# KHU-VLL/DEVIAS

Measured on AMD Instinct MI355X. Metric: clips/sec fwd+bwd, ViT-B/16 16x224^2 slot head, bs=32/GPU, higher is better.
Workload: dtype bf16

## Files before the change

devias_amd/_lib.py:

```python
from __future__ import annotations

import ctypes
import os
from ctypes import POINTER, Structure, c_char_p, c_float, c_int, c_int32, c_int64, c_void_p

import torch

_HERE = os.path.dirname(os.path.abspath(__file__))
LIB_PATH = os.environ.get("DEVIAS_LIB_PATH") or os.path.join(_HERE, "libdevias_amd.so")

F32, BF16 = 0, 1
ATTN_Q_PRESCALED = 1
ABI_VERSION = 168
ACT_NONE, ACT_GELU, ACT_RELU, ACT_SIGMOID, ACT_DGELU, ACT_DRELU = 0, 1, 2, 3, 4, 5


class GemmArgs(Structure):
    _fields_ = [
        ("A", c_void_p), ("B", c_void_p), ("C", c_void_p),
        ("M", c_int32), ("N", c_int32), ("K", c_int32),
        ("lda", c_int32), ("ldb", c_int32), ("ldc", c_int32),
        ("trans_a", c_int32), ("trans_b", c_int32),
        ("dtype", c_int32), ("c_f32", c_int32),
        ("bias", c_void_p), ("act", c_int32),
        ("aux_in", c_void_p), ("aux_out", c_void_p), ("ld_aux", c_int32),
        ("res", c_void_p), ("ldr", c_int32), ("res_mod", c_int32),
        ("beta", c_float), ("split_k", c_int32), ("ws", c_void_p),
        ("colsum", c_void_p), ("colsum_beta", c_float),
        ("row_scale", c_void_p), ("rows_per_scale", c_int32),
        ("batch", c_int32), ("stride_a", c_int64), ("stride_b", c_int64), ("stride_c", c_int64),
        ("sk_ws", c_void_p), ("sk_ws_bytes", c_int64),
    ]


class LossDims(Structure):
    _fields_ = [(n, c_int32) for n in ("B", "S", "C", "nb", "ns", "D", "G", "N", "nh")] + \
               [("w_scene", c_float), ("w_mask_pred", c_float), ("w_mask_distill", c_float), ("dtype", c_int32), ("scene_ce", c_int32)]


_FP = POINTER(c_float)


class BlockArgs(Structure):
    _fields_ = [(n, c_int32) for n in ("B", "N", "D", "H", "hidden", "dtype")] + [("eps", c_float)] + \
               [(n, c_void_p) for n in ("n1w", "n1b", "n2w", "n2b", "Wqkv", "Wp", "W1", "W2", "qkv_bias", "pb", "b1", "b2", "ds1", "ds2", "save", "ws")] + \
               [("ws_bytes", c_int64), ("sk_ws", c_void_p), ("sk_ws_bytes", c_int64)] + \
               [(n, c_void_p) for n in ("WqkvT", "WpT", "W1T", "W2T")] + \
               [("WqkvS", c_void_p), ("qkv_biasS", c_void_p)]


class BlockGrads(Structure):
    _fields_ = [(n, c_void_p) for n in ("dn1w", "dn1b", "dWqkv", "dbqkv", "dWp", "dbp", "dn2w", "dn2b", "dW1", "db1", "dW2", "db2", "dx_colsum")] + \
               [("db2_done", c_int32), ("dbq", c_void_p), ("dbv", c_void_p)]


class HeadArgs(Structure):
    _fields_ = [(n, c_int32) for n in ("R", "D", "C", "h1", "h2", "G", "dtype")] + \
               [(n, c_void_p) for n in ("Wh", "W0", "W2", "W4", "bh", "b0", "b2", "b4", "ws")] + [("ws_bytes", c_int64), ("drop_mask", c_void_p)]


class HeadGrads(Structure):
    _fields_ = [(n, c_void_p) for n in ("dWh", "dbh", "dW0", "db0", "dW2", "db2", "dW4", "db4")]


AGG_MAX_DEPTH = 16
AGG_PARAM_FIELDS = ("Wq", "Wk", "Wv", "Wo", "W1", "W2", "bo", "norm_w", "norm_b", "ctx_w", "ctx_b", "b1", "b2", "ffn_w", "ffn_b")
AGG_GRAD_FIELDS = ("dWq", "dWk", "dWv", "dWo", "dbo", "dnorm_w", "dnorm_b", "dctx_w", "dctx_b", "dW1", "db1", "dW2", "db2", "dffn_w", "dffn_b")


class AggLayerParams(Structure):
    _fields_ = [(n, c_void_p) for n in AGG_PARAM_FIELDS]


class AggLayerGrads(Structure):
    _fields_ = [(n, c_void_p) for n in AGG_GRAD_FIELDS]


class AggArgs(Structure):
    _fields_ = [(n, c_int32) for n in ("B", "N", "S", "D", "depth", "tied", "heads", "dh", "ff", "dtype")] + \
               [("eps_enc", c_float), ("eps_agg", c_float)] + \
               [(n, c_void_p) for n in ("norm_w", "norm_b", "latents", "last_w", "last_b")] + \
               [("sets", AggLayerParams * AGG_MAX_DEPTH), ("save", c_void_p), ("ws", c_void_p), ("ws_bytes", c_int64)]


class AggGrads(Structure):
    _fields_ = [(n, c_void_p) for n in ("dnorm_w", "dnorm_b", "dlatents", "dlast_w", "dlast_b", "dx_colsum")] + \
               [("sets", AggLayerGrads * AGG_MAX_DEPTH)]


_P, _I, _L, _F = c_void_p, c_int32, c_int64, c_float
PROTOTYPES = {
    "devias_version": (c_int, []),
    "devias_last_error": (c_char_p, []),
    "devias_device_info": (c_int, [c_int, POINTER(c_int64)]),
    "devias_allreduce_bucket": (c_int, [_P, _P, _L, _I, _P]),
    "devias_shutdown": (None, []),
    "devias_counter": (c_int64, [c_int32]),
    "devias_counters_reset": (None, []),
    "devias_set_option": (c_int, [c_char_p, c_int32]),
    "devias_get_option": (c_int, [c_char_p, POINTER(c_int32)]),
    "devias_debug_mfma_probe": (c_int, [_P, _L, _I, _I, _P, _P, _P]),
    "devias_debug_mfma_probe_flops": (c_int64, [_I, _I]),
    "devias_debug_gemm_timer_arm": (c_int, [_I, _I, _I, _I, _I]),
    "devias_debug_dkdv_stamps": (c_int, [_P, _I]),
    "devias_debug_gemm_timer_read": (c_int, [POINTER(c_int32), POINTER(c_float)]),
    "devias_debug_gemm_timer_read_each": (c_int, [POINTER(c_int32), POINTER(c_float), c_int32]),
    "devias_gemm_release_queue_stream": (c_int, [_P]),
    "devias_gemm": (c_int, [POINTER(GemmArgs), _P]),
    "devias_gemm_workspace_bytes": (c_int64, [_I, _I, _I]),
    "devias_cast": (c_int, [_P, _I, _P, _I, _L, _P]),
    "devias_cast_scale": (c_int, [_P, _I, _P, _I, _L, c_float, _P]),
    "devias_patch_im2col": (c_int, [_P, _I, _P, _I, _I, _I, _I, _I, _I, _I, _I, _P]),
    "devias_colsum": (c_int, [_P, _I, _I, _I, _I, _P, _F, _P, _P]),
    "devias_colsum_workspace_bytes": (c_int64, [_I, _I]),
    "devias_rows_reduce_mod": (c_int, [_P, _I, _I, _I, _I, _P, _P]),
    "devias_rows_broadcast": (c_int, [_P, _I, _I, _P, _I, _I, _P]),
    "devias_act_bwd": (c_int, [_P, _P, _P, _I, _I, _L, _P]),
    "devias_row_scale": (c_int, [_P, _P, _I, _P, _I, _I, _I, _P]),
    "devias_add": (c_int, [_P, _P, _P, _I, _L, _P]),
    "devias_mul_mask": (c_int, [_P, _P, _P, _P, _I, _L, _P]),
    "devias_layernorm_fwd": (c_int, [_P, _P, _P, _P, _P, _P, _I, _I, _F, _I, _P]),
    "devias_layernorm_bwd": (c_int, [_P, _P, _P, _P, _P, _P, _P, _P, _P, _F, _P, _I, _I, _I, _P, _P]),
    "devias_layernorm_bwd_workspace_bytes": (c_int64, [_I, _I]),
    "devias_mhsa_fwd": (c_int, [_P, _P, _P, _I, _I, _I, _F, _I, _P]),
    "devias_mhsa_bwd": (c_int, [_P, _P, _P, _P, _P, _P, _I, _I, _I, _F, _I, _P, _P]),
    "devias_mhsa_fwd_flags": (c_int, [_P, _P, _P, _I, _I, _I, _F, _I, _I, _P]),
    "devias_mhsa_bwd_flags": (c_int, [_P, _P, _P, _P, _P, _P, _I, _I, _I, _F, _I, _P, _I, _P]),
    "devias_mhsa_bwd_bias_flags": (c_int, [_P, _P, _P, _P, _P, _P, _I, _I, _I, _F, _I, _F, ctypes.c_uint64, _P, _P, _P, _P, _I, _P]),
    "devias_mhsa_bwd_workspace_bytes": (c_int64, [_I, _I, _I]),
    "devias_mhsa_bwd_bias_dv_from_do": (c_int32, [_I, _F]),
    "devias_mhsa_fwd_dropout": (c_int, [_P, _P, _P, _I, _I, _I, _F, _I, _F, ctypes.c_uint64, _P]),
    "devias_mhsa_bwd_dropout": (c_int, [_P, _P, _P, _P, _P, _P, _I, _I, _I, _F, _I, _F, ctypes.c_uint64, _P]),
    "devias_mhsa_bwd_bias": (c_int, [_P, _P, _P, _P, _P, _P, _I, _I, _I, _F, _I, _F, ctypes.c_uint64, _P, _P, _P, _P, _P]),
    "devias_mhsa_bwd_bias_workspace_bytes": (c_int64, [_I, _I, _I]),
    "devias_slot_attn_fwd": (c_int, [_P, _P, _P, _P, _P, _I, _I, _I, _I, _I, _F, _I, _P, _P]),
    "devias_slot_attn_bwd": (c_int, [_P, _P, _P, _P, _P, _P, _P, _P, _P, _I, _I, _I, _I, _I, _F, _I, _P, _P]),
    "devias_slot_attn_kv_grad": (c_int, [_P, _P, _P, _P, _P, _P, _I, _I, _I, _I, _I, _I, _F, _I, _P]),
    "devias_slot_attn_workspace_bytes": (c_int64, [_I, _I, _I, _I, _I]),
    "devias_slotf_fwd": (c_int, [_P, _P, _P, _P, _P, _I, _I, _I, _I, _I, _F, _I, _P, _P]),
    "devias_slotf_bwd": (c_int, [_P, _P, _P, _P, _P, _P, _P, _P, _I, _I, _I, _I, _I, _F, _I, _P, _P]),
    "devias_slotf_pack": (c_int, [_P, _P, _P, _P, _P, _P, _P, _I, _I, _I, _I, _I, _I, _I, _F, _I, _P]),
    "devias_slotf_workspace_bytes": (c_int64, [_I, _I, _I, _I, _I]),
    "devias_slot_select": (c_int, [_P, _I, _I, _I, _I, _I, _P, _P]),
    "devias_head_match_loss_fwd": (c_int, [POINTER(LossDims), _P, _P, _P, _P, _P, _P, _P, _P, _P, _P, _P, _P, _P]),
    "devias_head_match_loss_bwd": (c_int, [POINTER(LossDims), _P, _P, _P, _P, _P, _P, _P, _P, _P, _P, _P, _P, _P, _P, _P]),
    "devias_head_match_loss_workspace_bytes": (c_int64, [_I]),
    "devias_head_match_loss_labels_fwd": (c_int, [POINTER(LossDims), _P, _P, _P, _P, _P, _P, _P, _P, _P, _P, _P, _P, _P]),
    "devias_head_match_loss_labels_bwd": (c_int, [POINTER(LossDims), _P, _P, _P, _P, _P, _P, _P, _P, _P, _P, _P, _P, _P, _P, _P]),
    "devias_adamw_step": (c_int, [_P, _P, _P, _P, _L, _F, _F, _F, _F, _F, _I, _F, _P]),
    "devias_grad_sumsq_multi": (c_int, [_P, _P, _P, _I, _P, _P]),
    "devias_clip_coef": (c_int, [_P, _I, _F, _P, _P]),
    "devias_adamw_multi": (c_int, [_P, _P, _P, _I, _F, _F, _F, _F, _P, _P]),
    "devias_fame_diff_color": (c_int, [_P, _I, _I, _I, _I, _P, _P, _P]),
    "devias_fame_blur": (c_int, [_P, _P, _I, _I, _I, _I, _F, _P]),
    "devias_fame_seg_refine": (c_int, [_P, _P, _I, _I, _I, _F, _P, _P]),
    "devias_fame_binarize_pool": (c_int, [_P, _I, _I, _I, _I, _I, _P, _P, _P]),
    "devias_fame_mix": (c_int, [_P, _P, _I, _P, _P, _P, _P, _I, _I, _I, _P]),
    "devias_debug_cu_hog": (c_int, [_I, _I, _P]),
    "devias_range_push": (None, [c_char_p]),
    "devias_range_pop": (None, []),
    "devias_encoder_block_save_bytes": (c_int64, [_I, _I, _I, _I, _I, _I]),
    "devias_encoder_block_scratch_bytes": (c_int64, [_I, _I, _I, _I, _I, _I]),
    "devias_encoder_block_workspace_bytes": (c_int64, [_I, _I, _I, _I, _I, _I]),
    "devias_encoder_block_fwd": (c_int, [POINTER(BlockArgs), _P, _P, _P]),
    "devias_encoder_block_bwd": (c_int, [POINTER(BlockArgs), _P, _P, _P, POINTER(BlockGrads), _P, _L, _P]),
    "devias_head_workspace_bytes": (c_int64, [_I, _I, _I, _I, _I, _I, _I]),
    "devias_head_save_bytes": (c_int64, [_I, _I, _I, _I, _I]),
    "devias_head_fwd": (c_int, [POINTER(HeadArgs), _P, _P, _P, _P, _P]),
    "devias_head_bwd": (c_int, [POINTER(HeadArgs), _P, _P, _P, _P, _P, _P, POINTER(HeadGrads), _P]),
    "devias_agg_block_save_bytes": (c_int64, [POINTER(AggArgs)]),
    "devias_agg_block_scratch_bytes": (c_int64, [POINTER(AggArgs)]),
    "devias_agg_block_workspace_bytes": (c_int64, [POINTER(AggArgs)]),
    "devias_agg_block_fwd": (c_int, [POINTER(AggArgs), _P, _P, POINTER(c_void_p), _P]),
    "devias_agg_block_bwd": (c_int, [POINTER(AggArgs), _P, _P, _P, _P, POINTER(AggGrads), _P, _L, _P]),
    "devias_policy_gemm_cus": (c_int32, []),
    "devias_policy_small_m_split": (c_int32, [_I, _I, _I, _I]),
    "devias_policy_wgrad_split": (c_int32, [_I, _I, _I, _I]),
}
COUNTERS = {"gemm128_f32": 0, "gemm128_bf16": 1, "gemm_ss": 2, "gemm256": 3, "gemm256p": 4, "splitk_reduce": 5,
            "mhsa_fwd_bf16": 6, "mhsa_bwd_bf16": 7, "mhsa_fwd_f32": 8, "mhsa_bwd_f32": 9, "mhsa_bwd_fused": 10, "gemm_sk": 11, "gemm256w": 12, "gemm_smallm": 13, "gemm256d": 14,
            "dkdv1w": 15, "dkdv1w_pers": 16, "dkdv1w_rest": 17, "dkdv2w": 18, "mhsa_qpre": 19, "loss_labels": 20}
OPT_CHUNK = 16384
OPT_TENSOR_BYTES = 64

_lib = None


class DeviasLibraryError(RuntimeError):
    pass


def load() -> ctypes.CDLL:
    global _lib
    if _lib is not None:
        return _lib
    if not os.path.exists(LIB_PATH):
        raise DeviasLibraryError(
            f"{LIB_PATH} is missing: the HIP extension is not built. Run `python -m devias_amd.build` "
            "(hipcc, gfx950). There is no CPU/PyTorch fallback for the DEVIAS hot path.")
    try:
        lib = ctypes.CDLL(LIB_PATH)
    except OSError as e:
        raise DeviasLibraryError(f"cannot load {LIB_PATH}: {e}") from e
    for name, (res, args) in PROTOTYPES.items():
        try:
            fn = getattr(lib, name)
        except AttributeError as e:
            raise DeviasLibraryError(f"{LIB_PATH} does not export {name}; rebuild it") from e
        fn.restype = res
        fn.argtypes = args
    if lib.devias_version() < ABI_VERSION:
        raise DeviasLibraryError(f"{LIB_PATH} is ABI version {lib.devias_version()}, this binding needs {ABI_VERSION}; rebuild it (python -m devias_amd.build --force)")
    _lib = lib
    return lib


CALLS = [0]


def check(rc: int, what: str) -> None:
    CALLS[0] += 1
    if rc != 0:
        msg = load().devias_last_error()
        raise RuntimeError(f"{what} failed (code {rc}): {msg.decode() if msg else '?'}")
```

devias_amd/csrc/api.hip:

```cpp
#include "common.h"
#include <string.h>

static thread_local char g_err[512] = "";

int devias_set_error(int code, const char* fmt, ...) {
    va_list ap;
    va_start(ap, fmt);
    vsnprintf(g_err, sizeof(g_err), fmt, ap);
    va_end(ap);
    return code;
}

extern "C" int devias_version(void) { return 168; }

#include <atomic>
static std::atomic<int64_t> g_cnt[DEVIAS_CNT_MAX];
void devias_count(int id) { if (id >= 0 && id < DEVIAS_CNT_MAX) g_cnt[id].fetch_add(1, std::memory_order_relaxed); }
extern "C" int64_t devias_counter(int32_t id) { return (id >= 0 && id < DEVIAS_CNT_MAX) ? g_cnt[id].load(std::memory_order_relaxed) : -1; }
extern "C" void devias_counters_reset(void) { for (int i = 0; i < DEVIAS_CNT_MAX; ++i) g_cnt[i].store(0, std::memory_order_relaxed); }

extern "C" int devias_set_option(const char* name, int32_t value) {
    if (!name) return devias_set_error(DEVIAS_EINVAL, "devias_set_option: null name");
    if (devias_gemm_set_option(name, value) || devias_attn_set_option(name, value)) return DEVIAS_OK;
    if (!strcmp(name, "regions_defer")) { devias_defer_enabled() = value; return DEVIAS_OK; }
    return devias_set_error(DEVIAS_EINVAL, "devias_set_option: unknown option '%s'", name);
}

extern "C" int devias_get_option(const char* name, int32_t* value) {
    if (!name || !value) return devias_set_error(DEVIAS_EINVAL, "devias_get_option: null argument");
    int v = 0;
    if (devias_gemm_get_option(name, &v) || devias_attn_get_option(name, &v)) { *value = v; return DEVIAS_OK; }
    if (!strcmp(name, "regions_defer")) { *value = devias_defer_enabled(); return DEVIAS_OK; }
    return devias_set_error(DEVIAS_EINVAL, "devias_get_option: unknown option '%s'", name);
}

extern "C" const char* devias_last_error(void) { return g_err; }
DeviasDeferList*& devias_defer_slot() { static thread_local DeviasDeferList* slot = nullptr; return slot; }
int& devias_defer_enabled() { static int on = [] { const char* e = getenv("DEVIAS_REGIONS_DEFER"); return e ? atoi(e) : 1; }(); return on; }

extern "C" int devias_device_info(int device, int64_t* out5) {
    if (!out5) return devias_set_error(DEVIAS_EINVAL, "devias_device_info: null output");
    hipDeviceProp_t p;
    hipError_t e = hipGetDeviceProperties(&p, device);
    if (e != hipSuccess) return devias_set_error(DEVIAS_ELAUNCH, "devias_device_info: %s", hipGetErrorString(e));
    out5[0] = p.multiProcessorCount;
    out5[1] = p.clockRate;
    out5[2] = (int64_t)p.sharedMemPerBlock;
    out5[3] = p.warpSize;
    int arch = 0;
    const char* s = strstr(p.gcnArchName, "gfx");
    if (s) arch = atoi(s + 3);
    out5[4] = arch;
    return DEVIAS_OK;
}


#include <dlfcn.h>
typedef int (*devias_nccl_allreduce_fn)(const void*, void*, size_t, int, int, void*, hipStream_t);
static devias_nccl_allreduce_fn resolve_allreduce() {
    static devias_nccl_allreduce_fn fn = [] {
        void* sym = dlsym(RTLD_DEFAULT, "ncclAllReduce");
        if (!sym) {
            void* h = dlopen("librccl.so", RTLD_NOW | RTLD_GLOBAL);
            if (!h) h = dlopen("librccl.so.1", RTLD_NOW | RTLD_GLOBAL);
            if (h) sym = dlsym(h, "ncclAllReduce");
        }
        return (devias_nccl_allreduce_fn)sym;
    }();
    return fn;
}
extern "C" int devias_allreduce_bucket(void* nccl_comm, void* bucket, int64_t count, int32_t dtype, void* stream) {
    if (!nccl_comm || !bucket || count <= 0) return devias_set_error(DEVIAS_EINVAL, "devias_allreduce_bucket: null communicator / bucket or empty bucket");
    if (dtype != DEVIAS_F32 && dtype != DEVIAS_BF16) return devias_set_error(DEVIAS_EINVAL, "devias_allreduce_bucket: bad dtype %d", dtype);
    devias_nccl_allreduce_fn fn = resolve_allreduce();
    if (!fn) return devias_set_error(DEVIAS_EUNSUPPORTED, "devias_allreduce_bucket: ncclAllReduce not found (librccl.so is not loadable)");
    const int nccl_dtype = dtype == DEVIAS_F32 ? 7  : 9 ;
    const int rc = fn(bucket, bucket, (size_t)count, nccl_dtype, 0 , nccl_comm, (hipStream_t)stream);
    if (rc != 0) return devias_set_error(DEVIAS_ELAUNCH, "devias_allreduce_bucket: ncclAllReduce returned %d", rc);
    return DEVIAS_OK;
}

extern "C" void devias_shutdown(void) { devias_counters_reset(); }


#include "roctx_shim.h"
#include <stdlib.h>
typedef int (*roctx_push_fn)(const char*);
typedef int (*roctx_pop_fn)(void);
static roctx_push_fn g_roctx_push = nullptr;
static roctx_pop_fn g_roctx_pop = nullptr;
static int g_roctx_state = -1;
static int roctx_resolve() {
    const char* e = getenv("DEVIAS_ROCTX");
    if (!e || atoi(e) == 0) return 0;
    const char* libs[] = {"librocprofiler-sdk-roctx.so", "librocprofiler-sdk-roctx.so.1", "libroctx64.so", "libroctx64.so.4"};
    for (const char* l : libs) {
// ... 17 lines not shown
```

devias_amd/csrc/gemm.hip:

```cpp
#include "common.h"
#include <mutex>
#include <utility>
#include <stdlib.h>
#include <string.h>
#include <atomic>

namespace {

enum { BM = 128, BN = 128, NTHREADS = 256 };

struct GemmP {
    const void* A; const void* B; void* C;
    int M, N, K, lda, ldb, ldc;
    const float* bias; int act;
    const void* aux_in; void* aux_out; int ld_aux;
    const void* res; int ldr, res_mod;
    float beta; int c_f32; int vec_c; int vec16;
    float* ws; int k_per_split; int split_k;
    int tiles_m, tiles_n;
    const float* row_scale; int rows_per_scale;
    float* colsum_part;
    int group_m;
    int epi_swap;
    int debug;
    int aux_nt;
    int c_nt;
    int tail_split;
    int64_t sA, sB, sC;
    unsigned int* tq; unsigned int* tq_clear; int tq_nwhole[2], tq_items[2];
};

#ifdef DEVIAS_GEMM_DEBUG
#define GDBG(flag) (p.debug & (flag))
#else
#define GDBG(flag) 0
#endif

template <typename T> struct Tr;
template <> struct Tr<bf16> {
    enum { BK = 64, KSTEP = 32, CH = 8, KC_BYTES = 128 * 128, KS_BYTES = 64 * 256 };
    typedef bf16x8 frag;
};
template <> struct Tr<float> {
    enum { BK = 16, KSTEP = 4, CH = 4, KC_BYTES = 128 * 20 * 4, KS_BYTES = 16 * 144 * 4 };
    typedef float frag;
};

__device__ __forceinline__ int ks_f(int k) { return (k & 3) | (((k >> 3) & 1) << 2); }
template <typename T> __device__ __forceinline__ int off_kc(int row, int k);
template <typename T> __device__ __forceinline__ int off_ks(int k, int col);
template <> __device__ __forceinline__ int off_kc<bf16>(int row, int k) {
    return row * 128 + ((((k >> 3) ^ (row & 7))) << 4) + (k & 7) * 2;
}
template <> __device__ __forceinline__ int off_ks<bf16>(int k, int col) {
    return k * 256 + ((((col >> 4) ^ ks_f(k))) << 5) + (col & 15) * 2;
}
template <> __device__ __forceinline__ int off_kc<float>(int row, int k) { return (row * 20 + k) * 4; }
template <> __device__ __forceinline__ int off_ks<float>(int k, int col) { return (k * 144 + col) * 4; }

template <typename T, bool KSTRIDED, bool VEC>
struct Stage {
    enum { BK = Tr<T>::BK, CH = Tr<T>::CH, NCH = 128 * BK / CH / NTHREADS, NEL = 128 * BK / NTHREADS };
    u32x4 v[NCH];

    __device__ __forceinline__ void load(const T* __restrict__ ptr, int ld, int r0, int R, int k0, int kend, int tid) {
        if constexpr (VEC) {
#pragma unroll
            for (int i = 0; i < NCH; ++i) {
                int c = tid + i * NTHREADS;
                int row, k;
                if constexpr (!KSTRIDED) { row = c / (BK / CH); k = (c % (BK / CH)) * CH; }
                else { k = c / (128 / CH); row = (c % (128 / CH)) * CH; }
                int gr = r0 + row, gk = k0 + k;
                bool ok = gr < R && gk < kend;
                const T* src = KSTRIDED ? ptr + (int64_t)gk * ld + gr : ptr + (int64_t)gr * ld + gk;
                u32x4 z = {0u, 0u, 0u, 0u};
                v[i] = ok ? *reinterpret_cast<const u32x4*>(src) : z;
            }
        } else {
            T* e = reinterpret_cast<T*>(v);
#pragma unroll
            for (int i = 0; i < NCH; ++i) {
                int c = tid + i * NTHREADS;
                int row, k;
                if constexpr (!KSTRIDED) { row = c / (BK / CH); k = (c % (BK / CH)) * CH; }
                else { k = c / (128 / CH); row = (c % (128 / CH)) * CH; }
#pragma unroll
                for (int j = 0; j < CH; ++j) {
                    int gr = r0 + row + (KSTRIDED ? j : 0), gk = k0 + k + (KSTRIDED ? 0 : j);
                    bool ok = gr < R && gk < kend;
                    const T* src = KSTRIDED ? ptr + (int64_t)gk * ld + gr : ptr + (int64_t)gr * ld + gk;
                    e[i * CH + j] = ok ? *src : from_f32<T>(0.f);
                }
            }
        }
    }

    __device__ __forceinline__ void store(char* lds, int tid) const {
#pragma unroll
        for (int i = 0; i < NCH; ++i) {
            int c = tid + i * NTHREADS;
            int off;
            if constexpr (!KSTRIDED) { int row = c / (BK / CH), k = (c % (BK / CH)) * CH; off = off_kc<T>(row, k); }
            else { int k = c / (128 / CH), col = (c % (128 / CH)) * CH; off = off_ks<T>(k, col); }
            *reinterpret_cast<u32x4*>(lds + off) = v[i];
        }
    }
};

template <bool KSTRIDED>
__device__ __forceinline__ bf16x8 read_frag(const char* lds, int base16, int ks, int lane, bf16*) {
    if constexpr (!KSTRIDED) {
// ... 590 lines not shown
template <int N>
__device__ __forceinline__ void tr_fence(TrFrag (&f)[N]) {
    static_assert(N == 4 || N == 8, "fragment groups of 4 (B) or 8 (A)");
    if constexpr (N == 4)
        asm volatile("s_waitcnt lgkmcnt(0)" : "+v"(f[0].lo), "+v"(f[0].hi), "+v"(f[1].lo), "+v"(f[1].hi), "+v"(f[2].lo), "+v"(f[2].hi), "+v"(f[3].lo), "+v"(f[3].hi) :: "memory");
    else
        asm volatile("s_waitcnt lgkmcnt(0)" : "+v"(f[0].lo), "+v"(f[0].hi), "+v"(f[1].lo), "+v"(f[1].hi), "+v"(f[2].lo), "+v"(f[2].hi), "+v"(f[3].lo), "+v"(f[3].hi),
                     "+v"(f[4].lo), "+v"(f[4].hi), "+v"(f[5].lo), "+v"(f[5].hi), "+v"(f[6].lo), "+v"(f[6].hi), "+v"(f[7].lo), "+v"(f[7].hi) :: "memory");
}
template <int N>
__device__ __forceinline__ void plain_fence(bf16x8 (&f)[N]) {
    static_assert(N == 4 || N == 8, "fragment groups of 4 (B) or 8 (A)");
    if constexpr (N == 4) asm volatile("s_waitcnt lgkmcnt(0)" : "+v"(f[0]), "+v"(f[1]), "+v"(f[2]), "+v"(f[3]) :: "memory");
    else asm volatile("s_waitcnt lgkmcnt(0)" : "+v"(f[0]), "+v"(f[1]), "+v"(f[2]), "+v"(f[3]), "+v"(f[4]), "+v"(f[5]), "+v"(f[6]), "+v"(f[7]) :: "memory");
}

__device__ __forceinline__ void ktile_nt_pinned(f32x4 (&acc)[8][4], const char* cur, char* nxt, const bf16* a_next, int lda,
                                                const bf16* b_next, int ldb, int wave, int lane, int wm, int wn) {
    const char* sA = cur; const char* sB = cur + 32768;
    const uint32_t vo_a = glds_voff_kc(lda, lane), vo_b = glds_voff_kc(ldb, lane);
    bf16x8 fb0[4], fb1[4], fa0[4], fa1[4];
#define G_RA(ks, ih, i) read_frag2<false>(sA, wm * 128 + ((ih) * 4 + (i)) * 16, ks, lane)
#define G_RB(ks, j) read_frag2<false>(sB, wn * 64 + (j) * 16, ks, lane)
#define G_MM4(ih, i, fb, fa) _Pragma("unroll") for (int j = 0; j < 4; ++j) acc[(ih) * 4 + (i)][j] = mfma16(fb[j], fa[i], acc[(ih) * 4 + (i)][j]);
#define G_SB __builtin_amdgcn_sched_barrier(0);
#define G_DMA(n) { const int r8 = wave * 32 + ((n) & 3) * 8; \
                   const char* ub = reinterpret_cast<const char*>((n) < 4 ? a_next + (int64_t)r8 * lda : b_next + (int64_t)r8 * ldb); \
                   __builtin_amdgcn_global_load_lds((glb_void_ptr)(ub + ((n) < 4 ? vo_a : vo_b)), (lds_void_ptr)(nxt + ((n) < 4 ? 0 : 32768) + r8 * 128), 16, 0, 0); }
    G_SB
#pragma unroll
    for (int j = 0; j < 4; ++j) fb0[j] = G_RB(0, j);
#pragma unroll
    for (int i = 0; i < 4; ++i) fa0[i] = G_RA(0, 0, i);
    G_SB
    G_MM4(0, 0, fb0, fa0) G_DMA(0) fa1[0] = G_RA(0, 1, 0); fb1[0] = G_RB(1, 0); G_SB
    G_MM4(0, 1, fb0, fa0) G_DMA(1) fa1[1] = G_RA(0, 1, 1); fb1[1] = G_RB(1, 1); G_SB
    G_MM4(0, 2, fb0, fa0) G_DMA(2) fa1[2] = G_RA(0, 1, 2); fb1[2] = G_RB(1, 2); G_SB
    G_MM4(0, 3, fb0, fa0) G_DMA(3) fa1[3] = G_RA(0, 1, 3); fb1[3] = G_RB(1, 3); G_SB
    G_MM4(1, 0, fb0, fa1) G_DMA(4) fa0[0] = G_RA(1, 0, 0); G_SB
    G_MM4(1, 1, fb0, fa1) G_DMA(5) fa0[1] = G_RA(1, 0, 1); G_SB
    G_MM4(1, 2, fb0, fa1) G_DMA(6) fa0[2] = G_RA(1, 0, 2); G_SB
    G_MM4(1, 3, fb0, fa1) G_DMA(7) fa0[3] = G_RA(1, 0, 3); G_SB
    G_MM4(0, 0, fb1, fa0) fa1[0] = G_RA(1, 1, 0); G_SB
    G_MM4(0, 1, fb1, fa0) fa1[1] = G_RA(1, 1, 1); G_SB
    G_MM4(0, 2, fb1, fa0) fa1[2] = G_RA(1, 1, 2); G_SB
    G_MM4(0, 3, fb1, fa0) fa1[3] = G_RA(1, 1, 3); G_SB
    G_MM4(1, 0, fb1, fa1) G_SB
    G_MM4(1, 1, fb1, fa1) G_SB
    G_MM4(1, 2, fb1, fa1) G_SB
    G_MM4(1, 3, fb1, fa1) G_SB
#undef G_RA
#undef G_RB
#undef G_MM4
#undef G_SB
#undef G_DMA
}

template <bool TA, bool TB>
__device__ __forceinline__ void ktile_generic(f32x4 (&acc)[8][4], const char* cur, int lane, int wm, int wn) {
#pragma unroll
    for (int ks = 0; ks < 2; ++ks) {
        bf16x8 fa[8], fb[4];
        if constexpr (TA || TB) {
            TrFrag ta[TA ? 8 : 1], tb[TB ? 4 : 1];
            if constexpr (!TB) { _Pragma("unroll") for (int j = 0; j < 4; ++j) fb[j] = read_frag2<false>(cur + 32768, wn * 64 + j * 16, ks, lane); }
            if constexpr (!TA) { _Pragma("unroll") for (int i = 0; i < 8; ++i) fa[i] = read_frag2<false>(cur, wm * 128 + i * 16, ks, lane); }
            if constexpr (TB) { _Pragma("unroll") for (int j = 0; j < 4; ++j) tb[j] = read_frag2a(cur + 32768, wn * 64 + j * 16, ks, lane); }
            if constexpr (TA) { _Pragma("unroll") for (int i = 0; i < 8; ++i) ta[i] = read_frag2a(cur, wm * 128 + i * 16, ks, lane); }
            if constexpr (TB) { tr_fence(tb); _Pragma("unroll") for (int j = 0; j < 4; ++j) fb[j] = tr_assemble(tb[j]); } else plain_fence(fb);
            if constexpr (TA) { tr_fence(ta); _Pragma("unroll") for (int i = 0; i < 8; ++i) fa[i] = tr_assemble(ta[i]); } else plain_fence(fa);
        } else {
#pragma unroll
            for (int j = 0; j < 4; ++j) fb[j] = read_frag2<TB>(cur + 32768, wn * 64 + j * 16, ks, lane);
#pragma unroll
            for (int i = 0; i < 8; ++i) fa[i] = read_frag2<TA>(cur, wm * 128 + i * 16, ks, lane);
        }
#pragma unroll
        for (int i = 0; i < 8; ++i)
#pragma unroll
            for (int j = 0; j < 4; ++j) acc[i][j] = mfma16(fb[j], fa[i], acc[i][j]);
    }
}

template <bool TA, bool TB, int PIN = 0>
__global__ __launch_bounds__(NT2) void gemm256_kernel(GemmP p) {
    __shared__ __attribute__((aligned(16))) char smem[2 * STAGE2];
    const int tid = threadIdx.x, lane = tid & 63;
    const int wave = __builtin_amdgcn_readfirstlane(tid >> 6);
    const int wm = wave >> 2, wn = wave & 3;
    const int ntiles = p.tiles_m * p.tiles_n;
    int t, z;
    if (gridDim.y == 1 && p.split_k > 1) {
        const int total = ntiles * p.split_k, per = (total + 7) >> 3;
        const int j = (int)(blockIdx.x & 7) * per + (int)(blockIdx.x >> 3);
        if (j >= total || (int)(blockIdx.x >> 3) >= per) return;
        z = j / ntiles; t = j - z * ntiles;
    } else {
        t = xcd_remap(blockIdx.x, ntiles);
        z = blockIdx.y;
    }
    int tm, tn;
    tile_coords(t, p.tiles_m, p.tiles_n, p.group_m, tm, tn);
    const int m0 = tm * T2, n0 = tn * T2;
    const int kbeg = z * p.k_per_split;
    const int kend = min(p.K, kbeg + p.k_per_split);
    int nk = (kend - kbeg) / 64;
    if (GDBG(1)) nk = min(nk, 1);
    const bf16* A = reinterpret_cast<const bf16*>(p.A);
    const bf16* B = reinterpret_cast<const bf16*>(p.B);

#ifdef DEVIAS_GEMM_DEBUG
    unsigned long long st0 = 0, st1 = 0, st2 = 0, st3 = 0;
    if (GDBG(8)) st0 = __builtin_amdgcn_s_memrealtime();
#endif
    f32x4 acc[8][4];
#pragma unroll
    for (int i = 0; i < 8; ++i)
#pragma unroll
        for (int j = 0; j < 4; ++j) acc[i][j] = f32x4{0.f, 0.f, 0.f, 0.f};

    if (nk > 0) {
        glds_tile<TA>(A, p.lda, m0, kbeg, smem, wave, lane);
        glds_tile<TB>(B, p.ldb, n0, kbeg, smem + 32768, wave, lane);
    }
    for (int kt = 0; kt < nk; ++kt) {
#ifdef DEVIAS_GEMM_DEBUG
        if (GDBG(8) && kt == 0) st1 = __builtin_amdgcn_s_memrealtime();
#endif
        asm volatile("s_waitcnt vmcnt(0)" ::: "memory");
        __syncthreads();
#ifdef DEVIAS_GEMM_DEBUG
        if (GDBG(8) && kt == 0) st2 = __builtin_amdgcn_s_memrealtime();
#endif
        char* cur = smem + (kt & 1) * STAGE2;
        char* nxt = smem + ((kt + 1) & 1) * STAGE2;
        if constexpr (!TA && !TB && PIN != 0) {
            const int kn = kbeg + (kt + 1 < nk ? kt + 1 : kt) * 64;
            ktile_nt_pinned(acc, cur, nxt, A + (int64_t)m0 * p.lda + kn, p.lda, B + (int64_t)n0 * p.ldb + kn, p.ldb, wave, lane, wm, wn);
        } else {
            if (kt + 1 < nk && !GDBG(4)) {
                glds_tile<TA>(A, p.lda, m0, kbeg + (kt + 1) * 64, nxt, wave, lane);
                glds_tile<TB>(B, p.ldb, n0, kbeg + (kt + 1) * 64, nxt + 32768, wave, lane);
            }
            ktile_generic<TA, TB>(acc, cur, lane, wm, wn);
        }
    }

#ifdef DEVIAS_GEMM_DEBUG
    if (GDBG(8)) {
        st3 = __builtin_amdgcn_s_memrealtime();
        if (tid == 0) {
            unsigned long long* d = reinterpret_cast<unsigned long long*>(p.ws) + (size_t)blockIdx.x * 6;
            d[0] = st0; d[1] = st1; d[2] = st2; d[3] = st3;
            d[4] = __builtin_amdgcn_s_getreg(0x1800 | 20) ; d[5] = t;
        }
    }
    if (GDBG(2) && acc[0][0][0] != 12345.678f) return;
#endif
    if constexpr (PIN == 1) asm volatile("s_waitcnt vmcnt(0)" ::: "memory");
    if (p.epi_swap) { epilogue_swap<8>(p, acc, m0 + wm * 128, n0 + wn * 64, z, lane); return; }
    __syncthreads();
    epilogue_staged<8, 4>(p, acc, smem + wave * 16384, m0 + wm * 128, n0 + wn * 64, z, lane);
}


__device__ __forceinline__ void piece_rows(int code, int& lo, int& hi) {
    if (code < 0) { lo = 0; hi = 16; }
    else if (code < 16) { lo = 8 * code; hi = lo + 8; }
    else if (code < 32) { const int i = code - 16; lo = i == 0 ? 0 : (i == 1 ? 5 : 11); hi = i == 0 ? 5 : (i == 1 ? 11 : 16); }
    else { lo = 4 * (code - 32); hi = lo + 4; }
}
__device__ __forceinline__ void piece_wave_rows(int code, int wm, int& il, int& ih) {
    int lo, hi;
    piece_rows(code, lo, hi);
    il = max(lo - 8 * wm, 0); ih = min(hi - 8 * wm, 8);
    if (ih < il) ih = il;
}
__device__ __forceinline__ bool piece_needs_wave_rows(int code, int w) {
    int lo, hi;
    piece_rows(code, lo, hi);
    return 2 * w < hi && 2 * w + 2 > lo;
}
template <int IL, int IH>
__device__ __forceinline__ void ktile_nt_rows(f32x4 (&acc)[IH - IL][4], const char* cur, int lane, int wm, int wn) {
#pragma unroll
    for (int ks = 0; ks < 2; ++ks) {
        bf16x8 fb[4];
#pragma unroll
        for (int j = 0; j < 4; ++j) fb[j] = read_frag2<false>(cur + 32768, wn * 64 + j * 16, ks, lane);
#pragma unroll
        for (int i = IL; i < IH; ++i) {
            const bf16x8 fa = read_frag2<false>(cur, wm * 128 + i * 16, ks, lane);
#pragma unroll
            for (int j = 0; j < 4; ++j) acc[i - IL][j] = mfma16(fb[j], fa, acc[i - IL][j]);
        }
    }
}

enum { TQ_RING = 64, TQ_LINE = 32 , TQ_SLOT = 16 * TQ_LINE, TQ_MASKS = 8 * TQ_LINE * 4 , TQ_NONE = 0x0fffffff };
__device__ unsigned int g_tile_queue[TQ_RING][TQ_SLOT];

__device__ __forceinline__ void tq_issue(unsigned& ticket, unsigned int* slot, int queue) {
    const unsigned voff = (unsigned)queue * (TQ_LINE * 4), one = 1u;
    asm volatile("s_nop 4\n\ts_mov_b64 exec, 1\n\tglobal_atomic_add %0, %1, %2, %3 sc0\n\ts_mov_b64 exec, -1" : "+v"(ticket) : "v"(voff), "v"(one), "s"(slot) : "memory");
}
__device__ __forceinline__ void tq_issue_claim(unsigned& old, unsigned int* slot, int queue, unsigned bit) {
    const unsigned voff = TQ_MASKS + (unsigned)queue * (TQ_LINE * 4);
    asm volatile("s_nop 4\n\ts_mov_b64 exec, 1\n\tglobal_atomic_or %0, %1, %2, %3 sc0\n\ts_mov_b64 exec, -1" : "+v"(old) : "v"(voff), "v"(bit), "s"(slot) : "memory");
}
__device__ __forceinline__ void tq_issue_peek(unsigned& snap, unsigned int* slot, int lane) {
    const unsigned voff = (unsigned)(lane & 15) * (TQ_LINE * 4), zero = 0u;
    asm volatile("s_nop 4\n\ts_mov_b64 exec, 0xffff\n\tglobal_atomic_add %0, %1, %2, %3 sc0\n\ts_mov_b64 exec, -1" : "+v"(snap) : "v"(voff), "v"(zero), "s"(slot) : "memory");
}
template <bool WAIT>
__device__ __forceinline__ void tq_publish(char* word, unsigned seq, int code) {
    const unsigned v = ((seq & 15u) << 28) | ((unsigned)code & 0x0fffffffu);
    const unsigned addr = (unsigned)(size_t)(__attribute__((address_space(3))) char*)word;
    if constexpr (WAIT) asm volatile("ds_write_b32 %0, %1\n\ts_waitcnt lgkmcnt(0)" ::"v"(addr), "v"(v) : "memory");
    else asm volatile("ds_write_b32 %0, %1" ::"v"(addr), "v"(v) : "memory");
}
__device__ __forceinline__ int tq_read(const char* word, unsigned seq) {
    unsigned v;
    const unsigned addr = (unsigned)(size_t)(__attribute__((address_space(3))) const char*)word;
    asm volatile("ds_read_b32 %0, %1\n\ts_waitcnt lgkmcnt(0)" : "=v"(v) : "v"(addr) : "memory");
    v = __builtin_amdgcn_readfirstlane(v);
    return (v >> 28) == (seq & 15u) ? (int)(v & 0x0fffffffu) : -2;
}

template <bool TB, int SIDE, bool DYN, int EPI = -1>
__global__ __launch_bounds__(NT2) void gemm256p_kernel(GemmP p) {
    __shared__ __attribute__((aligned(16))) char smem[2 * STAGE2 + (DYN ? 16 : 0)];
    const int tid = threadIdx.x, lane = tid & 63;
#ifdef DEVIAS_GEMM_DEBUG
    const unsigned long long t_entry = __builtin_amdgcn_s_memrealtime();
#endif
    const int wave = __builtin_amdgcn_readfirstlane(tid >> 6);
    const int wm = wave >> 2, wn = wave & 3;
    const int ntiles = p.tiles_m * p.tiles_n;
    const int nk = p.K / 64;
    const bf16* A = reinterpret_cast<const bf16*>(p.A);
    const bf16* B = reinterpret_cast<const bf16*>(p.B);
    const int xcd = blockIdx.x & 7, stride = gridDim.x >> 3;
    const int q = ntiles >> 3, r = ntiles & 7;
    const int base = xcd < r ? xcd * (q + 1) : r * (q + 1) + (xcd - r) * q;
    const int cnt = q + (xcd < r ? 1 : 0);
    const int li0 = blockIdx.x >> 3;
    int li = li0;
    if constexpr (!DYN) { if (li >= cnt) return; }
    auto coords = [&](int l, int& m0, int& n0) {
        int tm, tn;
        tile_coords(base + l, p.tiles_m, p.tiles_n, p.group_m, tm, tn);
        m0 = tm * T2; n0 = tn * T2;
    };
    const int rfull = cnt / stride, rem = cnt - rfull * stride;
    const bool split = p.tail_split != 0 && rfull >= 1 && rem > 0 && 2 * rem <= stride;
    const int parts = (!split || DYN || TB || p.colsum_part != nullptr || p.tail_split < 3) ? 2 : min(min(p.tail_split, 4), stride / rem);
    auto tile_at = [&](int k, int& l, int& half) -> bool {
        half = -1;
        if (k < rfull) { l = li0 + k * stride; return true; }
        if (k > rfull) return false;
        if (split) {
            if (li0 >= parts * rem) return false;
            l = rfull * stride + li0 / parts;
            half = (parts == 2 ? 0 : (parts == 3 ? 16 : 32)) + li0 % parts;
            return true;
        }
        if (li0 >= rem) return false;
        l = rfull * stride + li0;
        return true;
    };
    char* const tq_word = smem + 2 * STAGE2;
    int nwhole_a = p.tq_nwhole[0], nwhole_b = p.tq_nwhole[1], items_a = p.tq_items[0], items_b = p.tq_items[1];
    unsigned int* tq = p.tq;
    if constexpr (DYN) asm volatile("" : "+s"(nwhole_a), "+s"(nwhole_b), "+s"(items_a), "+s"(items_b), "+s"(tq));
    auto qgeom = [&](int y, int& qbase, int& nwhole, int& items) {
        qbase = y < r ? y * (q + 1) : r * (q + 1) + (y - r) * q;
        nwhole = y < r ? nwhole_a : nwhole_b;
        items = y < r ? items_a : items_b;
    };
    auto decode = [&](int code, int& m0, int& n0, int& half) {
        const int y = code >> 20, i = code & 0xfffff;
        int qbase, nwhole, items;
        qgeom(y, qbase, nwhole, items);
        const int l = i < nwhole ? i : nwhole + ((i - nwhole) >> 1);
        half = i < nwhole ? -1 : ((i - nwhole) & 1);
        int tm, tn;
        tile_coords(qbase + l, p.tiles_m, p.tiles_n, p.group_m, tm, tn);
        m0 = tm * T2; n0 = tn * T2;
    };
    int fq = xcd;
    bool fdead = false;
    unsigned ticket = 0, seq = 0;
    auto settle = [&]() -> int {
        const int t = stride + (int)__builtin_amdgcn_readfirstlane(ticket);
        int qbase, nwhole, items;
        qgeom(fq, qbase, nwhole, items);
        return t < items ? ((fq << 20) | t) : -2;
    };
    auto find_elsewhere = [&]() -> int {
        const int lane_f = __builtin_amdgcn_mbcnt_hi(~0u, __builtin_amdgcn_mbcnt_lo(~0u, 0u));
        const unsigned wmask = stride >= 32 ? 0xffffffffu : ((1u << stride) - 1u);
        for (int attempt = 0; attempt < 256 && !fdead; ++attempt) {
            unsigned snap = 0;
            tq_issue_peek(snap, tq, lane_f);
            asm volatile("s_waitcnt vmcnt(0)" : "+v"(snap) :: "memory");
            int pick = -1, kind = 0;
            unsigned bit = 0;
            for (int d = 1; d <= 8 && pick < 0; ++d) {
                const int y = (xcd + d) & 7;
                int qbase, nwhole, items;
                qgeom(y, qbase, nwhole, items);
                if (stride + (int)__builtin_amdgcn_readlane(snap, y) < items) pick = y;
            }
            for (int d = 0; d < 8 && pick < 0 && !(p.debug & 512); ++d) {
                const int y = (xcd + d) & 7;
                const unsigned avail = ~(unsigned)__builtin_amdgcn_readlane(snap, 8 + y) & wmask;
                if (avail) { pick = y; kind = 1; bit = avail & (0u - avail); }
            }
            if (pick < 0) { fdead = true; break; }
            if (kind == 0) {
                fq = pick;
                tq_issue(ticket, tq, fq);
                asm volatile("s_waitcnt vmcnt(0)" : "+v"(ticket) :: "memory");
                const int c = settle();
                if (c != -2) return c;
            } else {
                unsigned old = 0;
                tq_issue_claim(old, tq, pick, bit);
                asm volatile("s_waitcnt vmcnt(0)" : "+v"(old) :: "memory");
                if (!((unsigned)__builtin_amdgcn_readfirstlane(old) & bit)) return (pick << 20) | (int)__builtin_ctz(bit);
            }
        }
        fdead = true;
        return (int)TQ_NONE;
    };
    if constexpr (DYN) {
        if (blockIdx.x == 0 && tid < 16)
            asm volatile("s_nop 4\n\tglobal_store_dword %0, %1, %2 sc1" ::"v"((unsigned)tid * (TQ_LINE * 4)), "v"(0u), "s"(p.tq_clear) : "memory");
    }
// ... 58 lines not shown
                tq_publish<true>(tq_word + 4, 1, c1);
                if (c1 != (int)TQ_NONE && !fdead) tq_issue(ticket, tq, fq);
            }
            __builtin_amdgcn_s_barrier();
            asm volatile("" ::: "memory");
            const int code = tq_read(tq_word, 0);
            if (code == (int)TQ_NONE) return;
            if (code != ((xcd << 20) | li0)) {
                decode(code, m0, n0, half);
                __builtin_amdgcn_s_barrier();
                glds_tile<false>(A, p.lda, m0, 0, smem, wave, lane);
                glds_tile<TB>(B, p.ldb, n0, 0, smem + 32768, wave, lane);
                asm volatile("s_waitcnt vmcnt(0)" ::: "memory");
            }
            ncode = tq_read(tq_word + 4, 1);
            has_next = ncode != (int)TQ_NONE;
            m0n = m0; n0n = n0;
            if (has_next) decode(ncode, m0n, n0n, halfn);
            seq = 2;
        }
        bool act = half < 0 || wm == half;
        bool tail_piece = false;
        int gtail = 0;
        for (int g = 0, kt = 0;; ++g) {
            __builtin_amdgcn_s_barrier();
            asm volatile("" ::: "memory");
            if (kt == 0) { PSTAMP(1); PSTAMP(9); }
            char* cur = smem + (g & 1) * STAGE2;
            char* nxt = smem + ((g + 1) & 1) * STAGE2;
            const bool same = kt + 1 < nk;
            const int am = (same || !has_next) ? m0 : m0n, bn = (same || !has_next) ? n0 : n0n;
            const int kn = same ? (kt + 1) * 64 : (has_next ? 0 : kt * 64);
            int lane_k = __builtin_amdgcn_mbcnt_hi(~0u, __builtin_amdgcn_mbcnt_lo(~0u, 0u));
            asm volatile("" : "+v"(lane_k));
            const bool stage_a = p.tail_split < 2 || act || (DYN && !same && has_next && (halfn < 0 || wm == halfn));
            if constexpr (!TB) {
                if (act) ktile_nt_pinned(acc, cur, nxt, A + (int64_t)am * p.lda + kn, p.lda, B + (int64_t)bn * p.ldb + kn, p.ldb, wave, lane_k, wm, wn);
                else {
                    if (stage_a) glds_tile<false>(A, p.lda, am, kn, nxt, wave, lane_k);
                    glds_tile<false>(B, p.ldb, bn, kn, nxt + 32768, wave, lane_k);
                }
            } else {
                if (stage_a) glds_tile<false>(A, p.lda, am, kn, nxt, wave, lane_k);
                glds_tile<true>(B, p.ldb, bn, kn, nxt + 32768, wave, lane_k);
                if (act) ktile_generic<false, true>(acc, cur, lane_k, wm, wn);
            }
            if (same) {
                ++kt;
                asm volatile("s_waitcnt vmcnt(0)" ::: "memory");
                if (kt == 1) PSTAMP(4);
                continue;
            }
            PSTAMP(2); PSTAMP(10);
            int lane_e = __builtin_amdgcn_mbcnt_hi(~0u, __builtin_amdgcn_mbcnt_lo(~0u, 0u));
            asm volatile("" : "+v"(lane_e));
            if (act) epilogue_swap<8, true, SIDE, EPI>(p, acc, m0 + wm * 128, n0 + wn * 64, 0, lane_e);
            if (!has_next) break;
            int m0x = 0, n0x = 0, halfx = -1;
            bool issued = false;
            if constexpr (DYN) {
                PSTAMP(5);
                if (wave == 0) {
                    asm volatile("" : "+v"(ticket));
                    int c = fdead ? (int)TQ_NONE : settle();
                    if (c == -2) c = find_elsewhere();
                    tq_publish<false>(tq_word, seq, c);
                    issued = c != (int)TQ_NONE && !fdead;
                    if (issued) tq_issue(ticket, tq, fq);
                }
                do { ncode = tq_read(tq_word, seq); } while (ncode == -2);
                ++seq;
                if (ncode != (int)TQ_NONE) decode(ncode, m0x, n0x, halfx);
                PSTAMP(6);
            }
            if (DYN && !act) asm volatile("s_waitcnt vmcnt(0)" ::: "memory");
#if !defined(TQ_EXP) || TQ_EXP != 1
            else if (DYN && issued) asm volatile("s_waitcnt vmcnt(17)" ::: "memory");
#endif
            else asm volatile("s_waitcnt vmcnt(16)" ::: "memory");
            PSTAMP(3);
            kt = 0;
            ++tk;
            m0 = m0n; n0 = n0n; half = halfn;
            if (!DYN && !TB && half >= 16) { tail_piece = true; gtail = g + 1; break; }
            act = half < 0 || wm == half;
            if constexpr (!DYN) {
                int ln = li;
                has_next = tile_at(tk + 1, ln, halfn);
                if (has_next) coords(ln, m0n, n0n);
            } else {
                has_next = ncode != (int)TQ_NONE;
                if (has_next) { m0n = m0x; n0n = n0x; halfn = halfx; }
            }
#pragma unroll
            for (int i = 0; i < 8; ++i)
#pragma unroll
                for (int j = 0; j < 4; ++j) acc[i][j] = f32x4{0.f, 0.f, 0.f, 0.f};
        }
        if constexpr (!DYN && !TB && !(EPI >= 0 && (EPI & EPI_CS))) {
            if (tail_piece) {
                int il, ih;
                piece_wave_rows(half, wm, il, ih);
                auto run = [&](auto ilc, auto ihc) {
                    constexpr int IL = decltype(ilc)::value, IH = decltype(ihc)::value, NR = IH > IL ? IH - IL : 1;
                    f32x4 tacc[NR][4];
#pragma unroll
                    for (int i = 0; i < NR; ++i)
#pragma unroll
                        for (int j = 0; j < 4; ++j) tacc[i][j] = f32x4{0.f, 0.f, 0.f, 0.f};
                    const bool stage_a = p.tail_split < 2 || piece_needs_wave_rows(half, wave);
                    for (int kt = 0, g = gtail; kt < nk; ++kt, ++g) {
                        __builtin_amdgcn_s_barrier();
                        asm volatile("" ::: "memory");
                        char* cur = smem + (g & 1) * STAGE2;
                        char* nxt = smem + ((g + 1) & 1) * STAGE2;
                        int lane_k = __builtin_amdgcn_mbcnt_hi(~0u, __builtin_amdgcn_mbcnt_lo(~0u, 0u));
                        asm volatile("" : "+v"(lane_k));
                        if (kt + 1 < nk) {
                            if (stage_a) glds_tile<false>(A, p.lda, m0, (kt + 1) * 64, nxt, wave, lane_k);
                            glds_tile<false>(B, p.ldb, n0, (kt + 1) * 64, nxt + 32768, wave, lane_k);
                        }
                        if constexpr (IH > IL) ktile_nt_rows<IL, IH>(tacc, cur, lane_k, wm, wn);
                        asm volatile("s_waitcnt vmcnt(0)" ::: "memory");
                    }
                    if constexpr (IH > IL) {
                        int lane_e = __builtin_amdgcn_mbcnt_hi(~0u, __builtin_amdgcn_mbcnt_lo(~0u, 0u));
                        asm volatile("" : "+v"(lane_e));
                        epilogue_swap<NR, true, SIDE, EPI>(p, tacc, m0 + wm * 128 + IL * 16, n0 + wn * 64, 0, lane_e);
                    }
                };
                using std::integral_constant;
                if (il >= ih) run(integral_constant<int, 0>{}, integral_constant<int, 0>{});
                else if (il == 0 && ih == 5) run(integral_constant<int, 0>{}, integral_constant<int, 5>{});
                else if (il == 5 && ih == 8) run(integral_constant<int, 5>{}, integral_constant<int, 8>{});
                else if (il == 0 && ih == 3) run(integral_constant<int, 0>{}, integral_constant<int, 3>{});
                else if (il == 3 && ih == 8) run(integral_constant<int, 3>{}, integral_constant<int, 8>{});
                else if (il == 0 && ih == 4) run(integral_constant<int, 0>{}, integral_constant<int, 4>{});
                else run(integral_constant<int, 4>{}, integral_constant<int, 8>{});
            }
        }
        asm volatile("s_waitcnt vmcnt(0)" ::: "memory");
    }
}


enum { NTW = 256 };

#define DEVIAS_A10(b) "a" #b "0", "a" #b "1", "a" #b "2", "a" #b "3", "a" #b "4", "a" #b "5", "a" #b "6", "a" #b "7", "a" #b "8", "a" #b "9"
template <int I> __device__ __forceinline__ void acc_zero1() { asm volatile("v_accvgpr_write_b32 a[%c0], 0" ::"i"(I)); }
template <int... I> __device__ __forceinline__ void acc_zero_seq(std::integer_sequence<int, I...>) { (acc_zero1<I>(), ...); }
__device__ __forceinline__ void acc_claim() {
    asm volatile("" ::: DEVIAS_A10(), DEVIAS_A10(1), DEVIAS_A10(2), DEVIAS_A10(3), DEVIAS_A10(4), DEVIAS_A10(5), DEVIAS_A10(6), DEVIAS_A10(7), DEVIAS_A10(8), DEVIAS_A10(9),
                 DEVIAS_A10(10), DEVIAS_A10(11), DEVIAS_A10(12), DEVIAS_A10(13), DEVIAS_A10(14), DEVIAS_A10(15), DEVIAS_A10(16), DEVIAS_A10(17), DEVIAS_A10(18), DEVIAS_A10(19),
                 DEVIAS_A10(20), DEVIAS_A10(21), DEVIAS_A10(22), DEVIAS_A10(23), DEVIAS_A10(24), "a250", "a251", "a252", "a253", "a254", "a255");
}
__device__ __forceinline__ void acc_zero() { acc_zero_seq(std::make_integer_sequence<int, 256>{}); }
template <int I> __device__ __forceinline__ float acc_read1() { float x; asm volatile("v_accvgpr_read_b32 %0, a[%c1]" : "=v"(x) : "i"(I)); return x; }

template <int SIDE>
__device__ __forceinline__ bf16x8 side_load_w(const GemmP& p, int mrow0, int ncol0, int lane, int n) {
    const int lm = lane & 15, g = lane >> 4;
    const bf16* side = reinterpret_cast<const bf16*>(SIDE == 1 ? p.res : p.aux_in);
    const int side_ld = SIDE == 1 ? p.ldr : p.ld_aux;
    const int h = n >> 4, i = (n >> 1) & 7, pr = n & 1;
    int m = mrow0 + i * 16 + lm;
    if (SIDE == 1 && p.res_mod > 0) m %= p.res_mod;
    return *reinterpret_cast<const bf16x8*>(side + (int64_t)m * side_ld + ncol0 + 64 * h + 16 * (2 * pr + (g & 1)) + 8 * (g >> 1));
}

template <int SIDE>
__device__ __forceinline__ void epilogue_w(const GemmP& p, int mrow0, int ncol0, int lane, bf16x8 (&sbuf)[SIDE != 0 ? 16 : 1]) {
    const int lm = lane & 15, g = lane >> 4;
    const uint32_t col2 = (uint32_t)(16 * (g & 1) + 8 * (g >> 1)) * 2;
    const uint32_t vo_c = (uint32_t)lm * (uint32_t)p.ldc * 2 + col2, vo_x = (uint32_t)lm * (uint32_t)p.ld_aux * 2 + col2;
    constexpr bool BIAS_ON = SIDE != 2, CS_ON = SIDE != 1;
    f32x4 bias4[BIAS_ON ? 8 : 1];
    if constexpr (BIAS_ON) {
#pragma unroll
        for (int j = 0; j < 8; ++j) bias4[j] = p.bias ? *reinterpret_cast<const f32x4*>(p.bias + ncol0 + j * 16 + g * 4) : f32x4{0.f, 0.f, 0.f, 0.f};
    }
    float rs_lo = 1.f, rs_hi = 1.f;
    int rs_edge = 0;
    if (p.row_scale) {
        const int r0 = mrow0 / p.rows_per_scale, rl = (p.M - 1) / p.rows_per_scale;
        rs_lo = p.row_scale[r0]; rs_hi = p.row_scale[r0 < rl ? r0 + 1 : rl];
        rs_edge = (r0 + 1) * p.rows_per_scale;
    }
    bf16* aux_out = reinterpret_cast<bf16*>(p.aux_out);
    constexpr int PF = 16;
    auto side_load = [&](int n) -> bf16x8 { return side_load_w<SIDE>(p, mrow0, ncol0, lane, n); };
    float cs[CS_ON ? 4 : 1][8];
    if constexpr (CS_ON) {
#pragma unroll
        for (int c = 0; c < 4; ++c)
#pragma unroll
            for (int e = 0; e < 8; ++e) cs[c][e] = 0.f;
    }
    static_for<32>([&](auto nc) {
        constexpr int n = decltype(nc)::value, h = n >> 4, i = (n >> 1) & 7, pr = n & 1;
        constexpr int ra = 16 * (8 * h + i) + 8 * pr;
        const int m = mrow0 + i * 16 + lm;
        bf16x8 side8 = sbuf[SIDE != 0 ? n % PF : 0];
        if constexpr (SIDE != 0 && n + PF < 32) sbuf[n % PF] = side_load(n + PF);
        f32x4 A = f32x4{acc_read1<ra>(), acc_read1<ra + 1>(), acc_read1<ra + 2>(), acc_read1<ra + 3>()};
        f32x4 B = f32x4{acc_read1<ra + 4>(), acc_read1<ra + 5>(), acc_read1<ra + 6>(), acc_read1<ra + 7>()};
        if constexpr (BIAS_ON) { A += bias4[4 * h + 2 * pr]; B += bias4[4 * h + 2 * pr + 1]; }
        else { A += f32x4{0.f, 0.f, 0.f, 0.f}; B += f32x4{0.f, 0.f, 0.f, 0.f}; }
        float v[8];
#pragma unroll
        for (int r = 0; r < 4; ++r) {
            const auto sw = __builtin_amdgcn_permlane16_swap(__float_as_uint(A[r]), __float_as_uint(B[r]), false, false);
            v[r] = __uint_as_float(sw[0]);
            v[4 + r] = __uint_as_float(sw[1]);
        }
        if constexpr (SIDE == 2) {
            if (p.act == DEVIAS_ACT_DGELU) {
#pragma unroll
                for (int e = 0; e < 8; e += 2) {
                    const f32x2 d = dgelu_fast2(f32x2{(float)side8[e], (float)side8[e + 1]});
                    v[e] *= d[0]; v[e + 1] *= d[1];
                }
            } else {
#pragma unroll
                for (int e = 0; e < 8; ++e) v[e] = (float)side8[e] > 0.f ? v[e] : 0.f;
// ... 490 lines not shown
        for (int w = 0; w < 3; ++w) v += red[w][t][lane];
        if (m >= p.M) continue;
        if (p.bias) v += bias;
        if (p.act == DEVIAS_ACT_GELU) {
            if (aux_out) store4(aux_out + (int64_t)m * p.ld_aux + n, v);
#pragma unroll
            for (int e = 0; e < 4; ++e) v[e] = gelu_t<bf16>(v[e]);
        } else if (p.act == DEVIAS_ACT_RELU) {
#pragma unroll
            for (int e = 0; e < 4; ++e) v[e] = fmaxf(v[e], 0.f);
        } else if (p.act == DEVIAS_ACT_SIGMOID) {
#pragma unroll
            for (int e = 0; e < 4; ++e) v[e] = 1.0f / (1.0f + expf(-v[e]));
        } else if (dact) {
            const f32x4 a4 = {(float)auxv[t][0], (float)auxv[t][1], (float)auxv[t][2], (float)auxv[t][3]};
#pragma unroll
            for (int e = 0; e < 4; ++e) v[e] = p.act == DEVIAS_ACT_DGELU ? v[e] * dgelu_t<bf16>(a4[e]) : (a4[e] > 0.f ? v[e] : 0.f);
        }
        if (p.row_scale) v *= p.row_scale[m / p.rows_per_scale];
        if (res) v += f32x4{(float)resv[t][0], (float)resv[t][1], (float)resv[t][2], (float)resv[t][3]};
        store4(C + (int64_t)m * p.ldc + n, v);
    }
}

__global__ __launch_bounds__(256) void splitk_reduce_plain_kernel(const float* __restrict__ ws, int split_k, int64_t total4, float* __restrict__ C, float beta) {
    for (int64_t i = (int64_t)blockIdx.x * 256 + threadIdx.x; i < total4; i += (int64_t)gridDim.x * 256) {
        f32x4 v = *reinterpret_cast<const f32x4*>(ws + i * 4);
        for (int z = 1; z < split_k; ++z) v += *reinterpret_cast<const f32x4*>(ws + ((int64_t)z * total4 + i) * 4);
        if (beta != 0.f) v += beta * *reinterpret_cast<const f32x4*>(C + i * 4);
        *reinterpret_cast<f32x4*>(C + i * 4) = v;
    }
}

__global__ void gemm_colsum_final_kernel(const float* __restrict__ part, int nparts, int N, float* __restrict__ out, float beta) {
    __shared__ float sm[16][64];
    int n = blockIdx.x * 64 + threadIdx.x;
    float s = 0.f;
    if (n < N)
        for (int i = threadIdx.y; i < nparts; i += 16) s += part[(int64_t)i * N + n];
    sm[threadIdx.y][threadIdx.x] = s;
    __syncthreads();
    if (threadIdx.y == 0 && n < N) {
        float t = 0.f;
#pragma unroll
        for (int k = 0; k < 16; ++k) t += sm[k][threadIdx.x];
        out[n] = t + (beta != 0.f ? beta * out[n] : 0.f);
    }
}

template <typename T, bool VEC>
int launch(const GemmP& p, int ta, int tb, hipStream_t st, int batch = 1) {
    dim3 grid(p.tiles_m * p.tiles_n, p.split_k, batch), block(NTHREADS);
    if (!ta && !tb) hipLaunchKernelGGL((gemm_kernel<T, false, false, VEC>), grid, block, 0, st, p);
    else if (!ta && tb) hipLaunchKernelGGL((gemm_kernel<T, false, true, VEC>), grid, block, 0, st, p);
    else if (ta && tb) hipLaunchKernelGGL((gemm_kernel<T, true, true, VEC>), grid, block, 0, st, p);
    else hipLaunchKernelGGL((gemm_kernel<T, true, false, VEC>), grid, block, 0, st, p);
    return 0;
}

}

extern "C" int64_t devias_gemm_workspace_bytes(int32_t M, int32_t N, int32_t split_k) {
    return split_k > 1 ? (int64_t)split_k * M * N * 4 : 0;
}

namespace {
struct GemmKnobs {
    int epi_swap;
    int use256;
    int use_ss;
    int group_m;
    int persistent;
    int debug;
    int epi_spec;
    int wt;
    int aux_nt;
    int smallm;
    int tail_split;
    int w4;
    int splitk_xcd;
    int dynamic;
    int concurrent;
    int reserve;
    int ncu;
};
int env_int(const char* name, int dflt) { const char* e = getenv(name); return e ? atoi(e) : dflt; }
GemmKnobs& knobs() {
    static GemmKnobs k = [] {
        GemmKnobs x;
        x.epi_swap = env_int("DEVIAS_GEMM_EPI", 1);
        x.use256 = env_int("DEVIAS_GEMM256", 1);
        x.use_ss = env_int("DEVIAS_GEMM_SS", -1);
        x.group_m = env_int("DEVIAS_GEMM_GROUPM", 0);
        x.persistent = env_int("DEVIAS_GEMM_PERSIST", 1);
        x.debug = env_int("DEVIAS_GEMM_DEBUG", 0);
        x.reserve = env_int("DEVIAS_GEMM_RESERVE_CUS", 0);
        x.splitk_xcd = env_int("DEVIAS_GEMM_SPLITK_XCD", 1);
        x.dynamic = env_int("DEVIAS_GEMM_DYNAMIC", -1);
        x.concurrent = env_int("DEVIAS_GEMM_CONCURRENT", 0);
        x.w4 = env_int("DEVIAS_GEMM_W4", -1);
        x.tail_split = env_int("DEVIAS_GEMM_TAIL_SPLIT", 3);
        x.smallm = env_int("DEVIAS_GEMM_SMALLM", 1);
        x.epi_spec = env_int("DEVIAS_GEMM_EPI_SPEC", 1);
        x.wt = env_int("DEVIAS_GEMM_WT", 1);
        x.aux_nt = env_int("DEVIAS_GEMM_AUX_NT", 5);
        x.ncu = 0;
        return x;
    }();
    return k;
}
}

namespace {
struct TileQueueRing { unsigned int* base; hipStream_t owner; bool owned; unsigned seq; };
std::mutex g_tq_mutex;
TileQueueRing g_tq_ring[16];
}
static bool tile_queue_slot(hipStream_t st, unsigned int** slot, unsigned int** clear) {
    int dev = 0;
    if (hipGetDevice(&dev) != hipSuccess || dev < 0 || dev >= 16) return false;
    std::lock_guard<std::mutex> lock(g_tq_mutex);
    TileQueueRing& r = g_tq_ring[dev];
    if (!r.base) {
        void* sym = nullptr;
        if (hipGetSymbolAddress(&sym, HIP_SYMBOL(g_tile_queue)) != hipSuccess || !sym) { (void)hipGetLastError(); return false; }
        r.base = reinterpret_cast<unsigned int*>(sym);
    }
    if (!r.owned) { r.owner = st; r.owned = true; }
    if (r.owner != st) return false;
    const unsigned n = r.seq++;
    *slot = r.base + (size_t)(n % TQ_RING) * TQ_SLOT;
    *clear = r.base + (size_t)((n + TQ_RING / 2) % TQ_RING) * TQ_SLOT;
    return true;
}
extern "C" int devias_gemm_release_queue_stream(void* stream) {
    int dev = 0;
    if (hipGetDevice(&dev) != hipSuccess || dev < 0 || dev >= 16) return devias_set_error(DEVIAS_EINVAL, "devias_gemm_release_queue_stream: no current device");
    std::lock_guard<std::mutex> lock(g_tq_mutex);
    TileQueueRing& r = g_tq_ring[dev];
    if (r.base && hipMemsetAsync(r.base, 0, sizeof(unsigned int) * TQ_RING * TQ_SLOT, (hipStream_t)stream) != hipSuccess) {
        (void)hipGetLastError();
        return devias_set_error(DEVIAS_EINVAL, "devias_gemm_release_queue_stream: cannot zero the ring");
    }
    r.owner = (hipStream_t)stream; r.owned = true; r.seq = 0;
    return DEVIAS_OK;
}

int devias_policy_gemm_wt(void) { return knobs().wt; }

extern "C" int32_t devias_policy_gemm_cus(void) {
    const GemmKnobs& k = knobs();
    const int ncu = devias_device_cus();
    return (ncu - k.reserve > 8 ? ncu - k.reserve : 8) & ~7;
}

static int* gemm_option_slot(const char* name) {
    GemmKnobs& k = knobs();
    if (!strcmp(name, "gemm_epi")) return &k.epi_swap;
    if (!strcmp(name, "gemm256")) return &k.use256;
    if (!strcmp(name, "gemm_ss")) return &k.use_ss;
    if (!strcmp(name, "gemm_groupm")) return &k.group_m;
    if (!strcmp(name, "gemm_persistent")) return &k.persistent;
    if (!strcmp(name, "gemm_debug")) return &k.debug;
    if (!strcmp(name, "gemm_w4")) return &k.w4;
    if (!strcmp(name, "gemm_tail_split")) return &k.tail_split;
    if (!strcmp(name, "gemm_smallm")) return &k.smallm;
    if (!strcmp(name, "gemm_epi_spec")) return &k.epi_spec;
    if (!strcmp(name, "gemm_wt")) return &k.wt;
    if (!strcmp(name, "gemm_aux_nt")) return &k.aux_nt;
    if (!strcmp(name, "gemm_reserve_cus")) return &k.reserve;
    if (!strcmp(name, "gemm_splitk_xcd")) return &k.splitk_xcd;
    if (!strcmp(name, "gemm_dynamic")) return &k.dynamic;
    if (!strcmp(name, "gemm_concurrent")) return &k.concurrent;
    return nullptr;
}
int devias_gemm_set_option(const char* name, int value) {
    int* slot = gemm_option_slot(name);
    if (!slot) return 0;
    *slot = (!strcmp(name, "gemm_reserve_cus") && value < 0) ? 0 : value;
    return 1;
}
int devias_gemm_get_option(const char* name, int* value) {
    const int* slot = gemm_option_slot(name);
    if (!slot) return 0;
    *value = *slot;
    return 1;
}

namespace {
template <bool TB, int SIDE, bool DYN, int EPI>
void pers_launch1(dim3 grid, hipStream_t st, const GemmP& p) { hipLaunchKernelGGL((gemm256p_kernel<TB, SIDE, DYN, EPI>), grid, dim3(NT2), 0, st, p); }
template <bool DYN>
void pers_launch(bool tb, int side, int epi, dim3 grid, hipStream_t st, const GemmP& p) {
    if (!tb && side == 0) {
        if (epi == EPI_BIAS) pers_launch1<false, 0, DYN, EPI_BIAS>(grid, st, p);
        else if (epi == (DEVIAS_ACT_GELU | EPI_BIAS | EPI_AUX)) pers_launch1<false, 0, DYN, DEVIAS_ACT_GELU | EPI_BIAS | EPI_AUX>(grid, st, p);
        else if (epi == 0) pers_launch1<false, 0, DYN, 0>(grid, st, p);
        else if (epi == EPI_CS) pers_launch1<false, 0, DYN, EPI_CS>(grid, st, p);
        else pers_launch1<false, 0, DYN, -1>(grid, st, p);
    } else if (!tb && side == 1) {
        if (epi == EPI_BIAS) pers_launch1<false, 1, DYN, EPI_BIAS>(grid, st, p);
        else pers_launch1<false, 1, DYN, -1>(grid, st, p);
    } else if (!tb) {
        if (epi == (DEVIAS_ACT_DGELU | EPI_CS)) pers_launch1<false, 2, DYN, DEVIAS_ACT_DGELU | EPI_CS>(grid, st, p);
        else pers_launch1<false, 2, DYN, -1>(grid, st, p);
    } else if (side == 0) pers_launch1<true, 0, DYN, -1>(grid, st, p);
    else pers_launch1<true, 2, DYN, -1>(grid, st, p);
}
}

static int gemm_impl(const devias_gemm_args* a, void* stream) {
    hipStream_t st = (hipStream_t)stream;
    DEVIAS_REQUIRE(a && a->A && a->B && a->C, "devias_gemm: null operand");
    DEVIAS_REQUIRE(a->M > 0 && a->N > 0 && a->K > 0, "devias_gemm: bad dims M=%d N=%d K=%d", a->M, a->N, a->K);
    DEVIAS_REQUIRE(a->dtype == DEVIAS_F32 || a->dtype == DEVIAS_BF16, "devias_gemm: bad dtype %d", a->dtype);
    DEVIAS_REQUIRE(a->act >= 0 && a->act <= DEVIAS_ACT_DRELU, "devias_gemm: bad act %d", a->act);
    if (a->act == DEVIAS_ACT_DGELU || a->act == DEVIAS_ACT_DRELU)
        DEVIAS_REQUIRE(a->aux_in, "devias_gemm: act %d needs aux_in", a->act);
    const GemmKnobs& kn = knobs();
    const int es = a->dtype == DEVIAS_BF16 ? 2 : 4;
    const int ch = 16 / es;
    GemmP p;
    p.A = a->A; p.B = a->B; p.C = a->C;
    p.M = a->M; p.N = a->N; p.K = a->K; p.lda = a->lda; p.ldb = a->ldb; p.ldc = a->ldc;
    p.bias = a->bias; p.act = a->act; p.aux_in = a->aux_in; p.aux_out = a->aux_out; p.ld_aux = a->ld_aux;
    p.res = a->res; p.ldr = a->ldr; p.res_mod = a->res_mod;
    p.c_f32 = (a->c_f32 || a->dtype == DEVIAS_F32) ? 1 : 0;
    p.beta = p.c_f32 ? a->beta : 0.f;
    p.tiles_m = cdiv(a->M, BM); p.tiles_n = cdiv(a->N, BN);
    const int BK = a->dtype == DEVIAS_BF16 ? 64 : 16;
    int split = a->split_k > 1 ? a->split_k : 1;
    if (split > 1) {
        DEVIAS_REQUIRE(a->ws, "devias_gemm: split_k needs a workspace");
        int kps = cdiv(cdiv(a->K, split), BK) * BK;
        split = cdiv(a->K, kps);
        p.k_per_split = kps;
    } else {
        p.k_per_split = a->K;
    }
    p.split_k = split; p.ws = a->ws;
    p.colsum_part = nullptr;
    p.row_scale = a->row_scale; p.rows_per_scale = a->rows_per_scale > 0 ? a->rows_per_scale : 1;
    bool vec = aligned16(a->A) && aligned16(a->B) && (a->lda % ch == 0) && (a->ldb % ch == 0);
    vec = vec && (a->trans_a ? (a->M % ch == 0) : (a->K % ch == 0));
    vec = vec && (a->trans_b ? (a->N % ch == 0) : (a->K % ch == 0));
    if (a->batch > 1) vec = vec && (a->stride_a % ch == 0) && (a->stride_b % ch == 0);
    bool vc = (a->N % 4 == 0) && (a->ldc % 4 == 0) && (p.c_f32 ? aligned16(a->C) : aligned8(a->C));
    if (a->bias) vc = vc && aligned16(a->bias);
    if (a->res) vc = vc && (a->ldr % 4 == 0) && aligned8(a->res);
    if (a->aux_in) vc = vc && (a->ld_aux % 4 == 0) && aligned8(a->aux_in);
    if (a->aux_out) vc = vc && (a->ld_aux % 4 == 0) && aligned8(a->aux_out);
    if (es == 4) vc = vc && (!a->res || aligned16(a->res)) && (!a->aux_in || aligned16(a->aux_in)) &&
                      (!a->aux_out || aligned16(a->aux_out)) && aligned16(a->C);
    if (a->batch > 1) vc = vc && (a->stride_c % 4 == 0);
    p.vec_c = vc ? 1 : 0;
    const int batch = a->batch > 1 ? a->batch : 1;
    p.sA = batch > 1 ? a->stride_a : 0; p.sB = batch > 1 ? a->stride_b : 0; p.sC = batch > 1 ? a->stride_c : 0;
    if (batch > 1)
        DEVIAS_REQUIRE(split == 1 && !a->colsum && !a->res && !a->aux_in && !a->aux_out && batch <= 65535,
                       "devias_gemm: batched launches support bias / activation epilogues only (no split-K, residual, aux, colsum)");
    p.debug = kn.debug;
    p.tail_split = kn.tail_split;
    p.aux_nt = kn.aux_nt;
    p.c_nt = ((kn.aux_nt & 4) && a->aux_out) ? 1 : 0;
    p.epi_swap = kn.epi_swap;
    p.tq = nullptr; p.tq_clear = nullptr; p.tq_nwhole[0] = p.tq_nwhole[1] = p.tq_items[0] = p.tq_items[1] = 0;
    p.group_m = kn.group_m > 0 ? kn.group_m : ((!a->trans_a && a->N >= 2048) ? 8 : 1);

    const bool v16 = vc && (a->N % 8 == 0) && (a->ldc % 8 == 0) && aligned16(a->C) && (!a->bias || aligned16(a->bias)) &&
                     (!a->res || ((a->ldr % 8 == 0) && aligned16(a->res))) &&
                     (!a->aux_in || ((a->ld_aux % 8 == 0) && aligned16(a->aux_in))) &&
                     (!a->aux_out || ((a->ld_aux % 8 == 0) && aligned16(a->aux_out))) && (split == 1 || aligned16(a->ws));
    p.vec16 = (v16 && a->dtype == DEVIAS_BF16) ? 1 : 0;
    bool big = kn.use256 && a->dtype == DEVIAS_BF16 && vec && vc && (a->M % T2 == 0) && (a->N % T2 == 0) && (a->K % 64 == 0) &&
               (p.k_per_split % 64 == 0);
    big = big && v16 && batch == 1;
    bool ss = kn.use_ss != 0 && a->dtype == DEVIAS_BF16 && vec && v16 && (a->M % SS_BM == 0) && (a->N % SS_BN == 0) && (a->K % 64 == 0) &&
              (p.k_per_split % 64 == 0) && batch == 1 && !(a->trans_a && !a->trans_b);
    if (ss && big) {
        const bool nt = !a->trans_a && !a->trans_b;
        if (kn.use_ss < 0 || nt) ss = false;
    }
    const bool smallm = kn.smallm && a->dtype == DEVIAS_BF16 && !a->trans_a && (!a->trans_b || kn.smallm == 1) && a->M <= 128 && batch == 1 && !p.c_f32 && !a->colsum && vec && vc &&
                        (a->N % 16 == 0) && (a->K % 128 == 0) && (a->lda % 8 == 0) && (a->ldb % 8 == 0) && (a->ldc % 4 == 0) && aligned8(a->C) &&
                        (!a->bias || aligned16(a->bias)) && (!a->res || (a->ldr % 4 == 0 && aligned8(a->res))) &&
                        (!a->aux_in || (a->ld_aux % 4 == 0 && aligned8(a->aux_in))) && (!a->aux_out || (a->ld_aux % 4 == 0 && aligned8(a->aux_out)));
    if (smallm) {
        p.split_k = 1; p.k_per_split = a->K;
        const int mt = cdiv(a->M, 16);
        dim3 grid(a->N / 16), block(256);
        if (a->trans_b) { grid = dim3(a->N / 16, mt); hipLaunchKernelGGL((gemm_smallm_kernel<1, 12, true>), grid, block, 0, st, p); }
        else if (kn.smallm == 1 && mt > 1 && a->N / 16 < 128) { grid = dim3(a->N / 16, mt); hipLaunchKernelGGL((gemm_smallm_kernel<1, 12>), grid, block, 0, st, p); }
        else
        if (mt <= 1) hipLaunchKernelGGL((gemm_smallm_kernel<1, 12>), grid, block, 0, st, p);
        else if (mt <= 2) hipLaunchKernelGGL((gemm_smallm_kernel<2>), grid, block, 0, st, p);
        else if (mt <= 4) hipLaunchKernelGGL((gemm_smallm_kernel<4>), grid, block, 0, st, p);
        else if (mt <= 6) hipLaunchKernelGGL((gemm_smallm_kernel<6>), grid, block, 0, st, p);
        else hipLaunchKernelGGL((gemm_smallm_kernel<8>), grid, block, 0, st, p);
        devias_count(DEVIAS_CNT_GEMM_SMALLM);
        DEVIAS_CHECK_LAUNCH("devias_gemm(small M)");
        return DEVIAS_OK;
    }
    bool colsum_fused = false;
    if (a->colsum) {
        DEVIAS_REQUIRE(split == 1 && a->ws && !(a->c_f32 && a->dtype == DEVIAS_BF16),
                       "devias_gemm: colsum needs split_k == 1, a workspace (M/128 * N floats) and a T-typed C");
        if (ss || big) { p.colsum_part = a->ws; colsum_fused = true; }
    }
    if (ss) {
        p.tiles_m = a->M / SS_BM; p.tiles_n = a->N / SS_BN;
        dim3 grid(p.tiles_m * p.tiles_n, p.split_k), block(SS_NT);
        const int ta = a->trans_a, tb = a->trans_b;
        if (!ta && !tb) hipLaunchKernelGGL((gemm_ss_kernel<false, false, 2>), grid, block, 0, st, p);
        else if (!ta && tb) hipLaunchKernelGGL((gemm_ss_kernel<false, true, 2>), grid, block, 0, st, p);
        else hipLaunchKernelGGL((gemm_ss_kernel<true, true, 2>), grid, block, 0, st, p);
        devias_count(DEVIAS_CNT_GEMM_SS);
    } else if (big) {
        p.tiles_m = a->M / T2; p.tiles_n = a->N / T2;
        const int ta = a->trans_a, tb = a->trans_b;
        const int nt = p.tiles_m * p.tiles_n;
        const bool dyn = kn.dynamic > 0 || (kn.dynamic < 0 && kn.concurrent != 0);
        const int gp = dyn ? (devias_device_cus() & ~7) : devias_policy_gemm_cus();
        const bool dact = a->act == DEVIAS_ACT_DGELU || a->act == DEVIAS_ACT_DRELU;
        const int side = a->res ? 1 : (dact ? 2 : 0);
        const bool pers_ok = !ta && split == 1 && !p.c_f32 && p.epi_swap && gp >= 8 && !(a->res && dact) && !(tb && side == 1) &&
                             (!a->row_scale || p.rows_per_scale >= 128) && !(side == 2 && a->bias) && !(side == 1 && a->colsum) &&
                             !(side != 0 && a->aux_out);
#define PERS_LAUNCH(KERNEL, ...) do { \
            if (!tb) { if (side == 0) hipLaunchKernelGGL((KERNEL<false, 0 __VA_ARGS__>), grid, block, 0, st, p); else hipLaunchKernelGGL((KERNEL<false, 1 __VA_ARGS__>), grid, block, 0, st, p); } \
            else { if (side == 0) hipLaunchKernelGGL((KERNEL<true, 0 __VA_ARGS__>), grid, block, 0, st, p); else hipLaunchKernelGGL((KERNEL<true, 2 __VA_ARGS__>), grid, block, 0, st, p); } } while (0)
        const int w4_form = (tb ? 2 : 0) + (side != 0 ? 1 : 0);
        const int w4_mask = kn.w4 >= 0 ? kn.w4 : 0;
        const bool w4_ok = kn.persistent && !dyn && ((w4_mask >> w4_form) & 1) && pers_ok && !(!tb && side == 2) && nt > gp && a->K >= 128 &&
                           (a->act == DEVIAS_ACT_NONE || a->act == DEVIAS_ACT_GELU || a->act == DEVIAS_ACT_DGELU || a->act == DEVIAS_ACT_DRELU);
        if (w4_ok) {
            dim3 grid(gp), block(NTW);
            PERS_LAUNCH(gemm256w_kernel);
            devias_count(DEVIAS_CNT_GEMM256P);
            devias_count(DEVIAS_CNT_GEMM256W);
        } else if (kn.persistent && pers_ok && nt > gp) {
            dim3 grid(gp);
            const int epi = !kn.epi_spec ? -1 : (a->act | (a->bias ? EPI_BIAS : 0) | (a->aux_out ? EPI_AUX : 0) | (a->row_scale ? EPI_RS : 0) | (p.colsum_part ? EPI_CS : 0));
            unsigned int *tq = nullptr, *tq_clear = nullptr;
            if (!(dyn && a->K >= 128 && (gp >> 3) <= 32 && (nt >> 3) >= (gp >> 3) && tile_queue_slot(st, &tq, &tq_clear))) tq = nullptr;
            if (tq) {
                p.tq = tq;
                p.tq_clear = tq_clear;
                const int stride = gp >> 3;
                for (int v = 0; v < 2; ++v) {
                    const int cnt = (nt >> 3) + (v == 0 ? 1 : 0);
                    const int rfull = cnt / stride, rem = cnt - rfull * stride;
                    const bool split = kn.tail_split != 0 && rfull >= 1 && rem > 0 && 2 * rem <= stride;
                    p.tq_nwhole[v] = split ? rfull * stride : cnt;
                    p.tq_items[v] = split ? rfull * stride + 2 * rem : cnt;
                }
                pers_launch<true>(tb != 0, side, epi, grid, st, p);
                devias_count(DEVIAS_CNT_GEMM256D);
            } else {
                pers_launch<false>(tb != 0, side, epi, grid, st, p);
            }
            devias_count(DEVIAS_CNT_GEMM256P);
        } else {
            dim3 grid(nt, p.split_k), block(NT2);
            if (p.split_k > 1 && kn.splitk_xcd) grid = dim3(8 * ((nt * p.split_k + 7) / 8));
            if (!ta && !tb) hipLaunchKernelGGL((gemm256_kernel<false, false, 1>), grid, block, 0, st, p);
            else if (!ta && tb) hipLaunchKernelGGL((gemm256_kernel<false, true>), grid, block, 0, st, p);
            else if (ta && tb) hipLaunchKernelGGL((gemm256_kernel<true, true>), grid, block, 0, st, p);
            else hipLaunchKernelGGL((gemm256_kernel<true, false>), grid, block, 0, st, p);
            devias_count(DEVIAS_CNT_GEMM256);
        }
    } else if (a->dtype == DEVIAS_BF16) {
        if (vec) launch<bf16, true>(p, a->trans_a, a->trans_b, st, batch);
        else launch<bf16, false>(p, a->trans_a, a->trans_b, st, batch);
        devias_count(DEVIAS_CNT_GEMM128_BF16);
    } else {
        if (vec) launch<float, true>(p, a->trans_a, a->trans_b, st, batch);
        else launch<float, false>(p, a->trans_a, a->trans_b, st, batch);
        devias_count(DEVIAS_CNT_GEMM128_F32);
    }
    DEVIAS_CHECK_LAUNCH("devias_gemm");
    if (a->colsum) {
        const DeviasReduceJob cj = {a->ws, a->M / 128, a->N, a->N, a->colsum, a->colsum_beta};
        if (colsum_fused && devias_defer(&cj, 1)) {
        } else if (colsum_fused) {
            hipLaunchKernelGGL(gemm_colsum_final_kernel, dim3(cdiv(a->N, 64)), dim3(64, 16), 0, st, a->ws, a->M / 128, a->N, a->colsum, a->colsum_beta);
            DEVIAS_CHECK_LAUNCH("devias_gemm(colsum)");
        } else {
            int rc = devias_colsum(a->C, a->dtype, a->M, a->N, a->ldc, a->colsum, a->colsum_beta, a->ws, stream);
            if (rc) return rc;
        }
    }
    if (split > 1) {
        int64_t total = (int64_t)a->M * a->N;
        int blocks = (int)((total + 255) / 256); if (blocks > 2048) blocks = 2048;
        const bool plain = p.c_f32 && a->ldc == a->N && (total % 4 == 0) && !a->bias && a->act == DEVIAS_ACT_NONE && !a->res && !a->row_scale &&
                           aligned16(a->ws) && aligned16(a->C);
        if (plain) {
            int b4 = (int)((total / 4 + 255) / 256); if (b4 > 2048) b4 = 2048;
            hipLaunchKernelGGL(splitk_reduce_plain_kernel, dim3(b4), dim3(256), 0, st, a->ws, split, total / 4, reinterpret_cast<float*>(a->C), a->beta);
        } else if (a->dtype == DEVIAS_BF16) hipLaunchKernelGGL((splitk_reduce_kernel<bf16>), dim3(blocks), dim3(256), 0, st, p);
        else hipLaunchKernelGGL((splitk_reduce_kernel<float>), dim3(blocks), dim3(256), 0, st, p);
        devias_count(DEVIAS_CNT_SPLITK_REDUCE);
        DEVIAS_CHECK_LAUNCH("devias_gemm(split-k reduce)");
    }
    return DEVIAS_OK;
}

namespace {
struct GemmTimer {
    std::mutex mu;
    bool armed = false;
    int M = 0, N = 0, K = 0, ta = 0, tb = 0, n = 0;
    hipEvent_t e0[64], e1[64];
};
GemmTimer& gemm_timer() { static GemmTimer t; return t; }
std::atomic<int> g_gemm_timer_armed{0};
}
extern "C" int devias_debug_gemm_timer_arm(int32_t M, int32_t N, int32_t K, int32_t trans_a, int32_t trans_b) {
    GemmTimer& t = gemm_timer();
    std::lock_guard<std::mutex> lock(t.mu);
    for (int i = 0; i < t.n; ++i) { (void)hipEventDestroy(t.e0[i]); (void)hipEventDestroy(t.e1[i]); }
    t.n = 0;
    t.armed = M > 0;
    t.M = M; t.N = N; t.K = K; t.ta = trans_a != 0; t.tb = trans_b != 0;
    g_gemm_timer_armed.store(t.armed ? 1 : 0);
    return DEVIAS_OK;
}
extern "C" int devias_debug_gemm_timer_read(int32_t* count, float* total_ms) {
    DEVIAS_REQUIRE(count && total_ms, "devias_debug_gemm_timer_read: null output");
    GemmTimer& t = gemm_timer();
    std::lock_guard<std::mutex> lock(t.mu);
    float sum = 0.f;
    for (int i = 0; i < t.n; ++i) {
        float ms = 0.f;
        if (hipEventSynchronize(t.e1[i]) != hipSuccess || hipEventElapsedTime(&ms, t.e0[i], t.e1[i]) != hipSuccess) {
            (void)hipGetLastError();
            return devias_set_error(DEVIAS_ELAUNCH, "devias_debug_gemm_timer_read: event %d not readable", i);
        }
        sum += ms;
    }
    *count = t.n; *total_ms = sum;
    return DEVIAS_OK;
}

extern "C" int devias_debug_gemm_timer_read_each(int32_t* count, float* each_ms, int32_t cap) {
    DEVIAS_REQUIRE(count && each_ms && cap > 0, "devias_debug_gemm_timer_read_each: null output");
    GemmTimer& t = gemm_timer();
    std::lock_guard<std::mutex> lock(t.mu);
    for (int i = 0; i < t.n && i < cap; ++i) {
        float ms = 0.f;
        if (hipEventSynchronize(t.e1[i]) != hipSuccess || hipEventElapsedTime(&ms, t.e0[i], t.e1[i]) != hipSuccess) {
            (void)hipGetLastError();
            return devias_set_error(DEVIAS_ELAUNCH, "devias_debug_gemm_timer_read_each: event %d not readable", i);
        }
        each_ms[i] = ms;
    }
    *count = t.n < cap ? t.n : cap;
    return DEVIAS_OK;
}

extern "C" int devias_gemm(const devias_gemm_args* a, void* stream) {
    if (!g_gemm_timer_armed.load(std::memory_order_relaxed) || !a) return gemm_impl(a, stream);
    GemmTimer& t = gemm_timer();
    int slot = -1;
    {
        std::lock_guard<std::mutex> lock(t.mu);
        if (t.armed && a->M == t.M && a->N == t.N && a->K == t.K && (a->trans_a != 0) == (t.ta != 0) && (a->trans_b != 0) == (t.tb != 0) && t.n < 64 &&
            hipEventCreate(&t.e0[t.n]) == hipSuccess) {
            if (hipEventCreate(&t.e1[t.n]) == hipSuccess) slot = t.n++;
            else (void)hipEventDestroy(t.e0[t.n]);
        }
    }
    if (slot < 0) return gemm_impl(a, stream);
    (void)hipEventRecord(t.e0[slot], (hipStream_t)stream);
    const int rc = gemm_impl(a, stream);
    (void)hipEventRecord(t.e1[slot], (hipStream_t)stream);
    return rc;
}
```

devias_amd/csrc/regions.hip:

```cpp
#include "common.h"
#include <stdlib.h>
#include <string.h>
#include "roctx_shim.h"

namespace {

inline int64_t al256(int64_t n) { return (n + 255) & ~(int64_t)255; }
inline int esize(int dtype) { return dtype == DEVIAS_BF16 ? 2 : 4; }

int small_m_split(int M, int N, int K, int trans_a) {
    if (!(M <= 256 && K >= 512 && !trans_a)) return 1;
    const int tiles = cdiv(M, 128) * cdiv(N, 128);
    int s = K / 128;
    const int t = (256 + tiles - 1) / tiles;
    if (t < s) s = t;
    return s > 1 ? s : 1;
}
int wgrad_split(int Nout, int Kin, int Mrows, int dtype) {
    const int bk = dtype == DEVIAS_BF16 ? 64 : 16;
    const int cus = devias_policy_gemm_cus();
    int tiles, slots;
    if (bk == 64 && Nout % 256 == 0 && Kin % 128 == 0) { tiles = (Nout / 256) * (Kin / 128); slots = 2 * cus; }
    else { tiles = cdiv(Nout, 128) * cdiv(Kin, 128); slots = 3 * cus; }
    if (tiles >= slots || Mrows < 8 * bk) return 1;
    int s = slots / tiles;
    if (Mrows / (4 * bk) < s) s = Mrows / (4 * bk);
    if (s > 64) s = 64;
    return s > 1 ? s : 1;
}

struct Ctx {
    int dtype;
    float* ws; int64_t ws_bytes;
    void* sk_ws; int64_t sk_ws_bytes;
    void* st;
};

struct Epi {
    const float* bias = nullptr; int act = DEVIAS_ACT_NONE;
    const void* aux_in = nullptr; void* aux_out = nullptr;
    const void* res = nullptr; int res_mod = 0;
    float* colsum = nullptr; float colsum_beta = 0.f;
    const float* row_scale = nullptr; int rows_per_scale = 0;
};
int gemm(const Ctx& c, const void* A, const void* B, void* C, int M, int N, int K, int lda, int ldb, int trans_a, int trans_b, const Epi& e,
         int c_f32 = 0, float beta = 0.f, int split_k = 1) {
    devias_gemm_args a;
    memset(&a, 0, sizeof(a));
    a.A = A; a.B = B; a.C = C; a.M = M; a.N = N; a.K = K; a.lda = lda; a.ldb = ldb; a.ldc = N;
    a.trans_a = trans_a; a.trans_b = trans_b; a.dtype = c.dtype; a.c_f32 = c_f32;
    a.bias = e.bias; a.act = e.act; a.aux_in = e.aux_in; a.aux_out = e.aux_out; a.ld_aux = N;
    a.res = e.res; a.ldr = N; a.res_mod = e.res_mod; a.beta = beta;
    a.row_scale = e.row_scale; a.rows_per_scale = e.rows_per_scale;
    if (split_k == 1) split_k = small_m_split(M, N, K, trans_a);
    if (e.colsum) { split_k = 1; a.colsum = e.colsum; a.colsum_beta = e.colsum_beta; a.ws = c.ws; }
    a.split_k = split_k;
    if (split_k > 1) {
        if (devias_gemm_workspace_bytes(M, N, split_k) > c.ws_bytes) return devias_set_error(DEVIAS_EINVAL, "fused region: workspace too small for a split-K GEMM (%d x %d x %d)", M, N, split_k);
        a.ws = c.ws;
    }
    return devias_gemm(&a, c.st);
}
int wgrad(const Ctx& c, const void* dY, const void* X, float* dW, int M, int Nout, int Kin, float beta = 0.f) {
    Epi e;
    return gemm(c, dY, X, dW, Nout, Kin, M, Nout, Kin, 1, 1, e, 1, beta, wgrad_split(Nout, Kin, M, c.dtype));
}
int gemm_batched(const Ctx& c, const void* A, const void* B, void* C, int c_f32, int M, int N, int K, int lda, int ldb, int ldc, int64_t sa, int64_t sb, int64_t sc,
                 int batch, int trans_a, int trans_b) {
    devias_gemm_args a;
    memset(&a, 0, sizeof(a));
    a.A = A; a.B = B; a.C = C; a.M = M; a.N = N; a.K = K; a.lda = lda; a.ldb = ldb; a.ldc = ldc;
    a.trans_a = trans_a; a.trans_b = trans_b; a.dtype = c.dtype; a.c_f32 = c_f32; a.split_k = 1;
    a.batch = batch; a.stride_a = sa; a.stride_b = sb; a.stride_c = sc;
    return devias_gemm(&a, c.st);
}
int ln_fwd(const Ctx& c, const void* x, const float* g, const float* b, void* y, float* mean, float* rstd, int M, int D, float eps) {
    return devias_layernorm_fwd(x, g, b, y, mean, rstd, M, D, eps, c.dtype, c.st);
}
int ln_bwd(const Ctx& c, const void* dy, const void* x, const float* g, const float* mean, const float* rstd, const void* dres, void* dx, float* dg, float* db,
           float beta_acc, float* dx_colsum, int M, int D) {
    return devias_layernorm_bwd(dy, x, g, mean, rstd, dres, dx, dg, db, beta_acc, dx_colsum, M, D, c.dtype, c.ws, c.st);
}
int colsum(const Ctx& c, const void* x, int M, int N, float* out, float beta = 0.f) { return devias_colsum(x, c.dtype, M, N, N, out, beta, c.ws, c.st); }

#define RUN(call) do { int rc__ = (call); if (rc__) return rc__; } while (0)

int64_t max64(int64_t a, int64_t b) { return a > b ? a : b; }
int64_t gemm_ws(int M, int N, int K, int trans_a) { return devias_gemm_workspace_bytes(M, N, small_m_split(M, N, K, trans_a)); }
int64_t wgrad_ws(int Nout, int Kin, int M, int dtype) { return devias_gemm_workspace_bytes(Nout, Kin, wgrad_split(Nout, Kin, M, dtype)); }
int64_t colsum_gemm_ws(int M, int N) { return max64((int64_t)cdiv(M, 128) * N * 4, devias_colsum_workspace_bytes(M, N)); }

struct BlockSave {
    char *u, *qkv, *o, *x1, *u2, *hpre, *hact;
    float *mean1, *rstd1, *mean2, *rstd2, *lse;
    int64_t bytes;
    BlockSave(void* base, int B, int N, int D, int H, int hid, int dtype) {
        const int64_t M = (int64_t)B * N, es = esize(dtype);
        int64_t off = 0;
        const uintptr_t p = reinterpret_cast<uintptr_t>(base);
        auto take = [&](int64_t n) { char* r = reinterpret_cast<char*>(p + (uintptr_t)off); off += al256(n); return r; };
        u = take(M * D * es); qkv = take(M * 3 * D * es); o = take(M * D * es); x1 = take(M * D * es); u2 = take(M * D * es);
        hpre = take(M * hid * es); hact = take(M * hid * es);
        mean1 = (float*)take(M * 4); rstd1 = (float*)take(M * 4); mean2 = (float*)take(M * 4); rstd2 = (float*)take(M * 4);
        lse = (float*)take((int64_t)B * H * N * 4);
        bytes = off;
    }
};
struct BlockScratch {
    char *big, *small, *dx1, *g;
    float* delta;
    float *p_ln2, *p_ln1, *p_db1, *p_b2, *p_bp, *p_q, *p_v;
    int64_t bytes;
    BlockScratch(void* base, int B, int N, int D, int H, int hid, int dtype) {
        const int64_t M = (int64_t)B * N, es = esize(dtype);
        int64_t off = 0;
        const uintptr_t p = reinterpret_cast<uintptr_t>(base);
        auto take = [&](int64_t n) { char* r = reinterpret_cast<char*>(p + (uintptr_t)off); off += al256(n); return r; };
        big = take(M * (hid > 3 * D ? hid : 3 * D) * es); small = take(M * D * es); dx1 = take(M * D * es); g = take(M * D * es);
        delta = (float*)take((int64_t)B * H * N * 4);
        const int64_t lnw = devias_layernorm_bwd_workspace_bytes((int)M, D), csw = devias_colsum_workspace_bytes((int)M, 3 * D);
        p_ln2 = (float*)take(lnw); p_ln1 = (float*)take(lnw);
        p_db1 = (float*)take(max64((int64_t)cdiv(M, 128) * hid * 4, devias_colsum_workspace_bytes((int)M, hid)));
        p_b2 = (float*)take(csw); p_bp = (float*)take(csw);
        const int64_t abw = max64(csw, devias_mhsa_bwd_bias_workspace_bytes(B, N, H));
        p_q = (float*)take(abw); p_v = (float*)take(abw);
        bytes = off;
    }
};
inline bool block_qpre(const devias_block_args* a) { return a->dtype == DEVIAS_BF16 && a->WqkvS && a->qkv_biasS; }
int block_check(const devias_block_args* a, const char* who) {
    DEVIAS_REQUIRE(a, "%s: null args", who);
    DEVIAS_REQUIRE(a->B > 0 && a->N > 0 && a->D > 0 && a->H > 0 && a->hidden > 0 && a->D == a->H * 64, "%s: bad dims (B=%d N=%d D=%d H=%d hidden=%d; head dim must be 64)", who,
                   a->B, a->N, a->D, a->H, a->hidden);
    DEVIAS_REQUIRE(a->dtype == DEVIAS_BF16 || a->dtype == DEVIAS_F32, "%s: bad dtype %d", who, a->dtype);
    DEVIAS_REQUIRE(a->n1w && a->n1b && a->n2w && a->n2b && a->Wqkv && a->Wp && a->W1 && a->W2 && a->qkv_bias && a->pb && a->b1 && a->b2, "%s: null parameter", who);
    DEVIAS_REQUIRE((a->WqkvS != nullptr) == (a->qkv_biasS != nullptr) && (!a->WqkvS || a->dtype == DEVIAS_BF16), "%s: WqkvS and qkv_biasS go together (bf16 only)", who);
    DEVIAS_REQUIRE(a->save && a->ws && aligned16(a->save) && aligned16(a->ws), "%s: save / ws must be 16-byte aligned, non-null", who);
    DEVIAS_REQUIRE(a->ws_bytes >= devias_encoder_block_workspace_bytes(a->B, a->N, a->D, a->H, a->hidden, a->dtype), "%s: workspace too small", who);
    return DEVIAS_OK;
}

}

extern "C" int64_t devias_encoder_block_save_bytes(int32_t B, int32_t N, int32_t D, int32_t H, int32_t hidden, int32_t dtype) {
    return BlockSave(nullptr, B, N, D, H, hidden, dtype).bytes;
}
extern "C" int64_t devias_encoder_block_scratch_bytes(int32_t B, int32_t N, int32_t D, int32_t H, int32_t hidden, int32_t dtype) {
    return BlockScratch(nullptr, B, N, D, H, hidden, dtype).bytes;
}
extern "C" int64_t devias_encoder_block_workspace_bytes(int32_t B, int32_t N, int32_t D, int32_t H, int32_t hidden, int32_t dtype) {
    const int M = B * N;
    int64_t w = devias_layernorm_bwd_workspace_bytes(M, D);
    w = max64(w, colsum_gemm_ws(M, hidden));
    w = max64(w, devias_colsum_workspace_bytes(M, 3 * D));
    w = max64(w, max64(gemm_ws(M, 3 * D, D, 0), max64(gemm_ws(M, hidden, D, 0), max64(gemm_ws(M, D, hidden, 0), gemm_ws(M, D, 3 * D, 0)))));
    w = max64(w, max64(wgrad_ws(D, hidden, M, dtype), max64(wgrad_ws(hidden, D, M, dtype), max64(wgrad_ws(D, D, M, dtype), wgrad_ws(3 * D, D, M, dtype)))));
    return al256(w) + 256;
}

extern "C" int devias_encoder_block_fwd(const devias_block_args* a, const void* x, void* x2, void* stream) {
    RUN(block_check(a, "devias_encoder_block_fwd"));
    DEVIAS_REQUIRE(x && x2, "devias_encoder_block_fwd: null activation");
    const int B = a->B, N = a->N, D = a->D, H = a->H, hid = a->hidden, M = B * N;
    const Ctx c{a->dtype, a->ws, a->ws_bytes, a->sk_ws, a->sk_ws_bytes, stream};
    const BlockSave s(a->save, B, N, D, H, hid, a->dtype);
    devias_range r("encoder_block_fwd");
    RUN(ln_fwd(c, x, a->n1w, a->n1b, s.u, s.mean1, s.rstd1, M, D, a->eps));
    const bool qpre = block_qpre(a);
    { Epi e; e.bias = qpre ? a->qkv_biasS : a->qkv_bias; RUN(gemm(c, s.u, qpre ? a->WqkvS : a->Wqkv, s.qkv, M, 3 * D, D, D, D, 0, 0, e)); }
    RUN(devias_mhsa_fwd_flags(s.qkv, s.o, s.lse, B, N, H, 0.125f, a->dtype, qpre ? DEVIAS_ATTN_Q_PRESCALED : 0, stream));
    { Epi e; e.bias = a->pb; e.res = x; e.row_scale = a->ds1; e.rows_per_scale = N; RUN(gemm(c, s.o, a->Wp, s.x1, M, D, D, D, D, 0, 0, e)); }
    RUN(ln_fwd(c, s.x1, a->n2w, a->n2b, s.u2, s.mean2, s.rstd2, M, D, a->eps));
    { Epi e; e.bias = a->b1; e.act = DEVIAS_ACT_GELU; e.aux_out = s.hpre; RUN(gemm(c, s.u2, a->W1, s.hact, M, hid, D, D, D, 0, 0, e)); }
    { Epi e; e.bias = a->b2; e.res = s.x1; e.row_scale = a->ds2; e.rows_per_scale = N; RUN(gemm(c, s.hact, a->W2, x2, M, D, hid, hid, hid, 0, 0, e)); }
    return DEVIAS_OK;
}

extern "C" int devias_encoder_block_bwd(const devias_block_args* a, const void* x, const void* dx2, void* dx, const devias_block_grads* g,
                                        void* scratch, int64_t scratch_bytes, void* stream) {
    RUN(block_check(a, "devias_encoder_block_bwd"));
    DEVIAS_REQUIRE(x && dx2 && dx && g && scratch && aligned16(scratch), "devias_encoder_block_bwd: null / unaligned argument");
    DEVIAS_REQUIRE(g->dn1w && g->dn1b && g->dWqkv && (g->dbqkv || (g->dbq && g->dbv)) && g->dWp && g->dbp && g->dn2w && g->dn2b && g->dW1 && g->db1 && g->dW2 && g->dx_colsum &&
                   (g->db2 || g->db2_done), "devias_encoder_block_bwd: null gradient destination");
    const int B = a->B, N = a->N, D = a->D, H = a->H, hid = a->hidden, M = B * N;
    DEVIAS_REQUIRE(scratch_bytes >= devias_encoder_block_scratch_bytes(B, N, D, H, hid, a->dtype), "devias_encoder_block_bwd: scratch too small");
    const Ctx c{a->dtype, a->ws, a->ws_bytes, a->sk_ws, a->sk_ws_bytes, stream};
    const BlockSave s(a->save, B, N, D, H, hid, a->dtype);
    const BlockScratch t(scratch, B, N, D, H, hid, a->dtype);
    devias_range r("encoder_block_bwd");
    const bool wt = a->dtype == DEVIAS_BF16 && devias_policy_gemm_wt() != 0;
    const void *WqkvT = wt ? a->WqkvT : nullptr, *WpT = wt ? a->WpT : nullptr, *W1T = wt ? a->W1T : nullptr, *W2T = wt ? a->W2T : nullptr;
    DeviasDeferList dl; dl.n = 0;
    struct Collect { Collect(DeviasDeferList* l) { devias_defer_slot() = l; } ~Collect() { devias_defer_slot() = nullptr; } } collecting(&dl);
    auto with_ws = [&](float* area) { Ctx k = c; k.ws = area; return k; };
    const void* g2 = dx2;
    if (a->ds2) {
        RUN(devias_row_scale_colsum(dx2, a->ds2, N, t.g, a->dtype, M, D, g->db2, 0.f, t.p_b2, (hipStream_t)stream));
        g2 = t.g;
    } else if (!g->db2_done) {
        RUN(colsum(with_ws(t.p_b2), dx2, M, D, g->db2));
    }
    RUN(wgrad(c, g2, s.hact, g->dW2, M, D, hid));
    { Epi e; e.act = DEVIAS_ACT_DGELU; e.aux_in = s.hpre; e.colsum = g->db1;
      if (W2T) RUN(gemm(with_ws(t.p_db1), g2, W2T, t.big, M, hid, D, D, D, 0, 0, e)); else RUN(gemm(with_ws(t.p_db1), g2, a->W2, t.big, M, hid, D, D, hid, 0, 1, e)); }
    RUN(wgrad(c, t.big, s.u2, g->dW1, M, hid, D));
    { Epi e; if (W1T) RUN(gemm(c, t.big, W1T, t.small, M, D, hid, hid, hid, 0, 0, e)); else RUN(gemm(c, t.big, a->W1, t.small, M, D, hid, hid, D, 0, 1, e)); }
    RUN(ln_bwd(with_ws(t.p_ln2), t.small, s.x1, a->n2w, s.mean2, s.rstd2, dx2, t.dx1, g->dn2w, g->dn2b, 0.f, a->ds1 ? nullptr : g->dbp, M, D));
    const void* g1 = t.dx1;
    if (a->ds1) {
        RUN(devias_row_scale_colsum(t.dx1, a->ds1, N, t.g, a->dtype, M, D, g->dbp, 0.f, t.p_bp, (hipStream_t)stream));
        g1 = t.g;
    }
    RUN(wgrad(c, g1, s.o, g->dWp, M, D, D));
    const bool dv_from_do = g->dbq && g->dbv && devias_mhsa_bwd_bias_dv_from_do(a->dtype, 1.0f);
    const int aflags = block_qpre(a) ? DEVIAS_ATTN_Q_PRESCALED : 0;
    { Epi e; if (dv_from_do) e.colsum = g->dbv;
      const Ctx k = dv_from_do ? with_ws(t.p_v) : c;
      if (WpT) RUN(gemm(k, g1, WpT, t.small, M, D, D, D, D, 0, 0, e)); else RUN(gemm(k, g1, a->Wp, t.small, M, D, D, D, D, 0, 1, e)); }
    if (g->dbq && g->dbv)
        RUN(devias_mhsa_bwd_bias_flags(s.qkv, s.o, t.small, s.lse, t.delta, t.big, B, N, H, 0.125f, a->dtype, 1.0f, 0, g->dbq, dv_from_do ? nullptr : g->dbv, t.p_q, t.p_v, aflags, stream));
    else
        RUN(devias_mhsa_bwd_flags(s.qkv, s.o, t.small, s.lse, t.delta, t.big, B, N, H, 0.125f, a->dtype, t.p_q, aflags, stream));
    RUN(wgrad(c, t.big, s.u, g->dWqkv, M, 3 * D, D));
    if (g->dbq && g->dbv) {
    } else {
        RUN(colsum(with_ws(t.p_q), t.big, M, 3 * D, g->dbqkv));
    }
    { Epi e; if (WqkvT) RUN(gemm(c, t.big, WqkvT, t.small, M, D, 3 * D, 3 * D, 3 * D, 0, 0, e)); else RUN(gemm(c, t.big, a->Wqkv, t.small, M, D, 3 * D, 3 * D, D, 0, 1, e)); }
    RUN(ln_bwd(with_ws(t.p_ln1), t.small, x, a->n1w, s.mean1, s.rstd1, t.dx1, dx, g->dn1w, g->dn1b, 0.f, g->dx_colsum, M, D));
    RUN(devias_flush_deferred(&dl, (hipStream_t)stream));
    return DEVIAS_OK;
}

namespace {
struct HeadSave {
    char *m1, *m2, *sd;
    int64_t bytes;
    HeadSave(void* base, int R, int D, int h1, int h2, int dtype) {
        const int64_t es = esize(dtype);
        int64_t off = 0;
        const uintptr_t p = reinterpret_cast<uintptr_t>(base);
        auto take = [&](int64_t n) { char* r = reinterpret_cast<char*>(p + (uintptr_t)off); off += al256(n); return r; };
        m1 = take((int64_t)R * h1 * es); m2 = take((int64_t)R * h2 * es); sd = take((int64_t)R * D * es);
        bytes = off;
    }
};
int64_t head_tmp_bytes(int R, int D, int h1, int h2, int G, int dtype) {
    const int64_t es = esize(dtype);
    return al256((int64_t)R * G * es) + al256((int64_t)R * h2 * es) + al256((int64_t)R * h1 * es) + 2 * al256((int64_t)R * D * es);
}
int head_check(const devias_head_args* a, const char* who) {
    DEVIAS_REQUIRE(a && a->R > 0 && a->D > 0 && a->C > 0 && a->h1 > 0 && a->h2 > 0 && a->G > 0, "%s: bad dims", who);
    DEVIAS_REQUIRE(a->dtype == DEVIAS_BF16 || a->dtype == DEVIAS_F32, "%s: bad dtype %d", who, a->dtype);
    DEVIAS_REQUIRE(a->Wh && a->bh && a->W0 && a->b0 && a->W2 && a->b2 && a->W4 && a->b4 && a->ws, "%s: null parameter / workspace", who);
    DEVIAS_REQUIRE(a->ws_bytes >= devias_head_workspace_bytes(a->R, a->D, a->C, a->h1, a->h2, a->G, a->dtype), "%s: workspace too small", who);
    return DEVIAS_OK;
}
}

extern "C" int64_t devias_head_workspace_bytes(int32_t R, int32_t D, int32_t C, int32_t h1, int32_t h2, int32_t G, int32_t dtype) {
    int64_t w = 0;
    const int dims[][3] = {{R, C, D}, {R, h1, D}, {R, h2, h1}, {R, G, h2}, {R, h2, G}, {R, h1, h2}, {R, D, h1}, {R, D, C}};
    for (auto& d : dims) w = max64(w, gemm_ws(d[0], d[1], d[2], 0));
    const int wg[][2] = {{G, h2}, {h2, h1}, {h1, D}, {C, D}};
    for (auto& d : wg) w = max64(w, wgrad_ws(d[0], d[1], R, dtype));
    const int cs[] = {G, h2, h1, C};
    for (int n : cs) w = max64(w, devias_colsum_workspace_bytes(R, n));
    return al256(w) + 256 + head_tmp_bytes(R, D, h1, h2, G, dtype);
}
extern "C" int64_t devias_head_save_bytes(int32_t R, int32_t D, int32_t h1, int32_t h2, int32_t dtype) { return HeadSave(nullptr, R, D, h1, h2, dtype).bytes; }

extern "C" int devias_head_fwd(const devias_head_args* a, const void* slots, void* Z, void* Mk, void* save, void* stream) {
    RUN(head_check(a, "devias_head_fwd"));
    DEVIAS_REQUIRE(slots && Z && Mk && save, "devias_head_fwd: null pointer");
    const Ctx c{a->dtype, a->ws, a->ws_bytes, nullptr, 0, stream};
    const HeadSave s(save, a->R, a->D, a->h1, a->h2, a->dtype);
    devias_range r("head_fwd");
    const void* hin = slots;
    if (a->drop_mask) { RUN(devias_mul_mask(slots, a->drop_mask, nullptr, s.sd, a->dtype, (int64_t)a->R * a->D, stream)); hin = s.sd; }
    { Epi e; e.bias = a->bh; RUN(gemm(c, hin, a->Wh, Z, a->R, a->C, a->D, a->D, a->D, 0, 0, e)); }
    { Epi e; e.bias = a->b0; e.act = DEVIAS_ACT_RELU; RUN(gemm(c, slots, a->W0, s.m1, a->R, a->h1, a->D, a->D, a->D, 0, 0, e)); }
    { Epi e; e.bias = a->b2; e.act = DEVIAS_ACT_RELU; RUN(gemm(c, s.m1, a->W2, s.m2, a->R, a->h2, a->h1, a->h1, a->h1, 0, 0, e)); }
    { Epi e; e.bias = a->b4; e.act = DEVIAS_ACT_SIGMOID; RUN(gemm(c, s.m2, a->W4, Mk, a->R, a->G, a->h2, a->h2, a->h2, 0, 0, e)); }
    return DEVIAS_OK;
}

extern "C" int devias_head_bwd(const devias_head_args* a, const void* slots, const void* Mk, const void* save, const void* dZ, const void* dM, void* dslots,
                               const devias_head_grads* g, void* stream) {
    RUN(head_check(a, "devias_head_bwd"));
    DEVIAS_REQUIRE(slots && Mk && save && dZ && dM && dslots && g, "devias_head_bwd: null pointer");
    DEVIAS_REQUIRE(g->dWh && g->dbh && g->dW0 && g->db0 && g->dW2 && g->db2 && g->dW4 && g->db4, "devias_head_bwd: null gradient destination");
    const int R = a->R, D = a->D, C = a->C, h1 = a->h1, h2 = a->h2, G = a->G;
    const int64_t es = esize(a->dtype);
    const int64_t wk = devias_head_workspace_bytes(R, D, C, h1, h2, G, a->dtype) - head_tmp_bytes(R, D, h1, h2, G, a->dtype);
    const Ctx c{a->dtype, a->ws, wk, nullptr, 0, stream};
    char* tp = reinterpret_cast<char*>(a->ws) + wk;
    char* dp3 = tp; tp += al256((int64_t)R * G * es);
    char* dp2 = tp; tp += al256((int64_t)R * h2 * es);
    char* dp1 = tp; tp += al256((int64_t)R * h1 * es);
    char* dsm = tp; tp += al256((int64_t)R * D * es);
    char* dsd = tp;
    const HeadSave s(const_cast<void*>(save), R, D, h1, h2, a->dtype);
    devias_range r("head_bwd");
    RUN(devias_act_bwd(dM, Mk, dp3, DEVIAS_ACT_SIGMOID, a->dtype, (int64_t)R * G, stream));
    RUN(wgrad(c, dp3, s.m2, g->dW4, R, G, h2)); RUN(colsum(c, dp3, R, G, g->db4));
    { Epi e; e.act = DEVIAS_ACT_DRELU; e.aux_in = s.m2; RUN(gemm(c, dp3, a->W4, dp2, R, h2, G, G, h2, 0, 1, e)); }
    RUN(wgrad(c, dp2, s.m1, g->dW2, R, h2, h1)); RUN(colsum(c, dp2, R, h2, g->db2));
    { Epi e; e.act = DEVIAS_ACT_DRELU; e.aux_in = s.m1; RUN(gemm(c, dp2, a->W2, dp1, R, h1, h2, h2, h1, 0, 1, e)); }
    RUN(wgrad(c, dp1, slots, g->dW0, R, h1, D)); RUN(colsum(c, dp1, R, h1, g->db0));
    { Epi e; RUN(gemm(c, dp1, a->W0, dsm, R, D, h1, h1, D, 0, 1, e)); }
    if (a->drop_mask) {
// ... 263 lines not shown
```

devias_amd/modeling_slot.py:

```python
from __future__ import annotations

import math
from functools import partial
from typing import Dict, List, Optional

import numpy as np
import torch
import torch.nn as nn
from torch.autograd import Function

from . import ops
from .ops import ACT_DGELU, ACT_DRELU, ACT_GELU, ACT_NONE, ACT_RELU, ACT_SIGMOID

_MODEL_REGISTRY: Dict[str, callable] = {}


def register_model(fn):
    _MODEL_REGISTRY[fn.__name__] = fn
    try:
        from timm.models.registry import register_model as _timm_register
        _timm_register(fn)
    except Exception:
        pass
    return fn


def create_model(name: str, pretrained: bool = False, **kwargs):
    kwargs = {k: v for k, v in kwargs.items() if v is not None}
    return _MODEL_REGISTRY[name](pretrained=pretrained, **kwargs)


def _cfg(url="", **kwargs):
    return {"url": url, "num_classes": 400, "input_size": (3, 224, 224), "pool_size": None, "crop_pct": .9,
            "interpolation": "bicubic", "mean": (0.5, 0.5, 0.5), "std": (0.5, 0.5, 0.5), **kwargs}


def get_sinusoid_encoding_table(n_position: int, d_hid: int) -> torch.Tensor:
    pos = np.arange(n_position, dtype=np.float64)[:, None]
    j = np.arange(d_hid)
    angle = pos / np.power(10000.0, 2.0 * (j // 2) / d_hid)[None, :]
    table = angle.copy()
    table[:, 0::2] = np.sin(angle[:, 0::2])
    table[:, 1::2] = np.cos(angle[:, 1::2])
    return torch.tensor(table, dtype=torch.float32).unsqueeze(0)


import weakref

_WEIGHTS_EPOCH = [0]


def invalidate_weight_cache() -> None:
    _WEIGHTS_EPOCH[0] += 1


class _WeakIdDict:

    def __init__(self):
        self._d = {}

    def get(self, obj, default=None):
        e = self._d.get(id(obj))
        return e[1] if e is not None and e[0]() is obj else default

    def __setitem__(self, obj, value):
        k = id(obj)
        self._d[k] = (weakref.ref(obj, lambda _r, k=k, d=self._d: d.pop(k, None) if (d.get(k) is not None and d[k][0] is _r) else None), value)

    def __len__(self):
        return len(self._d)


class _WeightCache:
    def __init__(self):
        self._c = _WeakIdDict()
        self._cat = _WeakIdDict()
        self._qkvb = _WeakIdDict()
        self._t = _WeakIdDict()
        self._qs = _WeakIdDict()
        self.casts = 0
        self.transposes = 0
        self.qscaled = 0

    @staticmethod
    def _stamp(p: torch.Tensor):
        return (_WEIGHTS_EPOCH[0], p._version, p.data_ptr(), p.device)

    def get(self, p: torch.Tensor, dtype: torch.dtype) -> torch.Tensor:
        d = p.detach()
        if d.dim() > 2:
            d = d.reshape(d.shape[0], -1)
        if dtype == torch.float32:
            return d if d.is_contiguous() else d.contiguous()
        stamp = self._stamp(p)
        hit = self._c.get(p)
# ... 141 lines not shown
    def forward(ctx, x, weight, bias, pos, meta):
        ts, ps, cdt = meta
        A = ops.patch_im2col(x, ts, ps, cdt)
        w = _WCACHE.get(weight, cdt)
        y = ops.gemm(A, w, bias=_f32(bias), res=pos, res_mod=pos.shape[0])
        ctx.A = A
        ctx.params = (weight, bias)
        return y

    @staticmethod
    def backward(ctx, dy):
        dy = dy.contiguous()
        weight, bias = ctx.params
        dW = ops.wgrad(dy, ctx.A, out=_gout(weight, (weight.shape[0], -1))).view(weight.shape)
        db = _take_colsum(dy, out=_gout(bias))
        ctx.A = None
        return None, dW, db, None, None


class EncoderBlockFn(Function):

    @staticmethod
    def forward(ctx, x, n1w, n1b, qkvw, qb, vb, pw, pb, n2w, n2b, f1w, f1b, f2w, f2b, meta, ds1=None, ds2=None, drop=None):
        B, N, H, eps, cdt = meta
        scale = 64 ** -0.5
        E1, E2, adrop = drop if drop is not None else (None, None, None)
        assert (E1 is None) == (E2 is None) and (E1 is None or (ds1 is None and ds2 is None))
        n1w_, n1b_, n2w_, n2b_ = _f32(n1w), _f32(n1b), _f32(n2w), _f32(n2b)
        Wqkv, Wp, W1, W2 = (_WCACHE.get(w, cdt) for w in (qkvw, pw, f1w, f2w))
        u, mean1, rstd1 = ops.layernorm_fwd(x, n1w_, n1b_, eps)
        qkv_bias = torch.cat((_f32(qb), torch.zeros_like(_f32(vb)), _f32(vb)))
        qpre = _use_q_prescale(cdt, adrop)
        if qpre:
            D3 = qkv_bias.shape[0] // 3
            qkv_bias = qkv_bias.clone()
            qkv_bias[:D3] *= _Q_PRESCALE
            qkv = ops.gemm(u, _WCACHE.get_qscaled(qkvw, D3, _Q_PRESCALE, cdt), bias=qkv_bias)
        else:
            qkv = ops.gemm(u, Wqkv, bias=qkv_bias)
        o, lse = ops.mhsa_fwd(qkv, B, N, H, scale, drop=adrop, q_prescaled=qpre)
        if E1 is None:
            x1 = ops.gemm(o, Wp, bias=_f32(pb), res=x, row_scale=ds1, rows_per_scale=N)
        else:
            x1 = ops.mul_mask(ops.gemm(o, Wp, bias=_f32(pb)), E1, x)
        u2, mean2, rstd2 = ops.layernorm_fwd(x1, n2w_, n2b_, eps)
        hpre = torch.empty((x.shape[0], W1.shape[0]), dtype=cdt, device=x.device)
        hact = ops.gemm(u2, W1, bias=_f32(f1b), act=ACT_GELU, aux_out=hpre)
        if E2 is None:
            x2 = ops.gemm(hact, W2, bias=_f32(f2b), res=x1, row_scale=ds2, rows_per_scale=N)
        else:
            x2 = ops.mul_mask(ops.gemm(hact, W2, bias=_f32(f2b)), E2, x1)
        ctx.meta = meta
        ctx.drop = (E1, E2, adrop)
        ctx.qpre = qpre
        ctx.ds = (ds1, ds2)
        ctx.params = (n1w, n1b, qkvw, pw, pb, n2w, n2b, f1w, f1b, f2w, f2b, qb, vb)
        ctx.saved = (x, u, mean1, rstd1, qkv, o, lse, x1, u2, mean2, rstd2, hpre, hact, n1w_, n2w_, Wqkv, Wp, W1, W2)
        return x2

    @staticmethod
    def backward(ctx, dx2):
        B, N, H, eps, cdt = ctx.meta
        scale = 64 ** -0.5
        (x, u, mean1, rstd1, qkv, o, lse, x1, u2, mean2, rstd2, hpre, hact, n1w_, n2w_, Wqkv, Wp, W1, W2) = ctx.saved
        ctx.saved = None
        dx2 = dx2.contiguous()
        D = x.shape[1]
        dev = x.device
        ds1, ds2 = ctx.ds
        E1, E2, adrop = ctx.drop
        lane = _WgradLane(dev)
        (p_n1w, p_n1b, p_qkvw, p_pw, p_pb, p_n2w, p_n2b, p_f1w, p_f1b, p_f2w, p_f2b, p_qb, p_vb) = ctx.params
        f32 = lambda n: torch.empty((n,), dtype=torch.float32, device=dev)
        dst = lambda p_, n: _gout(p_) if _gout(p_) is not None else f32(n)
        if E2 is not None:
            g2 = ops.mul_mask(dx2, E2)
            db2 = ops.colsum(g2, out=_gout(p_f2b))
        elif ds2 is None:
            g2, db2 = dx2, _take_colsum(dx2, out=_gout(p_f2b))
        else:
            g2 = ops.row_scale(dx2, ds2, N)
            db2 = ops.colsum(g2, out=_gout(p_f2b))
        with lane.after_main():
            dW2 = ops.wgrad(g2, hact, out=_gout(p_f2w))
        db1 = dst(p_f1b, W1.shape[0])
        dhpre = ops.gemm(g2, W2, trans_b=True, act=ACT_DGELU, aux_in=hpre, colsum=db1)
        with lane.after_main():
            dW1 = ops.wgrad(dhpre, u2, out=_gout(p_f1w))
        du2 = ops.gemm(dhpre, W1, trans_b=True)
        dbp = dst(p_pb, D)
        dx1, dn2w, dn2b = ops.layernorm_bwd(du2, x1, n2w_, mean2, rstd2, dres=dx2, dx_colsum=dbp,
                                            dgamma=_gout(p_n2w), dbeta=_gout(p_n2b))
        if E1 is not None:
            g1 = ops.mul_mask(dx1, E1)
            dbp = ops.colsum(g1, out=dbp)
        elif ds1 is None:
            g1 = dx1
        else:
            g1 = ops.row_scale(dx1, ds1, N)
            dbp = ops.colsum(g1, out=dbp)
        with lane.after_main():
            dWp = ops.wgrad(g1, o, out=_gout(p_pw))
        dbq, dbv = dst(p_qb, D), dst(p_vb, D)
        if ops.mhsa_bwd_dv_from_do(g1.dtype, adrop):
            d_o = ops.gemm(g1, Wp, trans_b=True, colsum=dbv)
            dqkv = ops.mhsa_bwd(qkv, o, d_o, lse, B, N, H, scale, drop=adrop, bias_out=(dbq, None), q_prescaled=ctx.qpre)
        else:
            d_o = ops.gemm(g1, Wp, trans_b=True)
            dqkv = ops.mhsa_bwd(qkv, o, d_o, lse, B, N, H, scale, drop=adrop, bias_out=(dbq, dbv), q_prescaled=ctx.qpre)
        with lane.after_main():
            dWqkv = ops.wgrad(dqkv, u, out=_gout(p_qkvw))
        du = ops.gemm(dqkv, Wqkv, trans_b=True)
        dxs = f32(D)
        dx, dn1w, dn1b = ops.layernorm_bwd(du, x, n1w_, mean1, rstd1, dres=dx1, dx_colsum=dxs, dgamma=_gout(p_n1w), dbeta=_gout(p_n1b))
        _publish_colsum(dx, dxs)
        lane.join(dW2, dW1, dWp, dWqkv, dbq, dbv)
        return (dx, dn1w, dn1b, dWqkv, dbq, dbv, dWp, dbp, dn2w, dn2b, dW1, db1, dW2, db2, None, None, None, None)


class DropMaskFn(Function):

    @staticmethod
    def forward(ctx, x, mask):
        ctx.mask = mask
        return ops.mul_mask(x, mask)

    @staticmethod
    def backward(ctx, dy):
        return ops.mul_mask(dy.contiguous(), ctx.mask), None


class DropoutSource:

    def element_mask(self, kind: str, block: int, shape, keep: float, device) -> torch.Tensor:
        return ((keep + torch.rand(shape, device=device, dtype=torch.float32)).floor() / keep).contiguous()

    def path_scale(self, block: int, B: int, keep: float, device) -> torch.Tensor:
        return ((keep + torch.rand((2, B), device=device, dtype=torch.float32)).floor() / keep).contiguous()

    def attn_seed(self, block: int) -> int:
        return int(torch.randint(0, 2 ** 62, (1,), dtype=torch.int64).item())


_LAYER_KEYS = ("to_q", "to_k", "to_v", "to_out_w", "to_out_b", "norm_w", "norm_b", "ctx_w", "ctx_b",
               "ff0_w", "ff0_b", "ff3_w", "ff3_b", "ffn_w", "ffn_b")


class AggBlockFn(Function):

    @staticmethod
    def forward(ctx, x, norm_w, norm_b, latents, last_w, last_b, meta, *layer_params):
        B, N, S, depth, tied, heads, dh, eps_enc, eps_agg, cdt = meta
        nset = 1 if tied else depth
        assert len(layer_params) == nset * len(_LAYER_KEYS)
        LP = [dict(zip(_LAYER_KEYS, layer_params[i * 15:(i + 1) * 15])) for i in range(nset)]
        inner = heads * dh
        scale = dh ** -0.5
        dev = x.device
        M = x.shape[0]
        feats, m0, r0 = ops.layernorm_fwd(x, _f32(norm_w), _f32(norm_b), eps_enc)
        kvsets = []
        for P in LP:
            c, mc, rc = ops.layernorm_fwd(feats, _f32(P["ctx_w"]), _f32(P["ctx_b"]), eps_agg)
            Wkv = _WCACHE.get_cat((P["to_k"], P["to_v"]), cdt)
            kv = ops.gemm(c, Wkv)
            kvsets.append((c, mc, rc, Wkv, kv))
        xs = ops.rows_broadcast(_f32(latents), B * S, cdt)
        q_stack = torch.empty((depth, B * S, inner), dtype=cdt, device=dev)
        attn_stack = torch.empty((depth, B * heads, S, N), dtype=torch.float32, device=dev)
        rsum_stack = torch.empty((depth, B * heads, S), dtype=torch.float32, device=dev)
        layers = []
        for l in range(depth):
            P = LP[0 if tied else l]
            kv = kvsets[0 if tied else l][4]
            Wq, Wo, W1, W2 = (_WCACHE.get(P[k], cdt) for k in ("to_q", "to_out_w", "ff0_w", "ff3_w"))
            qn, mq, rq = ops.layernorm_fwd(xs, _f32(P["norm_w"]), _f32(P["norm_b"]), eps_agg)
            q = ops.gemm(qn, Wq, out=q_stack[l])
            _, _, o = ops.slot_attn_fwd(q, kv, B, S, N, heads, dh, scale, attn_out=attn_stack[l], rsum_out=rsum_stack[l])
            xs1 = ops.gemm(o, Wo, bias=_f32(P["to_out_b"]), res=xs)
            f, mf, rf = ops.layernorm_fwd(xs1, _f32(P["ffn_w"]), _f32(P["ffn_b"]), eps_agg)
            fpre = torch.empty((B * S, W1.shape[0]), dtype=cdt, device=dev)
            fact = ops.gemm(f, W1, bias=_f32(P["ff0_b"]), act=ACT_GELU, aux_out=fpre)
            xs2 = ops.gemm(fact, W2, bias=_f32(P["ff3_b"]), res=xs1)
            layers.append((xs, mq, rq, qn, o, xs1, mf, rf, f, fpre, fact, Wq, Wo, W1, W2))
            xs = xs2
        slots, ml, rl = ops.layernorm_fwd(xs, _f32(last_w), _f32(last_b), eps_agg)
        ctx.meta = meta
        ctx.saved = (x, m0, r0, feats, kvsets, layers, q_stack, attn_stack, rsum_stack, xs, ml, rl,
                     _f32(norm_w), _f32(last_w), [{k: _f32(P[k]) for k in ("norm_w", "ctx_w", "ffn_w")} for P in LP])
        return slots, attn_stack[depth - 1]

    @staticmethod
    def backward(ctx, dslots, dattn):
        B, N, S, depth, tied, heads, dh, eps_enc, eps_agg, cdt = ctx.meta
# ... 910 lines not shown
```

devias_amd/ops.py:

```python
from __future__ import annotations

import ctypes
from typing import Optional, Tuple

import torch

from . import _lib
from ._lib import ACT_DGELU, ACT_DRELU, ACT_GELU, ACT_NONE, ACT_RELU, ACT_SIGMOID, BF16, F32

_DT = {torch.float32: F32, torch.bfloat16: BF16}
_workspaces = {}


def dt_code(t: torch.dtype) -> int:
    try:
        return _DT[t]
    except KeyError:
        raise TypeError(f"devias_amd kernels support float32 and bfloat16 tensors, got {t}") from None


def _stream() -> int:
    return torch.cuda.current_stream().cuda_stream


def _p(t: Optional[torch.Tensor]) -> Optional[int]:
    return None if t is None else t.data_ptr()


def _chk(t: torch.Tensor, name: str, dtype=None) -> torch.Tensor:
    if not t.is_cuda:
        raise RuntimeError(f"{name}: devias_amd kernels need a GPU tensor (HIP extension only; no CPU fallback)")
    if not t.is_contiguous():
        raise RuntimeError(f"{name}: tensor must be contiguous, got strides {t.stride()}")
    if dtype is not None and t.dtype != dtype:
        raise TypeError(f"{name}: expected {dtype}, got {t.dtype}")
    return t


def workspace(nbytes: int, device) -> torch.Tensor:
    key = (torch.device(device).index or 0, torch.cuda.current_stream(device).cuda_stream)
    n = (int(nbytes) + 3) // 4
    ws = _workspaces.get(key)
    if ws is None or ws.numel() < n:
        ws = torch.empty(max(n, 1 << 20), dtype=torch.float32, device=device)
        _workspaces[key] = ws
    return ws




def get_option(name: str) -> int:
    v = ctypes.c_int32(0)
    _lib.check(_lib.load().devias_get_option(name.encode(), ctypes.byref(v)), "devias_get_option")
    return int(v.value)


def set_option(name: str, value: int) -> None:
    _lib.check(_lib.load().devias_set_option(name.encode(), int(value)), "devias_set_option")


def release_gemm_queue_stream(stream=None) -> None:
    st = torch.cuda.current_stream() if stream is None else stream
    _lib.check(_lib.load().devias_gemm_release_queue_stream(st.cuda_stream), "devias_gemm_release_queue_stream")


def counters(reset: bool = False) -> dict:
    lib = _lib.load()
    out = {k: int(lib.devias_counter(i)) for k, i in _lib.COUNTERS.items()}
    if reset:
        lib.devias_counters_reset()
    return out


def auto_split_k(M: int, N: int, K: int, bk: int = 64) -> int:
    cus = _lib.load().devias_policy_gemm_cus()
    if bk == 64 and M % 256 == 0 and N % 128 == 0:
        tiles, slots = (M // 256) * (N // 128), 2 * cus
    else:
        tiles, slots = ((M + 127) // 128) * ((N + 127) // 128), 3 * cus
    if tiles >= slots or K < 8 * bk:
        return 1
    return max(1, min(slots // tiles, K // (4 * bk), 64))


def gemm(A: torch.Tensor, B: torch.Tensor, *, trans_a: bool = False, trans_b: bool = False,
         bias: Optional[torch.Tensor] = None, act: int = ACT_NONE, aux_in: Optional[torch.Tensor] = None,
         aux_out: Optional[torch.Tensor] = None, res: Optional[torch.Tensor] = None, res_mod: int = 0,
         out: Optional[torch.Tensor] = None, out_f32: bool = False, beta: float = 0.0, split_k: int = 1,
         colsum: Optional[torch.Tensor] = None, colsum_beta: float = 0.0,
         row_scale: Optional[torch.Tensor] = None, rows_per_scale: int = 0) -> torch.Tensor:
    _chk(A, "gemm.A"); _chk(B, "gemm.B", A.dtype)
    assert A.dim() == 2 and B.dim() == 2
    M, K = (A.shape[1], A.shape[0]) if trans_a else (A.shape[0], A.shape[1])
    N, Kb = (B.shape[1], B.shape[0]) if trans_b else (B.shape[0], B.shape[1])
    if K != Kb:
        raise ValueError(f"gemm: reduction mismatch {K} vs {Kb}")
    cdt = torch.float32 if out_f32 else A.dtype
    if out is None:
        if beta != 0.0:
            raise ValueError("gemm: beta needs an existing `out`")
        out = torch.empty((M, N), dtype=cdt, device=A.device)
    else:
        _chk(out, "gemm.out", cdt)
        assert out.shape == (M, N)
    a = _lib.GemmArgs()
    a.A, a.B, a.C = A.data_ptr(), B.data_ptr(), out.data_ptr()
    a.M, a.N, a.K = M, N, K
    a.lda, a.ldb, a.ldc = A.shape[1], B.shape[1], N
    a.trans_a, a.trans_b = int(trans_a), int(trans_b)
    a.dtype = dt_code(A.dtype)
    a.c_f32 = int(cdt == torch.float32)
    a.bias = _p(_chk(bias, "gemm.bias", torch.float32)) if bias is not None else None
    a.act = act
    a.ld_aux = N
    if aux_in is not None:
        _chk(aux_in, "gemm.aux_in", A.dtype); assert aux_in.shape == (M, N)
        a.aux_in = aux_in.data_ptr()
    if aux_out is not None:
        _chk(aux_out, "gemm.aux_out", A.dtype); assert aux_out.shape == (M, N)
        a.aux_out = aux_out.data_ptr()
    if res is not None:
        _chk(res, "gemm.res", A.dtype)
        assert res.shape[-1] == N and res.numel() // N == (res_mod if res_mod > 0 else M)
        a.res, a.ldr, a.res_mod = res.data_ptr(), N, res_mod
    a.beta = beta
    if row_scale is not None:
        _chk(row_scale, "gemm.row_scale", torch.float32); assert rows_per_scale > 0 and row_scale.numel() * rows_per_scale >= M
        a.row_scale, a.rows_per_scale = row_scale.data_ptr(), rows_per_scale
    if split_k == 1 and M <= 256 and K >= 512 and not trans_a:
        tiles = ((M + 127) // 128) * ((N + 127) // 128)
        split_k = max(1, min(K // 128, (256 + tiles - 1) // tiles))
    if colsum is not None:
        _chk(colsum, "gemm.colsum", torch.float32); assert colsum.numel() == N
        split_k = 1
        a.colsum, a.colsum_beta = colsum.data_ptr(), colsum_beta
        nbytes = max(((M + 127) // 128) * N * 4, _lib.load().devias_colsum_workspace_bytes(M, N))
        a.ws = workspace(nbytes, A.device).data_ptr()
    a.split_k = split_k
    if split_k > 1:
        nbytes = _lib.load().devias_gemm_workspace_bytes(M, N, split_k)
        a.ws = workspace(nbytes, A.device).data_ptr()
    _lib.check(_lib.load().devias_gemm(ctypes.byref(a), _stream()), "devias_gemm")
    return out


def wgrad(dY: torch.Tensor, X: torch.Tensor, out: Optional[torch.Tensor] = None, beta: float = 0.0) -> torch.Tensor:
    M, N = dY.shape
    K = X.shape[1]
    sk = auto_split_k(N, K, M, bk=64 if dY.dtype == torch.bfloat16 else 16)
    return gemm(dY, X, trans_a=True, trans_b=True, out=out, out_f32=True, beta=beta, split_k=sk)


def cast(src: torch.Tensor, dtype: torch.dtype, out: Optional[torch.Tensor] = None, scale: Optional[float] = None) -> torch.Tensor:
    _chk(src, "cast.src")
    if out is None:
        out = torch.empty(src.shape, dtype=dtype, device=src.device)
    _chk(out, "cast.out", dtype)
    if scale is not None:
        _lib.check(_lib.load().devias_cast_scale(src.data_ptr(), dt_code(src.dtype), out.data_ptr(), dt_code(dtype), src.numel(), float(scale), _stream()),
                   "devias_cast_scale")
        return out
    _lib.check(_lib.load().devias_cast(src.data_ptr(), dt_code(src.dtype), out.data_ptr(), dt_code(dtype), src.numel(), _stream()),
               "devias_cast")
    return out


def patch_im2col(x: torch.Tensor, tubelet: int, patch: int, dtype: torch.dtype) -> torch.Tensor:
    _chk(x, "patch_im2col.x")
    B, C, T, H, W = x.shape
    n_tok = (T // tubelet) * (H // patch) * (W // patch)
    out = torch.empty((B * n_tok, C * tubelet * patch * patch), dtype=dtype, device=x.device)
    _lib.check(_lib.load().devias_patch_im2col(x.data_ptr(), dt_code(x.dtype), out.data_ptr(), dt_code(dtype), B, C, T, H, W,
                                               tubelet, patch, _stream()), "devias_patch_im2col")
    return out


def colsum(x: torch.Tensor, out: Optional[torch.Tensor] = None, beta: float = 0.0, cols: Optional[tuple] = None) -> torch.Tensor:
    _chk(x, "colsum.x")
    M, ld = x.shape
    c0, N = cols if cols is not None else (0, ld)
    assert 0 <= c0 and c0 + N <= ld
    if out is None:
        assert beta == 0.0
        out = torch.empty((N,), dtype=torch.float32, device=x.device)
    ws = workspace(_lib.load().devias_colsum_workspace_bytes(M, N), x.device)
    _lib.check(_lib.load().devias_colsum(x.data_ptr() + c0 * x.element_size(), dt_code(x.dtype), M, N, ld, out.data_ptr(), beta, ws.data_ptr(), _stream()),
               "devias_colsum")
    return out


def rows_reduce_mod(x: torch.Tensor, mod: int) -> torch.Tensor:
    _chk(x, "rows_reduce_mod.x")
    M, N = x.shape
    out = torch.empty((mod, N), dtype=torch.float32, device=x.device)
    _lib.check(_lib.load().devias_rows_reduce_mod(x.data_ptr(), dt_code(x.dtype), M, N, mod, out.data_ptr(), _stream()),
               "devias_rows_reduce_mod")
    return out


def rows_broadcast(src: torch.Tensor, M: int, dtype: torch.dtype) -> torch.Tensor:
    _chk(src, "rows_broadcast.src", torch.float32)
    mod, N = src.shape
    out = torch.empty((M, N), dtype=dtype, device=src.device)
    _lib.check(_lib.load().devias_rows_broadcast(src.data_ptr(), mod, N, out.data_ptr(), dt_code(dtype), M, _stream()),
               "devias_rows_broadcast")
    return out


def act_bwd(dy: torch.Tensor, y: torch.Tensor, act: int) -> torch.Tensor:
    _chk(dy, "act_bwd.dy"); _chk(y, "act_bwd.y", dy.dtype)
    dx = torch.empty_like(dy)
    _lib.check(_lib.load().devias_act_bwd(dy.data_ptr(), y.data_ptr(), dx.data_ptr(), act, dt_code(dy.dtype), dy.numel(), _stream()),
               "devias_act_bwd")
    return dx


def mul_mask(a: torch.Tensor, mask: torch.Tensor, b: Optional[torch.Tensor] = None) -> torch.Tensor:
    _chk(a, "mul_mask.a"); _chk(mask, "mul_mask.mask", torch.float32)
    assert mask.numel() == a.numel()
    if b is not None:
        _chk(b, "mul_mask.b", a.dtype)
    y = torch.empty_like(a)
    _lib.check(_lib.load().devias_mul_mask(a.data_ptr(), mask.data_ptr(), b.data_ptr() if b is not None else None, y.data_ptr(), dt_code(a.dtype), a.numel(), _stream()),
               "devias_mul_mask")
    return y


def row_scale(x: torch.Tensor, scale: torch.Tensor, rows_per_scale: int) -> torch.Tensor:
    _chk(x, "row_scale.x"); _chk(scale, "row_scale.scale", torch.float32)
    M, N = x.shape
    y = torch.empty_like(x)
    _lib.check(_lib.load().devias_row_scale(x.data_ptr(), scale.data_ptr(), rows_per_scale, y.data_ptr(), dt_code(x.dtype), M, N, _stream()),
               "devias_row_scale")
# ... 347 lines not shown
```

include/devias_amd.h:

```cpp
#ifndef DEVIAS_AMD_H
#define DEVIAS_AMD_H

#include <stdint.h>

#ifdef __cplusplus
extern "C" {
#endif

#define DEVIAS_OK 0
#define DEVIAS_EINVAL (-1)
#define DEVIAS_ELAUNCH (-2)
#define DEVIAS_EUNSUPPORTED (-3)

#define DEVIAS_F32 0
#define DEVIAS_BF16 1

#define DEVIAS_ACT_NONE 0
#define DEVIAS_ACT_GELU 1
#define DEVIAS_ACT_RELU 2
#define DEVIAS_ACT_SIGMOID 3
#define DEVIAS_ACT_DGELU 4
#define DEVIAS_ACT_DRELU 5

int devias_version(void);
const char* devias_last_error(void);
#define DEVIAS_CNT_GEMM128_F32 0
#define DEVIAS_CNT_GEMM128_BF16 1
#define DEVIAS_CNT_GEMM_SS 2
#define DEVIAS_CNT_GEMM256 3
#define DEVIAS_CNT_GEMM256P 4
#define DEVIAS_CNT_SPLITK_REDUCE 5
#define DEVIAS_CNT_MHSA_FWD_BF16 6
#define DEVIAS_CNT_MHSA_BWD_BF16 7
#define DEVIAS_CNT_MHSA_FWD_F32 8
#define DEVIAS_CNT_MHSA_BWD_F32 9
#define DEVIAS_CNT_GEMM_SK 11
#define DEVIAS_CNT_GEMM_SMALLM 13
#define DEVIAS_CNT_GEMM256W 12
#define DEVIAS_CNT_GEMM256D 14
#define DEVIAS_CNT_MHSA_BWD_FUSED 10
#define DEVIAS_CNT_DKDV1W 15
#define DEVIAS_CNT_DKDV1W_PERS 16
#define DEVIAS_CNT_DKDV1W_REST 17
#define DEVIAS_CNT_DKDV2W 18
#define DEVIAS_CNT_MHSA_QPRE 19
#define DEVIAS_CNT_LOSS_LABELS 20
#define DEVIAS_CNT_MAX 24
int64_t devias_counter(int32_t id);
void devias_counters_reset(void);
int devias_set_option(const char* name, int32_t value);
int devias_get_option(const char* name, int32_t* value);
int devias_gemm_release_queue_stream(void* stream);

int devias_allreduce_bucket(void* nccl_comm, void* bucket, int64_t count, int32_t dtype, void* stream);
void devias_shutdown(void);
void devias_range_push(const char* name);
void devias_range_pop(void);
int devias_debug_cu_hog(int32_t n_workgroups, int32_t usec, void* stream);
int devias_debug_mfma_probe(const void* data_bf16, int64_t data_elems, int32_t n_workgroups, int32_t iters, float* sink, uint64_t* stamps, void* stream);
int64_t devias_debug_mfma_probe_flops(int32_t n_workgroups, int32_t iters);
int devias_debug_gemm_timer_arm(int32_t M, int32_t N, int32_t K, int32_t trans_a, int32_t trans_b);
int devias_debug_gemm_timer_read(int32_t* count, float* total_ms);
int devias_debug_gemm_timer_read_each(int32_t* count, float* each_ms, int32_t cap);
int devias_debug_dkdv_stamps(uint64_t* out, int32_t n);

int devias_device_info(int device, int64_t* out5);

typedef struct {
    const void* A; const void* B; void* C;
    int32_t M, N, K;
    int32_t lda, ldb, ldc;
    int32_t trans_a, trans_b;
    int32_t dtype;
    int32_t c_f32;
    const float* bias;
    int32_t act;
    const void* aux_in;
    void* aux_out;
    int32_t ld_aux;
    const void* res;
    int32_t ldr, res_mod;
    float beta;
    int32_t split_k;
    float* ws;
    float* colsum;
    float colsum_beta;
    const float* row_scale;
    int32_t rows_per_scale;
    int32_t batch;
    int64_t stride_a, stride_b, stride_c;
    void* sk_ws;
    int64_t sk_ws_bytes;
} devias_gemm_args;
int devias_gemm(const devias_gemm_args* args, void* stream);
int64_t devias_gemm_workspace_bytes(int32_t M, int32_t N, int32_t split_k);

int devias_cast(const void* src, int32_t src_dtype, void* dst, int32_t dst_dtype, int64_t n, void* stream);
int devias_cast_scale(const void* src, int32_t src_dtype, void* dst, int32_t dst_dtype, int64_t n, float scale, void* stream);
int devias_patch_im2col(const void* x, int32_t x_dtype, void* out, int32_t out_dtype,
                        int32_t B, int32_t C, int32_t T, int32_t H, int32_t W, int32_t ts, int32_t ps, void* stream);
int devias_colsum(const void* x, int32_t dtype, int32_t M, int32_t N, int32_t ldx, float* out, float beta,
                  float* ws, void* stream);
int64_t devias_colsum_workspace_bytes(int32_t M, int32_t N);
int devias_rows_reduce_mod(const void* x, int32_t dtype, int32_t M, int32_t N, int32_t mod, float* out, void* stream);
int devias_rows_broadcast(const float* src, int32_t mod, int32_t N, void* out, int32_t dtype, int32_t M, void* stream);
int devias_act_bwd(const void* dy, const void* y_or_x, void* dx, int32_t act, int32_t dtype, int64_t n, void* stream);
int devias_row_scale(const void* x, const float* scale, int32_t rows_per_scale, void* y, int32_t dtype, int32_t M, int32_t N, void* stream);
int devias_mul_mask(const void* a, const float* mask, const void* b, void* y, int32_t dtype, int64_t n, void* stream);
int devias_add(const void* a, const void* b, void* y, int32_t dtype, int64_t n, void* stream);

int devias_layernorm_fwd(const void* x, const float* gamma, const float* beta, void* y, float* mean, float* rstd,
                         int32_t M, int32_t D, float eps, int32_t dtype, void* stream);
int devias_layernorm_bwd(const void* dy, const void* x, const float* gamma, const float* mean, const float* rstd,
                         const void* dres, void* dx, float* dgamma, float* dbeta, float beta_acc, float* dx_colsum,
                         int32_t M, int32_t D, int32_t dtype, float* ws, void* stream);
int64_t devias_layernorm_bwd_workspace_bytes(int32_t M, int32_t D);

int devias_mhsa_fwd(const void* qkv, void* o, float* lse, int32_t B, int32_t N, int32_t H, float scale,
                    int32_t dtype, void* stream);
int devias_mhsa_bwd(const void* qkv, const void* o, const void* d_o, const float* lse, float* delta, void* dqkv,
                    int32_t B, int32_t N, int32_t H, float scale, int32_t dtype, void* ws, void* stream);
int64_t devias_mhsa_bwd_workspace_bytes(int32_t B, int32_t N, int32_t H);
#define DEVIAS_ATTN_Q_PRESCALED 1
int devias_mhsa_fwd_flags(const void* qkv, void* o, float* lse, int32_t B, int32_t N, int32_t H, float scale,
                          int32_t dtype, int32_t flags, void* stream);
int devias_mhsa_bwd_flags(const void* qkv, const void* o, const void* d_o, const float* lse, float* delta, void* dqkv,
                          int32_t B, int32_t N, int32_t H, float scale, int32_t dtype, void* ws, int32_t flags, void* stream);
int devias_mhsa_fwd_dropout(const void* qkv, void* o, float* lse, int32_t B, int32_t N, int32_t H, float scale,
                            int32_t dtype, float keep, uint64_t seed, void* stream);
int devias_mhsa_bwd_dropout(const void* qkv, const void* o, const void* d_o, const float* lse, float* delta, void* dqkv,
                            int32_t B, int32_t N, int32_t H, float scale, int32_t dtype, float keep, uint64_t seed, void* stream);
int32_t devias_mhsa_bwd_bias_dv_from_do(int32_t dtype, float keep);
int devias_mhsa_bwd_bias(const void* qkv, const void* o, const void* d_o, const float* lse, float* delta, void* dqkv, int32_t B, int32_t N, int32_t H,
                         float scale, int32_t dtype, float keep, uint64_t seed, float* dbq, float* dbv, float* ws_q, float* ws_v, void* stream);
int devias_mhsa_bwd_bias_flags(const void* qkv, const void* o, const void* d_o, const float* lse, float* delta, void* dqkv, int32_t B, int32_t N, int32_t H,
                               float scale, int32_t dtype, float keep, uint64_t seed, float* dbq, float* dbv, float* ws_q, float* ws_v, int32_t flags, void* stream);
int64_t devias_mhsa_bwd_bias_workspace_bytes(int32_t B, int32_t N, int32_t H);

int devias_slot_attn_fwd(const void* q, const void* kv, float* attn, float* rsum, void* o,
                         int32_t B, int32_t S, int32_t N, int32_t h, int32_t dh, float scale, int32_t dtype,
                         float* ws, void* stream);
int devias_slot_attn_bwd(const void* q, const void* kv, const float* attn, const float* rsum, const void* o,
                         const void* d_o, const float* d_attn_ext, void* dq, float* ds,
                         int32_t B, int32_t S, int32_t N, int32_t h, int32_t dh, float scale, int32_t dtype,
                         float* ws, void* stream);
int devias_slot_attn_kv_grad(const void* q_stack, const void* do_stack, const float* ds_stack, const float* attn_stack,
                             const float* rsum_stack, void* dkv, int32_t L, int32_t B, int32_t S, int32_t N,
                             int32_t h, int32_t dh, float scale, int32_t dtype, void* stream);
int64_t devias_slot_attn_workspace_bytes(int32_t B, int32_t S, int32_t N, int32_t h, int32_t dh);

int devias_slotf_fwd(const void* qp, const void* ctx, float* attn, float* rsum, void* z, int32_t B, int32_t S, int32_t N,
                     int32_t h, int32_t D, float scale, int32_t dtype, float* ws, void* stream);
int devias_slotf_bwd(const void* ctx, const float* attn, const float* rsum, const void* z, const void* dz,
                     const float* d_attn_ext, void* dqp, float* ds, int32_t B, int32_t S, int32_t N, int32_t h, int32_t D,
                     float scale, int32_t dtype, float* ws, void* stream);
int devias_slotf_pack(const float* attn_stack, const float* rsum_stack, const float* ds_stack, const void* dz_stack,
                      const void* qp_stack, void* coef, void* vec, int32_t L, int32_t B, int32_t S, int32_t N, int32_t Np,
                      int32_t h, int32_t D, float scale, int32_t dtype, void* stream);
int64_t devias_slotf_workspace_bytes(int32_t B, int32_t S, int32_t N, int32_t h, int32_t D);

int devias_slot_select(const void* slots_head, int32_t dtype, int32_t B, int32_t S, int32_t C, int32_t nb,
                       int32_t* idx, void* stream);

typedef struct {
    int32_t B, S, C, nb, ns, D, G, N, nh;
    float w_scene, w_mask_pred, w_mask_distill;
    int32_t dtype;
    int32_t scene_ce;
} devias_loss_dims;
int devias_head_match_loss_fwd(const devias_loss_dims* d, const void* slots_head, const void* slots, const void* maskp,
                               const float* attn, const float* teacher, const int64_t* target, const float* fg,
                               const float* fgN, float* out_losses, int32_t* out_match, void* out_logits,
                               float* ws, void* stream);
int devias_head_match_loss_bwd(const devias_loss_dims* d, const void* slots_head, const void* slots, const void* maskp,
                               const float* attn, const float* teacher, const int64_t* target, const float* fg,
                               const float* fgN, const int32_t* match, const float* g_total,
                               void* d_slots_head, void* d_slots, void* d_maskp, float* d_attn, void* stream);
// ... 30 lines not shown
                       const float* grad_scale_dev, void* stream);

int devias_fame_diff_color(const float* video, int32_t B, int32_t T, int32_t H, int32_t W, float* diffs, int16_t* cmap, void* stream);
int devias_fame_blur(const float* in, float* out, int32_t n_img, int32_t H, int32_t W, int32_t ksize, float sigma, void* stream);
int devias_fame_seg_refine(const float* blurred, const int16_t* cmap, int32_t n_img, int32_t imgs_per_clip, int32_t HW, float eps,
                           float* refine, void* stream);
int devias_fame_binarize_pool(const float* blurred, int32_t n_img, int32_t H, int32_t W, int32_t num_fg, int32_t pool,
                              uint8_t* binmask, float* pooled, void* stream);
int devias_fame_mix(const float* video, const uint8_t* binmask, int32_t mask_stride, const int32_t* src, const int32_t* partner,
                    const int32_t* aug, float* out, int32_t B, int32_t CT, int32_t HW, void* stream);

typedef struct {
    int32_t B, N, D, H, hidden;
    int32_t dtype;
    float eps;
    const float *n1w, *n1b, *n2w, *n2b;
    const void *Wqkv, *Wp, *W1, *W2;
    const float* qkv_bias;
    const float *pb, *b1, *b2;
    const float *ds1, *ds2;
    void* save;
    float* ws; int64_t ws_bytes;
    void* sk_ws; int64_t sk_ws_bytes;
    const void *WqkvT, *WpT, *W1T, *W2T;
    const void* WqkvS; const float* qkv_biasS;
} devias_block_args;
typedef struct {
    float *dn1w, *dn1b, *dWqkv, *dbqkv , *dWp, *dbp, *dn2w, *dn2b, *dW1, *db1, *dW2, *db2;
    float* dx_colsum;
    int32_t db2_done;
    float *dbq, *dbv;
} devias_block_grads;
int64_t devias_encoder_block_save_bytes(int32_t B, int32_t N, int32_t D, int32_t H, int32_t hidden, int32_t dtype);
int64_t devias_encoder_block_scratch_bytes(int32_t B, int32_t N, int32_t D, int32_t H, int32_t hidden, int32_t dtype);
int64_t devias_encoder_block_workspace_bytes(int32_t B, int32_t N, int32_t D, int32_t H, int32_t hidden, int32_t dtype);
int devias_encoder_block_fwd(const devias_block_args* a, const void* x, void* x2, void* stream);
int devias_encoder_block_bwd(const devias_block_args* a, const void* x, const void* dx2, void* dx, const devias_block_grads* g,
                             void* scratch, int64_t scratch_bytes, void* stream);

typedef struct {
    int32_t R, D, C, h1, h2, G, dtype;
    const void *Wh, *W0, *W2, *W4;
    const float *bh, *b0, *b2, *b4;
    float* ws; int64_t ws_bytes;
    const float* drop_mask;
} devias_head_args;
typedef struct { float *dWh, *dbh, *dW0, *db0, *dW2, *db2, *dW4, *db4; } devias_head_grads;
int64_t devias_head_workspace_bytes(int32_t R, int32_t D, int32_t C, int32_t h1, int32_t h2, int32_t G, int32_t dtype);
int64_t devias_head_save_bytes(int32_t R, int32_t D, int32_t h1, int32_t h2, int32_t dtype);
int devias_head_fwd(const devias_head_args* a, const void* slots, void* Z, void* Mk, void* save, void* stream);
int devias_head_bwd(const devias_head_args* a, const void* slots, const void* Mk, const void* save, const void* dZ, const void* dM, void* dslots,
                    const devias_head_grads* g, void* stream);

#define DEVIAS_AGG_MAX_DEPTH 16
typedef struct {
    const void *Wq, *Wk, *Wv, *Wo, *W1, *W2;
    const float *bo, *norm_w, *norm_b, *ctx_w, *ctx_b, *b1, *b2, *ffn_w, *ffn_b;
} devias_agg_layer_params;
typedef struct { float *dWq, *dWk, *dWv, *dWo, *dbo, *dnorm_w, *dnorm_b, *dctx_w, *dctx_b, *dW1, *db1, *dW2, *db2, *dffn_w, *dffn_b; } devias_agg_layer_grads;
typedef struct {
    int32_t B, N, S, D, depth, tied, heads, dh, ff, dtype;
    float eps_enc, eps_agg;
    const float *norm_w, *norm_b;
    const float* latents;
    const float *last_w, *last_b;
    devias_agg_layer_params sets[DEVIAS_AGG_MAX_DEPTH];
    void* save;
    float* ws; int64_t ws_bytes;
} devias_agg_args;
typedef struct {
    float *dnorm_w, *dnorm_b, *dlatents, *dlast_w, *dlast_b;
    float* dx_colsum;
    devias_agg_layer_grads sets[DEVIAS_AGG_MAX_DEPTH];
} devias_agg_grads;
int64_t devias_agg_block_save_bytes(const devias_agg_args* a);
int64_t devias_agg_block_scratch_bytes(const devias_agg_args* a);
int64_t devias_agg_block_workspace_bytes(const devias_agg_args* a);
int devias_agg_block_fwd(const devias_agg_args* a, const void* x, void* slots, float** attn_out, void* stream);
int devias_agg_block_bwd(const devias_agg_args* a, const void* x, const void* dslots, const float* dattn, void* dx, const devias_agg_grads* g,
                         void* scratch, int64_t scratch_bytes, void* stream);
int32_t devias_policy_gemm_cus(void);
int32_t devias_policy_small_m_split(int32_t M, int32_t N, int32_t K, int32_t trans_a);
int32_t devias_policy_wgrad_split(int32_t Nout, int32_t Kin, int32_t Mrows, int32_t dtype);

#ifdef __cplusplus
}
#endif
#endif
```

Baseline: 674.2.

## Fuse weight-gradient GEMM into persistent dgrad kernel with cost-balanced K slabs

```diff
diff --git a/devias_amd/_lib.py b/devias_amd/_lib.py
--- a/devias_amd/_lib.py
+++ b/devias_amd/_lib.py
@@ -11,8 +11,9 @@
 
 F32, BF16 = 0, 1
 ATTN_Q_PRESCALED = 1
-ABI_VERSION = 168
+ABI_VERSION = 169
 ACT_NONE, ACT_GELU, ACT_RELU, ACT_SIGMOID, ACT_DGELU, ACT_DRELU = 0, 1, 2, 3, 4, 5
+PAIR_PLAIN, PAIR_CS, PAIR_DGELU_CS = 1, 2, 3
 
 
 class GemmArgs(Structure):
@@ -30,6 +31,7 @@
         ("row_scale", c_void_p), ("rows_per_scale", c_int32),
         ("batch", c_int32), ("stride_a", c_int64), ("stride_b", c_int64), ("stride_c", c_int64),
         ("sk_ws", c_void_p), ("sk_ws_bytes", c_int64),
+        ("wgrad_plan", c_int32),
     ]
 
 
@@ -108,6 +110,7 @@
     "devias_gemm_release_queue_stream": (c_int, [_P]),
     "devias_gemm": (c_int, [POINTER(GemmArgs), _P]),
     "devias_gemm_workspace_bytes": (c_int64, [_I, _I, _I]),
+    "devias_gemm_pair": (c_int, [POINTER(GemmArgs), POINTER(GemmArgs), _P]),
     "devias_cast": (c_int, [_P, _I, _P, _I, _L, _P]),
     "devias_cast_scale": (c_int, [_P, _I, _P, _I, _L, c_float, _P]),
     "devias_patch_im2col": (c_int, [_P, _I, _P, _I, _I, _I, _I, _I, _I, _I, _I, _P]),
@@ -176,10 +179,11 @@
     "devias_policy_gemm_cus": (c_int32, []),
     "devias_policy_small_m_split": (c_int32, [_I, _I, _I, _I]),
     "devias_policy_wgrad_split": (c_int32, [_I, _I, _I, _I]),
+    "devias_policy_gemm_pair_plan": (c_int32, [_I, _I, _I, _I, _I, POINTER(c_int32), _I]),
 }
 COUNTERS = {"gemm128_f32": 0, "gemm128_bf16": 1, "gemm_ss": 2, "gemm256": 3, "gemm256p": 4, "splitk_reduce": 5,
             "mhsa_fwd_bf16": 6, "mhsa_bwd_bf16": 7, "mhsa_fwd_f32": 8, "mhsa_bwd_f32": 9, "mhsa_bwd_fused": 10, "gemm_sk": 11, "gemm256w": 12, "gemm_smallm": 13, "gemm256d": 14,
-            "dkdv1w": 15, "dkdv1w_pers": 16, "dkdv1w_rest": 17, "dkdv2w": 18, "mhsa_qpre": 19, "loss_labels": 20}
+            "dkdv1w": 15, "dkdv1w_pers": 16, "dkdv1w_rest": 17, "dkdv2w": 18, "mhsa_qpre": 19, "loss_labels": 20, "gemm256pw": 21}
 OPT_CHUNK = 16384
 OPT_TENSOR_BYTES = 64
 
diff --git a/devias_amd/csrc/api.hip b/devias_amd/csrc/api.hip
--- a/devias_amd/csrc/api.hip
+++ b/devias_amd/csrc/api.hip
@@ -11,7 +11,7 @@
     return code;
 }
 
-extern "C" int devias_version(void) { return 168; }
+extern "C" int devias_version(void) { return 169; }
 
 #include <atomic>
 static std::atomic<int64_t> g_cnt[DEVIAS_CNT_MAX];
diff --git a/devias_amd/csrc/gemm.hip b/devias_amd/csrc/gemm.hip
--- a/devias_amd/csrc/gemm.hip
+++ b/devias_amd/csrc/gemm.hip
@@ -8,6 +8,18 @@
 namespace {
 
 enum { BM = 128, BN = 128, NTHREADS = 256 };
+
+struct SlabPlan {
+    int on;
+    int ntw, a, na;
+    int ls[2], es[2], ll[2], el[2];
+};
+__host__ __device__ __forceinline__ int slab_begin(const SlabPlan& s, int t, int z) {
+    const int v = t < s.na ? 0 : 1, sh = s.a + (v == 0 ? 1 : 0);
+    if (z <= sh) return z * s.ls[v] + (z < s.es[v] ? z : s.es[v]);
+    const int y = z - sh;
+    return sh * s.ls[v] + s.es[v] + y * s.ll[v] + (y < s.el[v] ? y : s.el[v]);
+}
 
 struct GemmP {
     const void* A; const void* B; void* C;
@@ -28,6 +40,7 @@
     int tail_split;
     int64_t sA, sB, sC;
     unsigned int* tq; unsigned int* tq_clear; int tq_nwhole[2], tq_items[2];
+    SlabPlan sp;
 };
 
 #ifdef DEVIAS_GEMM_DEBUG
@@ -784,28 +797,14 @@
     }
 }
 
-template <bool TA, bool TB, int PIN = 0>
-__global__ __launch_bounds__(NT2) void gemm256_kernel(GemmP p) {
-    __shared__ __attribute__((aligned(16))) char smem[2 * STAGE2];
+template <bool TA, bool TB, int PIN>
+__device__ __forceinline__ void gemm256_item(const GemmP& p, char* smem, int t, int z, int kbeg, int kend) {
     const int tid = threadIdx.x, lane = tid & 63;
     const int wave = __builtin_amdgcn_readfirstlane(tid >> 6);
     const int wm = wave >> 2, wn = wave & 3;
-    const int ntiles = p.tiles_m * p.tiles_n;
-    int t, z;
-    if (gridDim.y == 1 && p.split_k > 1) {
-        const int total = ntiles * p.split_k, per = (total + 7) >> 3;
-        const int j = (int)(blockIdx.x & 7) * per + (int)(blockIdx.x >> 3);
-        if (j >= total || (int)(blockIdx.x >> 3) >= per) return;
-        z = j / ntiles; t = j - z * ntiles;
-    } else {
-        t = xcd_remap(blockIdx.x, ntiles);
-        z = blockIdx.y;
-    }
     int tm, tn;
     tile_coords(t, p.tiles_m, p.tiles_n, p.group_m, tm, tn);
     const int m0 = tm * T2, n0 = tn * T2;
-    const int kbeg = z * p.k_per_split;
-    const int kend = min(p.K, kbeg + p.k_per_split);
     int nk = (kend - kbeg) / 64;
     if (GDBG(1)) nk = min(nk, 1);
     const bf16* A = reinterpret_cast<const bf16*>(p.A);
@@ -865,6 +864,26 @@
     epilogue_staged<8, 4>(p, acc, smem + wave * 16384, m0 + wm * 128, n0 + wn * 64, z, lane);
 }
 
+template <bool TA, bool TB, int PIN = 0>
+__global__ __launch_bounds__(NT2) void gemm256_kernel(GemmP p) {
+    __shared__ __attribute__((aligned(16))) char smem[2 * STAGE2];
+    const int ntiles = p.tiles_m * p.tiles_n;
+    int t, z;
+    if (gridDim.y == 1 && p.split_k > 1) {
+        const int total = ntiles * p.split_k, per = (total + 7) >> 3;
+        const int j = (int)(blockIdx.x & 7) * per + (int)(blockIdx.x >> 3);
+        if (j >= total || (int)(blockIdx.x >> 3) >= per) return;
+        z = j / ntiles; t = j - z * ntiles;
+    } else {
+        t = xcd_remap(blockIdx.x, ntiles);
+        z = blockIdx.y;
+    }
+    int kbeg, kend;
+    if (p.sp.on) { kbeg = slab_begin(p.sp, t, z) * 64; kend = slab_begin(p.sp, t, z + 1) * 64; }
+    else { kbeg = z * p.k_per_split; kend = min(p.K, kbeg + p.k_per_split); }
+    gemm256_item<TA, TB, PIN>(p, smem, t, z, kbeg, kend);
+}
+
 
 __device__ __forceinline__ void piece_rows(int code, int& lo, int& hi) {
     if (code < 0) { lo = 0; hi = 16; }
@@ -929,9 +948,9 @@
     return (v >> 28) == (seq & 15u) ? (int)(v & 0x0fffffffu) : -2;
 }
 
-template <bool TB, int SIDE, bool DYN, int EPI = -1>
-__global__ __launch_bounds__(NT2) void gemm256p_kernel(GemmP p) {
-    __shared__ __attribute__((aligned(16))) char smem[2 * STAGE2 + (DYN ? 16 : 0)];
+template <bool TB, int SIDE, bool DYN, int EPI, bool PIECES>
+__device__ __forceinline__ void gemm256p_body(const GemmP& p, char* smem) {
+    static_assert(!PIECES || (!DYN && !TB && !(EPI >= 0 && (EPI & EPI_CS))), "tail pieces: static lists, B k-contiguous, no column sums");
     const int tid = threadIdx.x, lane = tid & 63;
 #ifdef DEVIAS_GEMM_DEBUG
     const unsigned long long t_entry = __builtin_amdgcn_s_memrealtime();
@@ -956,7 +975,7 @@
     };
     const int rfull = cnt / stride, rem = cnt - rfull * stride;
     const bool split = p.tail_split != 0 && rfull >= 1 && rem > 0 && 2 * rem <= stride;
-    const int parts = (!split || DYN || TB || p.colsum_part != nullptr || p.tail_split < 3) ? 2 : min(min(p.tail_split, 4), stride / rem);
+    const int parts = (!PIECES || !split || DYN || TB || p.colsum_part != nullptr || p.tail_split < 3) ? 2 : min(min(p.tail_split, 4), stride / rem);
     auto tile_at = [&](int k, int& l, int& half) -> bool {
         half = -1;
         if (k < rfull) { l = li0 + k * stride; return true; }
@@ -1181,7 +1200,7 @@
             kt = 0;
             ++tk;
             m0 = m0n; n0 = n0n; half = halfn;
-            if (!DYN && !TB && half >= 16) { tail_piece = true; gtail = g + 1; break; }
+            if constexpr (PIECES) { if (half >= 16) { tail_piece = true; gtail = g + 1; break; } }
             act = half < 0 || wm == half;
             if constexpr (!DYN) {
                 int ln = li;
@@ -1196,7 +1215,7 @@
 #pragma unroll
                 for (int j = 0; j < 4; ++j) acc[i][j] = f32x4{0.f, 0.f, 0.f, 0.f};
         }
-        if constexpr (!DYN && !TB && !(EPI >= 0 && (EPI & EPI_CS))) {
+        if constexpr (PIECES) {
             if (tail_piece) {
                 int il, ih;
                 piece_wave_rows(half, wm, il, ih);
@@ -1239,6 +1258,52 @@
             }
         }
         asm volatile("s_waitcnt vmcnt(0)" ::: "memory");
+    }
+}
+
+template <bool TB, int SIDE, bool DYN, int EPI = -1>
+__global__ __launch_bounds__(NT2) void gemm256p_kernel(GemmP p) {
+    __shared__ __attribute__((aligned(16))) char smem[2 * STAGE2 + (DYN ? 16 : 0)];
+    gemm256p_body<TB, SIDE, DYN, EPI, (!DYN && !TB && !(EPI >= 0 && (EPI & EPI_CS)))>(p, smem);
+}
+
+struct PairP {
+    GemmP d, w;
+    unsigned long long hx;
+    int n_short, n_long;
+};
+template <int SIDE, int EPI, bool WFIRST>
+__global__ __launch_bounds__(NT2) void gemm256pw_kernel(PairP q) {
+    __shared__ __attribute__((aligned(16))) char smem[2 * STAGE2];
+    auto find_item = [&](int& t, int& z) -> bool {
+        const int xcd = blockIdx.x & 7, li0 = blockIdx.x >> 3, stride = gridDim.x >> 3;
+        int hb = 0, lb = 0, h = 0;
+#pragma unroll
+        for (int y = 0; y < 8; ++y) {
+            const int hy = (int)((q.hx >> (8 * y)) & 0xffu);
+            if (y < xcd) { hb += hy; lb += stride - hy; }
+            if (y == xcd) h = hy;
+        }
+        const int ntw = q.w.tiles_m * q.w.tiles_n;
+        int j;
+        if (li0 < h) { j = hb + li0; if (j >= q.n_short) return false; }
+        else { j = lb + li0 - h; if (j >= q.n_long) return false; j += q.n_short; }
+        z = j / ntw; t = j - z * ntw;
+        return z < q.w.split_k;
+    };
+    int t = 0, z = 0;
+    if constexpr (WFIRST) {
+        if (find_item(t, z)) gemm256_item<true, true, 0>(q.w, smem, t, z, slab_begin(q.w.sp, t, z) * 64, slab_begin(q.w.sp, t, z + 1) * 64);
+    } else {
+        gemm256p_body<false, SIDE, false, EPI, false>(q.d, smem);
+    }
+    asm volatile("s_waitcnt vmcnt(0)" ::: "memory");
+    __syncthreads();
+    if constexpr (WFIRST) {
+        gemm256p_body<false, SIDE, false, EPI, false>(q.d, smem);
+    } else {
+        if (!find_item(t, z)) return;
+        gemm256_item<true, true, 0>(q.w, smem, t, z, slab_begin(q.w.sp, t, z) * 64, slab_begin(q.w.sp, t, z + 1) * 64);
     }
 }
 
@@ -1895,6 +1960,9 @@
     int dynamic;
     int concurrent;
     int reserve;
+    int fuse_wgrad;
+    int pair_order;
+    int pair_scale;
     int ncu;
 };
 int env_int(const char* name, int dflt) { const char* e = getenv(name); return e ? atoi(e) : dflt; }
@@ -1917,6 +1985,9 @@
         x.epi_spec = env_int("DEVIAS_GEMM_EPI_SPEC", 1);
         x.wt = env_int("DEVIAS_GEMM_WT", 1);
         x.aux_nt = env_int("DEVIAS_GEMM_AUX_NT", 5);
+        x.fuse_wgrad = env_int("DEVIAS_GEMM_FUSE_WGRAD", 1);
+        x.pair_scale = env_int("DEVIAS_GEMM_PAIR_SCALE", 100);
+        x.pair_order = env_int("DEVIAS_GEMM_PAIR_ORDER", 0);
         x.ncu = 0;
         return x;
     }();
@@ -1985,6 +2056,9 @@
     if (!strcmp(name, "gemm_splitk_xcd")) return &k.splitk_xcd;
     if (!strcmp(name, "gemm_dynamic")) return &k.dynamic;
     if (!strcmp(name, "gemm_concurrent")) return &k.concurrent;
+    if (!strcmp(name, "gemm_fuse_wgrad")) return &k.fuse_wgrad;
+    if (!strcmp(name, "gemm_pair_scale")) return &k.pair_scale;
+    if (!strcmp(name, "gemm_pair_order")) return &k.pair_order;
     return nullptr;
 }
 int devias_gemm_set_option(const char* name, int value) {
@@ -1999,6 +2073,81 @@
     *value = *slot;
     return 1;
 }
+
+enum { PAIR_PLAIN = DEVIAS_PAIR_PLAIN, PAIR_CS = DEVIAS_PAIR_CS, PAIR_DGELU_CS = DEVIAS_PAIR_DGELU_CS };
+struct PairCost { float d_kt, d_tile; };
+static const PairCost kPairCost[4] = {{0.f, 0.f}, {1.75f, 2.f} , {1.75f, 2.f}, {1.90f, 10.f} };
+static int pair_cost_row(int form) { return form == PAIR_DGELU_CS ? PAIR_DGELU_CS : (form == PAIR_PLAIN || form == PAIR_CS ? PAIR_PLAIN : 0); }
+static const float kPairWgradKt = 2.0f, kPairWgradItem = 6.f;
+struct PairPlan {
+    SlabPlan sp;
+    int W, T, S, KT, base, H, n_short, n_long;
+    int cnt[8], rfull[8], rem[8], h[8];
+    unsigned long long hx;
+    float c_d, c_w, c_f;
+};
+static bool pair_plan(int M, int Nout, int Kin, int form, int S, PairPlan& pl) {
+    const GemmKnobs& kn = knobs();
+    memset(&pl, 0, sizeof(pl));
+    if (form < PAIR_PLAIN || form > PAIR_DGELU_CS) return false;
+    if (M <= 0 || Nout <= 0 || Kin <= 0 || (M % T2) || (Nout % T2) || (Kin % T2) || S < 2) return false;
+    if (kn.dynamic > 0 || (kn.dynamic < 0 && kn.concurrent != 0)) return false;
+    if (!kn.use256 || !kn.persistent || !kn.epi_swap || !kn.epi_spec || kn.debug || kn.w4 > 0) return false;
+    const int W = devias_policy_gemm_cus(), stride = W >> 3;
+    const int T = (M / T2) * (Kin / T2), ntw = (Nout / T2) * (Kin / T2), KT = M / 64;
+    if (W < 8 || stride > 255 || T <= W || ntw * S > W || KT < 4 * S) return false;
+    pl.W = W; pl.T = T; pl.S = S; pl.KT = KT;
+    pl.base = 1 << 30;
+    for (int x = 0; x < 8; ++x) {
+        pl.cnt[x] = (T >> 3) + (x < (T & 7) ? 1 : 0);
+        pl.rfull[x] = pl.cnt[x] / stride; pl.rem[x] = pl.cnt[x] % stride;
+        if (pl.rfull[x] < pl.base) pl.base = pl.rfull[x];
+    }
+    for (int x = 0; x < 8; ++x) {
+        if (pl.rfull[x] > pl.base && pl.rem[x] != 0) return false;
+        pl.h[x] = pl.rfull[x] > pl.base ? stride : pl.rem[x];
+        pl.H += pl.h[x];
+        pl.hx |= (unsigned long long)pl.h[x] << (8 * x);
+    }
+    const int items = ntw * S, nl = W - pl.H;
+    pl.n_short = items > nl ? items - nl : 0;
+    pl.n_long = items - pl.n_short;
+    if (pl.n_short > pl.H) return false;
+    pl.c_d = (Nout / 64 * kPairCost[pair_cost_row(form)].d_kt + kPairCost[pair_cost_row(form)].d_tile) * (float)kn.pair_scale * 0.01f;
+    pl.c_w = kPairWgradKt; pl.c_f = kPairWgradItem;
+    SlabPlan& sp = pl.sp;
+    sp.on = 1; sp.ntw = ntw; sp.a = pl.n_short / ntw; sp.na = pl.n_short % ntw;
+    const float D = pl.c_d / pl.c_w;
+    for (int v = 0; v < 2; ++v) {
+        const int sh = sp.a + (v == 0 ? 1 : 0), sl = S - sh;
+        if (v == 0 && sp.na == 0) { sp.ls[0] = sp.es[0] = sp.ll[0] = sp.el[0] = 0; continue; }
+        if (sl < 0) return false;
+        if (sh == 0) { sp.ls[v] = sp.es[v] = 0; sp.ll[v] = KT / S; sp.el[v] = KT % S; continue; }
+        if (sl == 0) { sp.ls[v] = KT / S; sp.es[v] = KT % S; sp.ll[v] = sp.el[v] = 0; continue; }
+        const float ls = ((float)KT - (float)sl * D) / (float)S;
+        if (ls < 4.f) return false;
+        int ht = (int)(ls * (float)sh + 0.5f);
+        if (ht < 4 * sh) ht = 4 * sh;
+        if (ht > KT - 4 * sl) return false;
+        sp.ls[v] = ht / sh; sp.es[v] = ht % sh;
+        sp.ll[v] = (KT - ht) / sl; sp.el[v] = (KT - ht) % sl;
+    }
+    return true;
+}
+static void pair_plan_wg(const PairPlan& pl, int b, int& ntile, int& first, int& step, int& wt, int& wz) {
+    const int x = b & 7, li0 = b >> 3, stride = pl.W >> 3;
+    int xbase = 0, hb = 0, lb = 0;
+    for (int y = 0; y < x; ++y) { xbase += pl.cnt[y]; hb += pl.h[y]; lb += stride - pl.h[y]; }
+    ntile = pl.rfull[x] + (li0 < pl.rem[x] ? 1 : 0);
+    first = xbase + li0; step = stride;
+    int j;
+    wt = wz = -1;
+    if (li0 < pl.h[x]) { j = hb + li0; if (j >= pl.n_short) return; }
+    else { j = lb + li0 - pl.h[x]; if (j >= pl.n_long) return; j += pl.n_short; }
+    wz = j / pl.sp.ntw; wt = j % pl.sp.ntw;
+}
+
+struct GemmForm { int kind; int ta, tb, side, epi, grid; };
 
 namespace {
 template <bool TB, int SIDE, bool DYN, int EPI>
@@ -2022,8 +2171,9 @@
 }
 }
 
-static int gemm_impl(const devias_gemm_args* a, void* stream) {
+static int gemm_impl(const devias_gemm_args* a, void* stream, int mode = 0, GemmP* outp = nullptr, GemmForm* form = nullptr) {
     hipStream_t st = (hipStream_t)stream;
+    if (form) form->kind = 0;
     DEVIAS_REQUIRE(a && a->A && a->B && a->C, "devias_gemm: null operand");
     DEVIAS_REQUIRE(a->M > 0 && a->N > 0 && a->K > 0, "devias_gemm: bad dims M=%d N=%d K=%d", a->M, a->N, a->K);
     DEVIAS_REQUIRE(a->dtype == DEVIAS_F32 || a->dtype == DEVIAS_BF16, "devias_gemm: bad dtype %d", a->dtype);
@@ -2078,6 +2228,7 @@
     p.c_nt = ((kn.aux_nt & 4) && a->aux_out) ? 1 : 0;
     p.epi_swap = kn.epi_swap;
     p.tq = nullptr; p.tq_clear = nullptr; p.tq_nwhole[0] = p.tq_nwhole[1] = p.tq_items[0] = p.tq_items[1] = 0;
+    memset(&p.sp, 0, sizeof(p.sp));
     p.group_m = kn.group_m > 0 ? kn.group_m : ((!a->trans_a && a->N >= 2048) ? 8 : 1);
 
     const bool v16 = vc && (a->N % 8 == 0) && (a->ldc % 8 == 0) && aligned16(a->C) && (!a->bias || aligned16(a->bias)) &&
@@ -2098,6 +2249,10 @@
                         (a->N % 16 == 0) && (a->K % 128 == 0) && (a->lda % 8 == 0) && (a->ldb % 8 == 0) && (a->ldc % 4 == 0) && aligned8(a->C) &&
                         (!a->bias || aligned16(a->bias)) && (!a->res || (a->ldr % 4 == 0 && aligned8(a->res))) &&
                         (!a->aux_in || (a->ld_aux % 4 == 0 && aligned8(a->aux_in))) && (!a->aux_out || (a->ld_aux % 4 == 0 && aligned8(a->aux_out)));
+    if (mode != 0 && (smallm || ss || !big)) {
+        DEVIAS_REQUIRE(mode == 1, "devias_gemm_pair: internal (mode 2 on a call it did not prepare)");
+        return DEVIAS_OK;
+    }
     if (smallm) {
         p.split_k = 1; p.k_per_split = a->K;
         const int mt = cdiv(a->M, 16);
@@ -2120,7 +2275,8 @@
                        "devias_gemm: colsum needs split_k == 1, a workspace (M/128 * N floats) and a T-typed C");
         if (ss || big) { p.colsum_part = a->ws; colsum_fused = true; }
     }
-    if (ss) {
+    if (mode == 2) {
+    } else if (ss) {
         p.tiles_m = a->M / SS_BM; p.tiles_n = a->N / SS_BN;
         dim3 grid(p.tiles_m * p.tiles_n, p.split_k), block(SS_NT);
         const int ta = a->trans_a, tb = a->trans_b;
@@ -2146,6 +2302,17 @@
         const int w4_mask = kn.w4 >= 0 ? kn.w4 : 0;
         const bool w4_ok = kn.persistent && !dyn && ((w4_mask >> w4_form) & 1) && pers_ok && !(!tb && side == 2) && nt > gp && a->K >= 128 &&
                            (a->act == DEVIAS_ACT_NONE || a->act == DEVIAS_ACT_GELU || a->act == DEVIAS_ACT_DGELU || a->act == DEVIAS_ACT_DRELU);
+        if (a->wgrad_plan > 0 && ta && tb && p.split_k > 1 && p.c_f32) {
+            PairPlan pl;
+            if (pair_plan(a->K, a->M, a->N, a->wgrad_plan, p.split_k, pl)) p.sp = pl.sp;
+        }
+        if (mode == 1) {
+            const int epi = !kn.epi_spec ? -1 : (a->act | (a->bias ? EPI_BIAS : 0) | (a->aux_out ? EPI_AUX : 0) | (a->row_scale ? EPI_RS : 0) | (p.colsum_part ? EPI_CS : 0));
+            if (!w4_ok && kn.persistent && pers_ok && nt > gp && !dyn) { form->kind = 1; form->tb = tb; form->side = side; form->epi = epi; form->grid = gp; }
+            else if (!w4_ok && !(kn.persistent && pers_ok && nt > gp)) { form->kind = 2; form->ta = ta; form->tb = tb; }
+            *outp = p;
+            return DEVIAS_OK;
+        }
         if (w4_ok) {
             dim3 grid(gp), block(NTW);
             PERS_LAUNCH(gemm256w_kernel);
@@ -2290,3 +2457,73 @@
     (void)hipEventRecord(t.e1[slot], (hipStream_t)stream);
     return rc;
 }
+
+namespace {
+template <int SIDE, int EPI>
+void pair_launch1(dim3 grid, hipStream_t st, const PairP& q, bool wfirst) {
+    if (wfirst) hipLaunchKernelGGL((gemm256pw_kernel<SIDE, EPI, true>), grid, dim3(NT2), 0, st, q);
+    else hipLaunchKernelGGL((gemm256pw_kernel<SIDE, EPI, false>), grid, dim3(NT2), 0, st, q);
+}
+}
+extern "C" int devias_gemm_pair(const devias_gemm_args* d, const devias_gemm_args* w, void* stream) {
+    DEVIAS_REQUIRE(d && w, "devias_gemm_pair: null args");
+    const GemmKnobs& kn = knobs();
+    const int pform = (d->act == DEVIAS_ACT_DGELU && d->colsum) ? PAIR_DGELU_CS : ((d->act == DEVIAS_ACT_NONE && d->colsum) ? PAIR_CS : (d->act == DEVIAS_ACT_NONE ? PAIR_PLAIN : 0));
+    devias_gemm_args wa = *w;
+    if (kn.fuse_wgrad && pform && wa.wgrad_plan == 0) wa.wgrad_plan = pform;
+    bool fuse = kn.fuse_wgrad != 0 && pform != 0 && pair_cost_row(wa.wgrad_plan) == pair_cost_row(pform) && d->A == w->A && d->M == w->K && d->K == w->M && d->N == w->N && d->dtype == DEVIAS_BF16 &&
+                w->dtype == DEVIAS_BF16 && !d->trans_a && !d->trans_b && w->trans_a && w->trans_b && w->c_f32 && !d->bias && !d->res && !d->aux_out && !d->row_scale &&
+                !w->bias && !w->res && !w->row_scale && w->act == DEVIAS_ACT_NONE && !w->colsum && d->batch <= 1 && w->batch <= 1 && w->split_k > 1;
+    PairP q;
+    GemmForm fd, fw;
+    if (fuse) {
+        int rc = gemm_impl(d, stream, 1, &q.d, &fd);
+        if (rc) return rc;
+        rc = gemm_impl(&wa, stream, 1, &q.w, &fw);
+        if (rc) return rc;
+        const bool epi_ok = (pform == PAIR_PLAIN && fd.side == 0 && fd.epi == 0) || (pform == PAIR_CS && fd.side == 0 && fd.epi == EPI_CS) ||
+                            (pform == PAIR_DGELU_CS && fd.side == 2 && fd.epi == (DEVIAS_ACT_DGELU | EPI_CS));
+        const int64_t total = (int64_t)w->M * w->N;
+        const bool plain = w->ldc == w->N && (total % 4 == 0) && aligned16(w->ws) && aligned16(w->C);
+        fuse = fd.kind == 1 && !fd.tb && epi_ok && fw.kind == 2 && fw.ta && fw.tb && q.w.sp.on && q.w.epi_swap && plain;
+    }
+    PairPlan pl;
+    if (fuse) fuse = pair_plan(d->M, d->K, d->N, pair_cost_row(pform), q.w.split_k, pl) && pl.W == fd.grid && !memcmp(&pl.sp, &q.w.sp, sizeof(pl.sp)) &&
+                     q.w.tiles_m * q.w.tiles_n == pl.sp.ntw && q.d.tiles_m * q.d.tiles_n == pl.T && q.w.K == pl.KT * 64;
+    if (!fuse) {
+        const int rc = devias_gemm(&wa, stream);
+        return rc ? rc : devias_gemm(d, stream);
+    }
+    q.d.tail_split = 0;
+    q.hx = pl.hx; q.n_short = pl.n_short; q.n_long = pl.n_long;
+    const bool wfirst = kn.pair_order != 0;
+    const dim3 grid(pl.W);
+    hipStream_t st = (hipStream_t)stream;
+    if (pform == PAIR_PLAIN) pair_launch1<0, 0>(grid, st, q, wfirst);
+    else if (pform == PAIR_CS) pair_launch1<0, EPI_CS>(grid, st, q, wfirst);
+    else pair_launch1<2, DEVIAS_ACT_DGELU | EPI_CS>(grid, st, q, wfirst);
+    devias_count(DEVIAS_CNT_GEMM256P);
+    devias_count(DEVIAS_CNT_GEMM256);
+    devias_count(DEVIAS_CNT_GEMM256PW);
+    DEVIAS_CHECK_LAUNCH("devias_gemm_pair");
+    int rc = gemm_impl(&wa, stream, 2);
+    if (rc) return rc;
+    return gemm_impl(d, stream, 2);
+}
+
+extern "C" int32_t devias_policy_gemm_pair_plan(int32_t M, int32_t Nout, int32_t Kin, int32_t form, int32_t split_k, int32_t* out, int32_t cap) {
+    PairPlan pl;
+    if (!pair_plan(M, Nout, Kin, form, split_k, pl)) return 0;
+    if (!out || cap < 12 + 8 * pl.W) return 1;
+    const int hdr[12] = {pl.W, pl.T, pl.S, pl.sp.ntw, pl.KT, pl.base, pl.n_short, pl.n_long, (int)(pl.c_d * 16.f + 0.5f), (int)(pl.c_w * 16.f + 0.5f), (int)(pl.c_f * 16.f + 0.5f), 0};
+    for (int i = 0; i < 12; ++i) out[i] = hdr[i];
+    for (int b = 0; b < pl.W; ++b) {
+        int nt, first, step, wt, wz, kb = 0, ke = 0;
+        pair_plan_wg(pl, b, nt, first, step, wt, wz);
+        float fin = nt * pl.c_d;
+        if (wt >= 0) { kb = slab_begin(pl.sp, wt, wz); ke = slab_begin(pl.sp, wt, wz + 1); fin += pl.c_f + (ke - kb) * pl.c_w; }
+        int32_t* o = out + 12 + 8 * b;
+        o[0] = nt; o[1] = first; o[2] = step; o[3] = wt; o[4] = wz; o[5] = kb * 64; o[6] = ke * 64; o[7] = (int32_t)(fin * 16.f + 0.5f);
+    }
+    return 1;
+}
diff --git a/devias_amd/csrc/regions.hip b/devias_amd/csrc/regions.hip
--- a/devias_amd/csrc/regions.hip
+++ b/devias_amd/csrc/regions.hip
@@ -43,9 +43,8 @@
     float* colsum = nullptr; float colsum_beta = 0.f;
     const float* row_scale = nullptr; int rows_per_scale = 0;
 };
-int gemm(const Ctx& c, const void* A, const void* B, void* C, int M, int N, int K, int lda, int ldb, int trans_a, int trans_b, const Epi& e,
-         int c_f32 = 0, float beta = 0.f, int split_k = 1) {
-    devias_gemm_args a;
+int gemm_fill(devias_gemm_args& a, const Ctx& c, const void* A, const void* B, void* C, int M, int N, int K, int lda, int ldb, int trans_a, int trans_b, const Epi& e,
+              int c_f32 = 0, float beta = 0.f, int split_k = 1) {
     memset(&a, 0, sizeof(a));
     a.A = A; a.B = B; a.C = C; a.M = M; a.N = N; a.K = K; a.lda = lda; a.ldb = ldb; a.ldc = N;
     a.trans_a = trans_a; a.trans_b = trans_b; a.dtype = c.dtype; a.c_f32 = c_f32;
@@ -59,11 +58,33 @@
         if (devias_gemm_workspace_bytes(M, N, split_k) > c.ws_bytes) return devias_set_error(DEVIAS_EINVAL, "fused region: workspace too small for a split-K GEMM (%d x %d x %d)", M, N, split_k);
         a.ws = c.ws;
     }
-    return devias_gemm(&a, c.st);
+    return DEVIAS_OK;
+}
+int gemm(const Ctx& c, const void* A, const void* B, void* C, int M, int N, int K, int lda, int ldb, int trans_a, int trans_b, const Epi& e,
+         int c_f32 = 0, float beta = 0.f, int split_k = 1) {
+    devias_gemm_args a;
+    const int rc = gemm_fill(a, c, A, B, C, M, N, K, lda, ldb, trans_a, trans_b, e, c_f32, beta, split_k);
+    return rc ? rc : devias_gemm(&a, c.st);
 }
 int wgrad(const Ctx& c, const void* dY, const void* X, float* dW, int M, int Nout, int Kin, float beta = 0.f) {
     Epi e;
     return gemm(c, dY, X, dW, Nout, Kin, M, Nout, Kin, 1, 1, e, 1, beta, wgrad_split(Nout, Kin, M, c.dtype));
+}
+int wgrad_form(const Ctx& c, const void* dY, const void* X, float* dW, int M, int Nout, int Kin, int form) {
+    devias_gemm_args w;
+    Epi none;
+    int on = 0;
+    const int rc = gemm_fill(w, c, dY, X, dW, Nout, Kin, M, Nout, Kin, 1, 1, none, 1, 0.f, wgrad_split(Nout, Kin, M, c.dtype));
+    if (rc) return rc;
+    if (devias_gemm_get_option("gemm_fuse_wgrad", &on) && on) w.wgrad_plan = form;
+    return devias_gemm(&w, c.st);
+}
+int linear_bwd_pair(const Ctx& cd, const Ctx& cw, const void* dY, const void* WT, void* dX, const void* X, float* dW, int M, int Nout, int Kin, const Epi& e) {
+    devias_gemm_args d, w;
+    Epi none;
+    int rc = gemm_fill(d, cd, dY, WT, dX, M, Kin, Nout, Nout, Nout, 0, 0, e);
+    if (!rc) rc = gemm_fill(w, cw, dY, X, dW, Nout, Kin, M, Nout, Kin, 1, 1, none, 1, 0.f, wgrad_split(Nout, Kin, M, cw.dtype));
+    return rc ? rc : devias_gemm_pair(&d, &w, cd.st);
 }
 int gemm_batched(const Ctx& c, const void* A, const void* B, void* C, int c_f32, int M, int N, int K, int lda, int ldb, int ldc, int64_t sa, int64_t sb, int64_t sc,
                  int batch, int trans_a, int trans_b) {
@@ -200,33 +221,33 @@
     } else if (!g->db2_done) {
         RUN(colsum(with_ws(t.p_b2), dx2, M, D, g->db2));
     }
-    RUN(wgrad(c, g2, s.hact, g->dW2, M, D, hid));
+    if (!W2T) RUN(wgrad_form(c, g2, s.hact, g->dW2, M, D, hid, DEVIAS_PAIR_DGELU_CS));
     { Epi e; e.act = DEVIAS_ACT_DGELU; e.aux_in = s.hpre; e.colsum = g->db1;
-      if (W2T) RUN(gemm(with_ws(t.p_db1), g2, W2T, t.big, M, hid, D, D, D, 0, 0, e)); else RUN(gemm(with_ws(t.p_db1), g2, a->W2, t.big, M, hid, D, D, hid, 0, 1, e)); }
-    RUN(wgrad(c, t.big, s.u2, g->dW1, M, hid, D));
-    { Epi e; if (W1T) RUN(gemm(c, t.big, W1T, t.small, M, D, hid, hid, hid, 0, 0, e)); else RUN(gemm(c, t.big, a->W1, t.small, M, D, hid, hid, D, 0, 1, e)); }
+      if (W2T) RUN(linear_bwd_pair(with_ws(t.p_db1), c, g2, W2T, t.big, s.hact, g->dW2, M, D, hid, e)); else RUN(gemm(with_ws(t.p_db1), g2, a->W2, t.big, M, hid, D, D, hid, 0, 1, e)); }
+    if (!W1T) RUN(wgrad_form(c, t.big, s.u2, g->dW1, M, hid, D, DEVIAS_PAIR_PLAIN));
+    { Epi e; if (W1T) RUN(linear_bwd_pair(c, c, t.big, W1T, t.small, s.u2, g->dW1, M, hid, D, e)); else RUN(gemm(c, t.big, a->W1, t.small, M, D, hid, hid, D, 0, 1, e)); }
     RUN(ln_bwd(with_ws(t.p_ln2), t.small, s.x1, a->n2w, s.mean2, s.rstd2, dx2, t.dx1, g->dn2w, g->dn2b, 0.f, a->ds1 ? nullptr : g->dbp, M, D));
     const void* g1 = t.dx1;
     if (a->ds1) {
         RUN(devias_row_scale_colsum(t.dx1, a->ds1, N, t.g, a->dtype, M, D, g->dbp, 0.f, t.p_bp, (hipStream_t)stream));
         g1 = t.g;
     }
-    RUN(wgrad(c, g1, s.o, g->dWp, M, D, D));
+    if (!WpT) RUN(wgrad_form(c, g1, s.o, g->dWp, M, D, D, DEVIAS_PAIR_PLAIN));
     const bool dv_from_do = g->dbq && g->dbv && devias_mhsa_bwd_bias_dv_from_do(a->dtype, 1.0f);
     const int aflags = block_qpre(a) ? DEVIAS_ATTN_Q_PRESCALED : 0;
     { Epi e; if (dv_from_do) e.colsum = g->dbv;
       const Ctx k = dv_from_do ? with_ws(t.p_v) : c;
-      if (WpT) RUN(gemm(k, g1, WpT, t.small, M, D, D, D, D, 0, 0, e)); else RUN(gemm(k, g1, a->Wp, t.small, M, D, D, D, D, 0, 1, e)); }
+      if (WpT) RUN(linear_bwd_pair(k, c, g1, WpT, t.small, s.o, g->dWp, M, D, D, e)); else RUN(gemm(k, g1, a->Wp, t.small, M, D, D, D, D, 0, 1, e)); }
     if (g->dbq && g->dbv)
         RUN(devias_mhsa_bwd_bias_flags(s.qkv, s.o, t.small, s.lse, t.delta, t.big, B, N, H, 0.125f, a->dtype, 1.0f, 0, g->dbq, dv_from_do ? nullptr : g->dbv, t.p_q, t.p_v, aflags, stream));
     else
         RUN(devias_mhsa_bwd_flags(s.qkv, s.o, t.small, s.lse, t.delta, t.big, B, N, H, 0.125f, a->dtype, t.p_q, aflags, stream));
-    RUN(wgrad(c, t.big, s.u, g->dWqkv, M, 3 * D, D));
+    if (!WqkvT) RUN(wgrad_form(c, t.big, s.u, g->dWqkv, M, 3 * D, D, DEVIAS_PAIR_PLAIN));
     if (g->dbq && g->dbv) {
     } else {
         RUN(colsum(with_ws(t.p_q), t.big, M, 3 * D, g->dbqkv));
     }
-    { Epi e; if (WqkvT) RUN(gemm(c, t.big, WqkvT, t.small, M, D, 3 * D, 3 * D, 3 * D, 0, 0, e)); else RUN(gemm(c, t.big, a->Wqkv, t.small, M, D, 3 * D, 3 * D, D, 0, 1, e)); }
+    { Epi e; if (WqkvT) RUN(linear_bwd_pair(c, c, t.big, WqkvT, t.small, s.u, g->dWqkv, M, 3 * D, D, e)); else RUN(gemm(c, t.big, a->Wqkv, t.small, M, D, 3 * D, 3 * D, D, 0, 1, e)); }
     RUN(ln_bwd(with_ws(t.p_ln1), t.small, x, a->n1w, s.mean1, s.rstd1, t.dx1, dx, g->dn1w, g->dn1b, 0.f, g->dx_colsum, M, D));
     RUN(devias_flush_deferred(&dl, (hipStream_t)stream));
     return DEVIAS_OK;
diff --git a/devias_amd/modeling_slot.py b/devias_amd/modeling_slot.py
--- a/devias_amd/modeling_slot.py
+++ b/devias_amd/modeling_slot.py
@@ -10,7 +10,7 @@
 from torch.autograd import Function
 
 from . import ops
-from .ops import ACT_DGELU, ACT_DRELU, ACT_GELU, ACT_NONE, ACT_RELU, ACT_SIGMOID
+from .ops import ACT_DGELU, ACT_DRELU, ACT_GELU, ACT_NONE, ACT_RELU, ACT_SIGMOID, PAIR_DGELU_CS, PAIR_PLAIN
 
 _MODEL_REGISTRY: Dict[str, callable] = {}
 
@@ -318,11 +318,11 @@
             g2 = ops.row_scale(dx2, ds2, N)
             db2 = ops.colsum(g2, out=_gout(p_f2b))
         with lane.after_main():
-            dW2 = ops.wgrad(g2, hact, out=_gout(p_f2w))
+            dW2 = ops.wgrad(g2, hact, out=_gout(p_f2w), pair_form=PAIR_DGELU_CS)
         db1 = dst(p_f1b, W1.shape[0])
         dhpre = ops.gemm(g2, W2, trans_b=True, act=ACT_DGELU, aux_in=hpre, colsum=db1)
         with lane.after_main():
-            dW1 = ops.wgrad(dhpre, u2, out=_gout(p_f1w))
+            dW1 = ops.wgrad(dhpre, u2, out=_gout(p_f1w), pair_form=PAIR_PLAIN)
         du2 = ops.gemm(dhpre, W1, trans_b=True)
         dbp = dst(p_pb, D)
         dx1, dn2w, dn2b = ops.layernorm_bwd(du2, x1, n2w_, mean2, rstd2, dres=dx2, dx_colsum=dbp,
@@ -336,7 +336,7 @@
             g1 = ops.row_scale(dx1, ds1, N)
             dbp = ops.colsum(g1, out=dbp)
         with lane.after_main():
-            dWp = ops.wgrad(g1, o, out=_gout(p_pw))
+            dWp = ops.wgrad(g1, o, out=_gout(p_pw), pair_form=PAIR_PLAIN)
         dbq, dbv = dst(p_qb, D), dst(p_vb, D)
         if ops.mhsa_bwd_dv_from_do(g1.dtype, adrop):
             d_o = ops.gemm(g1, Wp, trans_b=True, colsum=dbv)
@@ -345,7 +345,7 @@
             d_o = ops.gemm(g1, Wp, trans_b=True)
             dqkv = ops.mhsa_bwd(qkv, o, d_o, lse, B, N, H, scale, drop=adrop, bias_out=(dbq, dbv), q_prescaled=ctx.qpre)
         with lane.after_main():
-            dWqkv = ops.wgrad(dqkv, u, out=_gout(p_qkvw))
+            dWqkv = ops.wgrad(dqkv, u, out=_gout(p_qkvw), pair_form=PAIR_PLAIN)
         du = ops.gemm(dqkv, Wqkv, trans_b=True)
         dxs = f32(D)
         dx, dn1w, dn1b = ops.layernorm_bwd(du, x, n1w_, mean1, rstd1, dres=dx1, dx_colsum=dxs, dgamma=_gout(p_n1w), dbeta=_gout(p_n1b))
diff --git a/devias_amd/ops.py b/devias_amd/ops.py
--- a/devias_amd/ops.py
+++ b/devias_amd/ops.py
@@ -6,7 +6,7 @@
 import torch
 
 from . import _lib
-from ._lib import ACT_DGELU, ACT_DRELU, ACT_GELU, ACT_NONE, ACT_RELU, ACT_SIGMOID, BF16, F32
+from ._lib import ACT_DGELU, ACT_DRELU, ACT_GELU, ACT_NONE, ACT_RELU, ACT_SIGMOID, BF16, F32, PAIR_CS, PAIR_DGELU_CS, PAIR_PLAIN
 
 _DT = {torch.float32: F32, torch.bfloat16: BF16}
 _workspaces = {}
@@ -88,7 +88,8 @@
          aux_out: Optional[torch.Tensor] = None, res: Optional[torch.Tensor] = None, res_mod: int = 0,
          out: Optional[torch.Tensor] = None, out_f32: bool = False, beta: float = 0.0, split_k: int = 1,
          colsum: Optional[torch.Tensor] = None, colsum_beta: float = 0.0,
-         row_scale: Optional[torch.Tensor] = None, rows_per_scale: int = 0) -> torch.Tensor:
+         row_scale: Optional[torch.Tensor] = None, rows_per_scale: int = 0, wgrad_plan: int = 0, _fill_only: bool = False,
+         _ws: Optional[torch.Tensor] = None):
     _chk(A, "gemm.A"); _chk(B, "gemm.B", A.dtype)
     assert A.dim() == 2 and B.dim() == 2
     M, K = (A.shape[1], A.shape[0]) if trans_a else (A.shape[0], A.shape[1])
@@ -135,20 +136,39 @@
         split_k = 1
         a.colsum, a.colsum_beta = colsum.data_ptr(), colsum_beta
         nbytes = max(((M + 127) // 128) * N * 4, _lib.load().devias_colsum_workspace_bytes(M, N))
-        a.ws = workspace(nbytes, A.device).data_ptr()
+        assert _ws is None or _ws.numel() * 4 >= nbytes
+        a.ws = (_ws if _ws is not None else workspace(nbytes, A.device)).data_ptr()
     a.split_k = split_k
+    a.wgrad_plan = int(wgrad_plan)
     if split_k > 1:
         nbytes = _lib.load().devias_gemm_workspace_bytes(M, N, split_k)
         a.ws = workspace(nbytes, A.device).data_ptr()
+    if _fill_only:
+        return a, out
     _lib.check(_lib.load().devias_gemm(ctypes.byref(a), _stream()), "devias_gemm")
     return out
 
 
-def wgrad(dY: torch.Tensor, X: torch.Tensor, out: Optional[torch.Tensor] = None, beta: float = 0.0) -> torch.Tensor:
+def wgrad(dY: torch.Tensor, X: torch.Tensor, out: Optional[torch.Tensor] = None, beta: float = 0.0, pair_form: int = 0, _fill_only: bool = False):
     M, N = dY.shape
     K = X.shape[1]
     sk = auto_split_k(N, K, M, bk=64 if dY.dtype == torch.bfloat16 else 16)
-    return gemm(dY, X, trans_a=True, trans_b=True, out=out, out_f32=True, beta=beta, split_k=sk)
+    plan = pair_form if (pair_form and get_option("gemm_fuse_wgrad")) else 0
+    return gemm(dY, X, trans_a=True, trans_b=True, out=out, out_f32=True, beta=beta, split_k=sk, wgrad_plan=plan, _fill_only=_fill_only)
+
+
+def gemm_pair(dY: torch.Tensor, WT: torch.Tensor, X: torch.Tensor, *, act: int = ACT_NONE, aux_in: Optional[torch.Tensor] = None,
+              colsum: Optional[torch.Tensor] = None, dW: Optional[torch.Tensor] = None, beta: float = 0.0, wgrad_plan: int = 0):
+    cs_ws = None
+    if colsum is not None:
+        M, N = dY.shape[0], WT.shape[0]
+        nbytes = max(((M + 127) // 128) * N * 4, _lib.load().devias_colsum_workspace_bytes(M, N))
+        cs_ws = torch.empty((nbytes + 3) // 4, dtype=torch.float32, device=dY.device)
+    d, dX = gemm(dY, WT, act=act, aux_in=aux_in, colsum=colsum, _fill_only=True, _ws=cs_ws)
+    w, dW = wgrad(dY, X, out=dW, beta=beta, _fill_only=True)
+    w.wgrad_plan = int(wgrad_plan)
+    _lib.check(_lib.load().devias_gemm_pair(ctypes.byref(d), ctypes.byref(w), _stream()), "devias_gemm_pair")
+    return dX, dW
 
 
 def cast(src: torch.Tensor, dtype: torch.dtype, out: Optional[torch.Tensor] = None, scale: Optional[float] = None) -> torch.Tensor:
diff --git a/include/devias_amd.h b/include/devias_amd.h
--- a/include/devias_amd.h
+++ b/include/devias_amd.h
@@ -45,6 +45,7 @@
 #define DEVIAS_CNT_DKDV2W 18
 #define DEVIAS_CNT_MHSA_QPRE 19
 #define DEVIAS_CNT_LOSS_LABELS 20
+#define DEVIAS_CNT_GEMM256PW 21
 #define DEVIAS_CNT_MAX 24
 int64_t devias_counter(int32_t id);
 void devias_counters_reset(void);
@@ -91,8 +92,13 @@
     int64_t stride_a, stride_b, stride_c;
     void* sk_ws;
     int64_t sk_ws_bytes;
+    int32_t wgrad_plan;
 } devias_gemm_args;
+#define DEVIAS_PAIR_PLAIN 1
+#define DEVIAS_PAIR_CS 2
+#define DEVIAS_PAIR_DGELU_CS 3
 int devias_gemm(const devias_gemm_args* args, void* stream);
+int devias_gemm_pair(const devias_gemm_args* dgrad, const devias_gemm_args* wgrad, void* stream);
 int64_t devias_gemm_workspace_bytes(int32_t M, int32_t N, int32_t split_k);
 
 int devias_cast(const void* src, int32_t src_dtype, void* dst, int32_t dst_dtype, int64_t n, void* stream);
@@ -289,6 +295,7 @@
 int32_t devias_policy_gemm_cus(void);
 int32_t devias_policy_small_m_split(int32_t M, int32_t N, int32_t K, int32_t trans_a);
 int32_t devias_policy_wgrad_split(int32_t Nout, int32_t Kin, int32_t Mrows, int32_t dtype);
+int32_t devias_policy_gemm_pair_plan(int32_t M, int32_t Nout, int32_t Kin, int32_t form, int32_t split_k, int32_t* out, int32_t cap);
 
 #ifdef __cplusplus
 }
```

Result: no change. 678.5, median of 6 (+0.6%).
